# ai-forever/Kandinsky-2

Hardware: AMD Instinct MI355X
Metric: UNet denoise steps/sec @ 768x768 bs=1, 50 steps (higher is better)
Workload: dtype bf16; 1 GPU; Kandinsky-2.x text2img 768x768, decoder_steps=50, bs=1/GPU (CFG batch 2x4x96x96), 2.1-architecture UNet (1.23B) p_sampler step; parity pinned against the reference's modules; head=2.1, tile_configs_measured_in_this_process=0, images_per_gpu=1, parallelism=prompt-sharded x1, weights by one RCCL broadcast, world_size_observed=1, graph=True, chains=1, loop_graph=a 5-step loop replayed as ONE hipGraph (83 replay(s) = 415 timed steps)

## Files before the change

include/k22.h:

```cpp
#ifndef K22_H
#define K22_H
#include <stddef.h>
#include <stdint.h>
#ifdef __cplusplus
extern "C" {
#endif

#define K22_OK 0
#define K22_EINVAL (-1)
#define K22_EHIP (-2)
#define K22_ENOMEM (-3)

#define K22_BF16 0
#define K22_F32 1
#define K22_F16 2
#define K22_F16X3 3
#define K22_F16X2 4

int k22_version(void);
#define K22_BUILD_PACKED_FP32 1
#define K22_BUILD_DEBUG_VARIANTS 2
int k22_build_flags(void);
const char* k22_last_error(void);
int k22_set_option(const char* name, int value);
// ... 35 lines not shown
void k22_unet_destroy(K22UNet* u);


int k22_unet_plan(K22UNet* u, int B, int H, int W, size_t* workspace_bytes);
int k22_unet_bind(K22UNet* u, void* workspace, size_t workspace_bytes);

int k22_unet_set_condition(K22UNet* u, const float* full_emb, const float* pooled_emb, const float* image_emb,
                           void* stream);

int k22_unet_set_hint(K22UNet* u, const float* hint, void* stream);

int k22_unet_forward(K22UNet* u, const float* x, const float* timesteps, const float* inpaint_image,
                     const float* inpaint_mask, float* out, int use_graph, void* stream);

int k22_unet_sample_loop(K22UNet* u, float* x, float* x_tmp, const float* timesteps, const float* noise_seq, const float* init_img,
                         const float* mask, const float* inpaint_image, const float* inpaint_mask, const float* table,
                         const int* table_rows, int n_steps, float guidance, float clamp_lo, float clamp_hi, int pct_index,
                         double pct_gamma, void* scratch, int use_graph, void* stream);
enum { K22_LOOP_DDIM = 0, K22_LOOP_PLMS = 1 };
int k22_unet_ddim_loop(K22UNet* u, int kind, float* x, float* x_tmp, float* x0_out, const float* timesteps, const float* table,
                       const float* noise_seq, const float* inpaint_image, const float* inpaint_mask, float* eps_hist, int n_steps,
                       float guidance, int use_graph, void* stream);
int k22_unet_num_ops(const K22UNet* u);
int k22_unet_set_autotune(K22UNet* u, int on);
int k22_unet_tuning_report(const K22UNet* u, char* buf, size_t cap);

int k22_comm_broadcast_weights(void* arena, size_t bytes, int root, void* nccl_comm, void* stream);

int k22_tile_table_load(const char* path);
int k22_tile_table_save(const char* path);
int k22_tile_table_size(void);
int k22_tile_table_measured(void);
void k22_tile_table_clear(void);

int k22_unet_profile(K22UNet* u, int reps, double* ms, double* flops, double* bytes, int* launches, void* stream);

size_t k22_sampler_scratch_bytes(int N, int HW);
int k22_ddim_step(const float* x, const float* model_out, const float* noise, const float* table_row, float guidance, int use_cfg,
                  float* x_out, float* x0_out, int N, int HW, void* stream);
int k22_prepare_mask(const float* mask, float* out, int C, int H, int W, void* stream);
int k22_plms_step(const float* x, const float* model_out, const float* eps_hist1, const float* eps_hist2, const float* eps_hist3, int order,
                  const float* table_row, float guidance, int use_cfg, float* x_out, float* eps_out, float* x0_out, int N, int HW, void* stream);
int k22_sampler_step(const float* x, const float* model_out, const float* noise, const float* init_img,
                     const float* mask, const float* table, int step_index, float guidance, int use_cfg,
                     float clamp_lo, float clamp_hi, int pct_index, double pct_gamma, void* scratch,
                     float* x_out, float* x0_out, int N, int HW, void* stream);

int k22_gemm(const void* A0, const void* A1, const void* Wp, const float* bias, const void* residual, void* out,
             void* partial, int M, int N, int Npad, int K0, int K1, long lda0, long lda1, int ldo, int ldr,
             int out_f32, int act, int splitk, int bm, int bn, int dtype, void* stream);
int k22_x3_pack(const float* src, void* dst, long n, float scale, void* stream);
int k22_conv3x3(const void* x_padded, const void* Wp, const float* bias, const void* residual, void* out,
                void* partial, int B, int H, int W, int Cin, int Cout, int Npad, int out_mode, int act, int splitk,
                int bm, int bn, int dtype, void* stream);
int k22_conv3x3_skip(const void* x_padded, const void* Wp, const float* bias, const void* skip0, const void* skip1,
                     int SK0, int SK1, const void* Ws, const float* bias_s, void* out, void* partial, int B, int H, int W,
                     int Cin, int Cout, int Npad, int splitk, int bm, int dtype, void* stream);
int k22_conv3x3_gnstats(const void* x_padded, const void* Wp, const float* bias, const void* residual, void* out,
                        void* partial, int B, int H, int W, int Cin, int Cout, int Npad, int splitk, int bm, int bn,
                        float* stats, int stats_capacity_rows, int* rows_per_image, int dtype, void* stream);
int k22_gemm_gnstats(const void* A, const void* Wp, const float* bias, const void* residual, void* out, void* partial,
                     int B, int H, int W, int N, int Npad, int K, int splitk, int bm, float* stats,
                     int stats_capacity_rows, int* rows_per_image, int dtype, void* stream);
typedef struct K22IgemmProblem {
  int dtype, taps, M, N, Kc, K0, H, W;
  int out_mode, res_f32, act, a_raw, want_stats;
  int SK0, SK1;
  int att_T, att_S, att_Tkp;
  int ldo, ldr;
  int has_frag;
  int algo, bm, bn, splitk, stages;
} K22IgemmProblem;
typedef struct K22IgemmOperands {
  const void *A0, *A1, *Wp, *bias, *residual;
  void *out, *partial;
  const void *S0, *S1, *Ws, *bias2;
  void *kall, *vtall;
  const void *Wfrag, *Wsfrag;
  float* stats;
  int stats_capacity_rows;
} K22IgemmOperands;
int k22_igemm_cfg_accepted(const K22IgemmProblem* pr);
int k22_igemm_cfg(const K22IgemmProblem* pr, const K22IgemmOperands* ops, int* rows_per_image, void* stream);
int k22_debug_conv_trace(const void* x_padded, const void* Wp, const float* bias, void* out, int B, int H, int W, int Cin, int Cout,
                         int Npad, unsigned long long* trace, void* stream);
int k22_conv3x3_gn(const void* x0, const void* x1, int C0, int C1, const float* gamma, const float* beta, const float* film, long film_ld,
                   float eps, int act, void* scratch, const void* Wp, const float* bias, const void* residual, void* out, void* partial,
                   int B, int H, int W, int Cout, int Npad, int splitk, int bm, int algo, int dtype, void* stream);
int k22_groupnorm(const void* x0, const void* x1, int C0, int C1, int B, int H, int W, const float* gamma,
                  const float* beta, const float* film, long film_ld, float eps, int act, int mode, int pad,
                  void* scratch, void* out, int dtype, void* stream);
size_t k22_groupnorm_scratch_bytes(int B, int C);
int k22_attention(const void* qkv, const void* ctxkv, void* kall, void* vtall, void* out, int B, int H, int T, int S,
                  int dtype, void* stream);
int k22_qkv_project(const void* x, const void* Wp, const float* bias, void* q_out, void* kall, void* vtall,
                    int B, int H, int T, int S, int K, int bm, int bn, int dtype, void* stream);
int k22_qkv_project_stream(const void* x, const void* Wp, const float* bias, void* q_out, void* kall, void* vtall, void* partial,
                           int B, int H, int T, int S, int K, int bm, int splitk, int dtype, void* stream);
int k22_linear_smallm(const float* x, const void* W, const float* bias, const float* add, float* out, int M, int N,
                      int K, int act_in, int act_out, int wdtype, void* stream);
int k22_conv3x3_direct(const float* x, const float* w, const float* bias, float* y, int B, int Cin, int Cout, int Hin, int Win,
                       int stride, int act, void* stream);

size_t k22_afrag_bytes(int M, int K);
int k22_afrag_pack(const void* A, long lda, void* out, int M, int K, int dtype, void* stream);
int k22_skinny_gemm(const void* Afrag, const void* Wfrag, const float* bias, void* out, float* partial, int M, int N, int Npad, int K,
                    int splitk, int epi, int act, int ldo, int mt, int nb, int dtype, void* stream);
int k22_finish_ln(const float* partial, int splitk, const float* bias, float* x, long ldx, const float* gain, const float* beta, void* yfrag,
                  int M, int N, float eps, int dtype, void* stream);
int k22_small_attention(const void* qkv, const float* qkv_partial, int nsplit, const float* qkv_bias, void* out, int out_frag, int B, int H, int T,
                        int causal, const float* key_valid, int kv_n, int dtype, void* stream);

typedef struct K22PriorConfig {
  int dtype;
  int text_ctx;
  int xf_width;
  int xf_layers;
  int xf_heads;
  int xf_final_ln;
  int clip_dim;
  int clip_xf_width;
} K22PriorConfig;
typedef struct K22Prior K22Prior;
int k22_prior_create(const K22PriorConfig* cfg, const K22Weight* weights, int n_weights, K22Prior** out);
void k22_prior_destroy(K22Prior* m);
int k22_prior_plan(K22Prior* m, int B, size_t* workspace_bytes);
int k22_prior_bind(K22Prior* m, void* workspace, size_t workspace_bytes);
int k22_prior_tuning_report(const K22Prior* m, char* buf, size_t cap);
int k22_prior_forward(K22Prior* m, const float* x, const float* timesteps, const float* text_emb, const float* text_enc,
                      const float* key_valid, float* out, void* stream);
int k22_prior_sampler_step(const float* x, const float* model_out, const float* noise, const float* scales, const float* table_row,
                           float clamp, float* x_out, int bs, int D, void* stream);

typedef struct K22MoVQConfig {
  int dtype;
  int ch;
  int n_levels;
  int ch_mult[8];
  int num_res_blocks;
  int attn_levels;
  int z_channels;
  int out_ch;
} K22MoVQConfig;
typedef struct K22MoVQ K22MoVQ;
int k22_movq_create(const K22MoVQConfig* cfg, const K22Weight* weights, int n_weights, K22MoVQ** out);
void k22_movq_destroy(K22MoVQ* m);
int k22_movq_plan(K22MoVQ* m, int B, int h, int w, size_t* workspace_bytes);
int k22_movq_bind(K22MoVQ* m, void* workspace, size_t workspace_bytes);
int k22_movq_decode(K22MoVQ* m, const float* z, float* out, unsigned char* out_u8, void* stream);
int k22_movq_plan_encoder(K22MoVQ* m, int B, int H, int W, size_t* workspace_bytes);
int k22_movq_encode(K22MoVQ* m, const float* image, float* latent, void* stream);
int k22_movq_num_ops(const K22MoVQ* m);

enum { K22_ENC_CLIP_TEXT = 0, K22_ENC_CLIP_VISION = 1, K22_ENC_XLMR = 2 };
typedef struct K22EncoderConfig {
  int dtype;
  int kind;
  int width;
  int layers;
  int heads;
  int n_ctx;
  int vocab;
  int out_dim;
  int image_size;
  int patch;
  int max_pos;
// ... 47 lines not shown
```

kandinsky-2_amd/_lib.py:

```python
from __future__ import annotations

import ctypes as C
import os

_HERE = os.path.dirname(os.path.abspath(__file__))
LIB_PATH = os.environ.get("K22_LIB_PATH") or os.path.join(_HERE, "libk22hip.so")
TILE_TABLE_PATH = os.path.join(_HERE, "tiles_gfx950.txt")

K22_BF16, K22_F32, K22_F16, K22_F16X3, K22_F16X2 = 0, 1, 2, 3, 4
K22_LOOP_DDIM, K22_LOOP_PLMS = 0, 1
F16X3 = "f16x3"
F16X2 = "f16x2"
SPLIT_DTYPES = (F16X3, F16X2)
X3_WSCALE = 256.0


def dtype_code(backend_dtype) -> int:
    import torch
    try:
        return {torch.bfloat16: K22_BF16, torch.float32: K22_F32, torch.float16: K22_F16, F16X3: K22_F16X3, F16X2: K22_F16X2}[backend_dtype]
    except KeyError:
        raise ValueError('backend_dtype must be torch.bfloat16, torch.float16, torch.float32 "f16x3" or "f16x2"') from None
ACT_NONE, ACT_SILU, ACT_GELU = 0, 1, 2
OUT_ROWMAJOR, OUT_ROWMAJOR_F32, OUT_NCHW_F32, OUT_QKV = 0, 1, 2, 3
# ... 27 lines not shown


class K22PriorConfig(C.Structure):
    _fields_ = [("dtype", C.c_int), ("text_ctx", C.c_int), ("xf_width", C.c_int), ("xf_layers", C.c_int), ("xf_heads", C.c_int),
                ("xf_final_ln", C.c_int), ("clip_dim", C.c_int), ("clip_xf_width", C.c_int)]


class K22EncoderConfig(C.Structure):
    _fields_ = [("dtype", C.c_int), ("kind", C.c_int), ("width", C.c_int), ("layers", C.c_int), ("heads", C.c_int), ("n_ctx", C.c_int),
                ("vocab", C.c_int), ("out_dim", C.c_int), ("image_size", C.c_int), ("patch", C.c_int), ("max_pos", C.c_int),
                ("pad_id", C.c_int), ("ln_eps", C.c_float), ("mlp_dim", C.c_int), ("hidden_act", C.c_int)]


class K22Weight(C.Structure):
    _fields_ = [("name", C.c_char_p), ("ptr", C.c_void_p)]


_P, _I, _L, _F, _D, _Z = C.c_void_p, C.c_int, C.c_long, C.c_float, C.c_double, C.c_size_t

SIGNATURES = {
    "k22_version": (_I, []),
    "k22_build_flags": (_I, []),
    "k22_last_error": (C.c_char_p, []),
    "k22_set_option": (_I, [C.c_char_p, _I]),
    "k22_comm_broadcast_weights": (_I, [_P, _Z, _I, _P, _P]),
    "k22_tile_table_load": (_I, [C.c_char_p]),
    "k22_tile_table_save": (_I, [C.c_char_p]),
    "k22_tile_table_size": (_I, []),
    "k22_tile_table_measured": (_I, []),
    "k22_tile_table_clear": (None, []),
    "k22_unet_create": (_I, [C.POINTER(K22UNetConfig), C.POINTER(K22Weight), _I, C.POINTER(_P)]),
    "k22_unet_destroy": (None, [_P]),
    "k22_unet_plan": (_I, [_P, _I, _I, _I, C.POINTER(_Z)]),
    "k22_unet_bind": (_I, [_P, _P, _Z]),
    "k22_unet_set_condition": (_I, [_P, _P, _P, _P, _P]),
    "k22_unet_set_hint": (_I, [_P, _P, _P]),
    "k22_unet_forward": (_I, [_P, _P, _P, _P, _P, _P, _I, _P]),
    "k22_unet_sample_loop": (_I, [_P, _P, _P, _P, _P, _P, _P, _P, _P, _P, C.POINTER(_I), _I, _F, _F, _F, _I, _D, _P, _I, _P]),
    "k22_unet_ddim_loop": (_I, [_P, _I, _P, _P, _P, _P, _P, _P, _P, _P, _P, _I, _F, _I, _P]),
    "k22_unet_num_ops": (_I, [_P]),
    "k22_unet_set_autotune": (_I, [_P, _I]),
    "k22_unet_tuning_report": (_I, [_P, C.c_char_p, _Z]),
    "k22_unet_profile": (_I, [_P, _I, C.POINTER(_D), C.POINTER(_D), C.POINTER(_D), C.POINTER(_I), _P]),
    "k22_afrag_bytes": (_Z, [_I, _I]),
    "k22_afrag_pack": (_I, [_P, _L, _P, _I, _I, _I, _P]),
    "k22_skinny_gemm": (_I, [_P, _P, _P, _P, _P, _I, _I, _I, _I, _I, _I, _I, _I, _I, _I, _I, _P]),
    "k22_finish_ln": (_I, [_P, _I, _P, _P, _L, _P, _P, _P, _I, _I, _F, _I, _P]),
    "k22_small_attention": (_I, [_P, _P, _I, _P, _P, _I, _I, _I, _I, _I, _P, _I, _I, _P]),
    "k22_prior_create": (_I, [C.POINTER(K22PriorConfig), C.POINTER(K22Weight), _I, C.POINTER(_P)]),
    "k22_prior_destroy": (None, [_P]),
    "k22_prior_plan": (_I, [_P, _I, C.POINTER(_Z)]),
    "k22_prior_bind": (_I, [_P, _P, _Z]),
    "k22_prior_tuning_report": (_I, [_P, C.c_char_p, _Z]),
    "k22_prior_forward": (_I, [_P, _P, _P, _P, _P, _P, _P, _P]),
    "k22_prior_sampler_step": (_I, [_P, _P, _P, _P, _P, _F, _P, _I, _I, _P]),
    "k22_encoder_create": (_I, [C.POINTER(K22EncoderConfig), C.POINTER(K22Weight), _I, C.POINTER(_P)]),
    "k22_encoder_destroy": (None, [_P]),
    "k22_encoder_plan": (_I, [_P, _I, C.POINTER(_Z)]),
    "k22_encoder_bind": (_I, [_P, _P, _Z]),
    "k22_encoder_forward": (_I, [_P, _P, _P, _P, _P, _P, _P]),
    "k22_movq_create": (_I, [C.POINTER(K22MoVQConfig), C.POINTER(K22Weight), _I, C.POINTER(_P)]),
    "k22_movq_destroy": (None, [_P]),
    "k22_movq_plan": (_I, [_P, _I, _I, _I, C.POINTER(_Z)]),
    "k22_movq_bind": (_I, [_P, _P, _Z]),
    "k22_movq_decode": (_I, [_P, _P, _P, _P, _P]),
    "k22_movq_plan_encoder": (_I, [_P, _I, _I, _I, C.POINTER(_Z)]),
    "k22_movq_encode": (_I, [_P, _P, _P, _P]),
    "k22_movq_num_ops": (_I, [_P]),
    "k22_ddim_step": (_I, [_P, _P, _P, _P, _F, _I, _P, _P, _I, _I, _P]),
    "k22_blend_noised": (_I, [_P, _P, _P, _P, _F, _F, _P, _I, _I, _I, _I, _P]),
    "k22_prepare_mask": (_I, [_P, _P, _I, _I, _I, _P]),
    "k22_plms_step": (_I, [_P, _P, _P, _P, _P, _I, _P, _F, _I, _P, _P, _P, _I, _I, _P]),
    "k22_sampler_scratch_bytes": (_Z, [_I, _I]),
    "k22_sampler_step": (_I, [_P, _P, _P, _P, _P, _P, _I, _F, _I, _F, _F, _I, _D, _P, _P, _P, _I, _I, _P]),
    "k22_gemm": (_I, [_P, _P, _P, _P, _P, _P, _P, _I, _I, _I, _I, _I, _L, _L, _I, _I, _I, _I, _I, _I, _I, _I, _P]),
    "k22_x3_pack": (_I, [_P, _P, _L, _F, _P]),
    "k22_conv3x3": (_I, [_P, _P, _P, _P, _P, _P, _I, _I, _I, _I, _I, _I, _I, _I, _I, _I, _I, _I, _P]),
    "k22_conv3x3_skip": (_I, [_P, _P, _P, _P, _P, _I, _I, _P, _P, _P, _P, _I, _I, _I, _I, _I, _I, _I, _I, _I, _P]),
    "k22_gemm_gnstats": (_I, [_P, _P, _P, _P, _P, _P, _I, _I, _I, _I, _I, _I, _I, _I, _P, _I, C.POINTER(_I), _I, _P]),
    "k22_conv3x3_gnstats": (_I, [_P, _P, _P, _P, _P, _P, _I, _I, _I, _I, _I, _I, _I, _I, _I, _P, _I, C.POINTER(_I), _I, _P]),
    "k22_igemm_cfg_accepted": (_I, [C.POINTER(K22IgemmProblem)]),
    "k22_igemm_cfg": (_I, [C.POINTER(K22IgemmProblem), C.POINTER(K22IgemmOperands), C.POINTER(_I), _P]),
    "k22_conv3x3_gn": (_I, [_P, _P, _I, _I, _P, _P, _P, _L, _F, _I, _P, _P, _P, _P, _P, _P, _I, _I, _I, _I, _I, _I, _I, _I, _I, _P]),
    "k22_debug_conv_trace": (_I, [_P, _P, _P, _P, _I, _I, _I, _I, _I, _I, _P, _P]),
    "k22_groupnorm": (_I, [_P, _P, _I, _I, _I, _I, _I, _P, _P, _P, _L, _F, _I, _I, _I, _P, _P, _I, _P]),
    "k22_groupnorm_scratch_bytes": (_Z, [_I, _I]),
    "k22_attention": (_I, [_P, _P, _P, _P, _P, _I, _I, _I, _I, _I, _P]),
    "k22_qkv_project": (_I, [_P, _P, _P, _P, _P, _P, _I, _I, _I, _I, _I, _I, _I, _I, _P]),
    "k22_qkv_project_stream": (_I, [_P, _P, _P, _P, _P, _P, _P, _I, _I, _I, _I, _I, _I, _I, _I, _P]),
    "k22_linear_smallm": (_I, [_P, _P, _P, _P, _P, _I, _I, _I, _I, _I, _I, _P]),
    "k22_conv3x3_direct": (_I, [_P, _P, _P, _P, _I, _I, _I, _I, _I, _I, _I, _P]),
    "k22_debug_counter": (_L, [C.c_char_p]),
    "k22_stream_frag_bytes": (C.c_size_t, [_I, _I, _I, _I]),
    "k22_stream_repack": (_I, [_P, _P, _I, _I, _I, _I, _P]),
    "k22_debug_set_stream_frag": (_I, [_P, _P]),
    "k22_debug_set_stream_scratch": (_I, [_P, C.c_size_t]),
    "k22_spatialnorm_apply": (_I, [_P, _P, _P, _P, _P, _P, _P, _P, _I, _I, _I, _I, _I, _I, _I, _I, _I, _I, _P]),
    "k22_upsample2_pad": (_I, [_P, _P, _I, _I, _I, _I, _I, _P]),
    "k22_pad_copy": (_I, [_P, _P, _I, _I, _I, _I, _I, _P]),
    "k22_subsample_odd": (_I, [_P, _P, _I, _I, _I, _I, _I, _P]),
    "k22_softmax_rows": (_I, [_P, _L, _I, _F, _I, _P]),
    "k22_movq_prepare": (_I, [_P, _P, _P, _P, _P, _I, _I, _I, _I, _I, _P]),
    "k22_movq_enc_prepare": (_I, [_P, _P, _I, _I, _I, _I, _I, _P]),
    "k22_movq_quant_conv": (_I, [_P, _P, _P, _P, _I, _I, _P]),
    "k22_to_uint8_nhwc": (_I, [_P, _P, _I, _I, _I, _I, _P]),
    "k22_enc_layernorm": (_I, [_P, _L, _P, _P, _P, _L, _P, _I, _I, _F, _I, _P]),
    "k22_enc_embed": (_I, [_P, _P, _P, _P, _P, _I, _I, _I, _I, _I, _I, _I, _P]),
    "k22_enc_gather_eot": (_I, [_P, _P, _P, _I, _I, _I, _P]),
    "k22_enc_masked_mean": (_I, [_P, _P, _P, _I, _I, _I, _P]),
    "k22_enc_patchify": (_I, [_P, _P, _I, _I, _I, _I, _I, _P]),
    "k22_enc_vision_assemble": (_I, [_P, _P, _P, _P, _I, _I, _I, _P]),
    "k22_enc_mlp_act": (_I, [_P, _P, _L, _I, _I, _P]),
    "k22_enc_attention_generic": (_I, [_P, _P, _I, _I, _I, _I, _I, _P]),
    "k22_prior_layernorm": (_I, [_P, _L, _P, _P, _P, _I, _I, _I, _I, _P]),
    "k22_prior_finish_input": (_I, [_P, _P, _P, _I, _I, _I, _P]),
    "k22_attention_masked": (_I, [_P, _P, _P, _P, _P, _I, _I, _I, _I, _I, _P, _I, _I, _I, _P]),
}

_lib = None


def lib() -> C.CDLL:
    global _lib
    if _lib is None:
        if not os.path.exists(LIB_PATH):
            raise RuntimeError(
                f"{LIB_PATH} is missing: the HIP extension is the only compute path (no CPU fallback). "
                "Build it with `python -c 'import __graft_entry__ as g; g.build()'`.")
        l = C.CDLL(LIB_PATH)
        for name, (res, args) in SIGNATURES.items():
            fn = getattr(l, name)
            fn.restype = res
            fn.argtypes = args
        _lib = l
        tbl = os.environ.get("K22_TILE_TABLE", TILE_TABLE_PATH)
        if tbl != "0" and os.path.exists(tbl):
            if l.k22_tile_table_load(tbl.encode()) < 0:
                raise RuntimeError(f"k22: cannot read the tile table {tbl}")
    return _lib


def check(rc: int) -> None:
    if rc != 0:
        msg = lib().k22_last_error()
        raise RuntimeError(f"k22 error {rc}: {msg.decode() if msg else ''}")


def weight_array(arena, table):
    base = arena.data_ptr()
    arr = (K22Weight * len(table))()
    names = []
    for i, (name, (off, _n)) in enumerate(table.items()):
        nb = name.encode()
        names.append(nb)
        arr[i].name = nb
        arr[i].ptr = base + off
    return arr, names


def plan_and_bind(plan_fn, bind_fn, handle, device, *shape):
    import torch
    nbytes = C.c_size_t()
    check(plan_fn(handle, *shape, C.byref(nbytes)))
    ws = torch.empty(nbytes.value + 256, dtype=torch.uint8, device=device)
    check(bind_fn(handle, (ws.data_ptr() + 255) // 256 * 256, nbytes.value))
    return ws
# ... 13 lines not shown
```

kandinsky-2_amd/csrc/capi.hip:

```cpp
#include "kernels.h"
#include "elementwise.h"
#include "../../include/k22.h"
#include "tuning.h"
#include "skinny.h"
#include <dlfcn.h>
#include <stdio.h>
#include <string.h>

static thread_local char g_err[512] = "";

int k22_set_error(int code, const char* msg) {
  snprintf(g_err, sizeof(g_err), "%s", msg ? msg : "");
  return code;
}
int k22_set_error_hip(hipError_t e, const char* file, int line) {
  snprintf(g_err, sizeof(g_err), "HIP error %d (%s) at %s:%d", (int)e, hipGetErrorString(e), file, line);
  return K22_EHIP;
}

extern "C" {

int k22_version(void) { return 100; }
int k22_build_flags(void) {
  int f = 0;
#ifndef K22_NOPK
  f |= K22_BUILD_PACKED_FP32;
#endif
#if defined(K22_DEBUG_VARIANTS) || defined(K22_STREAM_DEBUG) || defined(K22_SKINNY_DEBUG)
  f |= K22_BUILD_DEBUG_VARIANTS;
#endif
  return f;
}

int k22_set_option(const char* name, int value) {
  if (name && !strcmp(name, "igemm_stages")) { igemm_set_default_stages(value); return K22_OK; }
  if (name && !strcmp(name, "igemm_xcd_remap")) { igemm_set_xcd_remap(value); return K22_OK; }
  if (name && !strcmp(name, "conv_algo")) { igemm_set_conv_algo(value); return K22_OK; }
  if (name && !strcmp(name, "gemm_algo")) { igemm_set_gemm_algo(value); return K22_OK; }
  if (name && !strcmp(name, "att_pipe")) { attention_set_pipe(value); return K22_OK; }
  return k22_set_error(K22_EINVAL, "k22_set_option: unknown option");
}
const char* k22_last_error(void) { return g_err; }

#ifdef K22_STREAM_DEBUG
static unsigned long long* g_dbg_trace = nullptr;
extern "C" int k22_debug_set_stream_trace(unsigned long long* t) { g_dbg_trace = t; return K22_OK; }
#define K22_DBG_TRACE(p) (p).st_trace = g_dbg_trace
#else
#define K22_DBG_TRACE(p) (void)0
#endif
static const void* g_dbg_wfrag = nullptr;
static const void* g_dbg_wsfrag = nullptr;
static void* g_dbg_scratch = nullptr;
static size_t g_dbg_scratch_bytes = 0;
static int dbg_frag(IgemmParams& p, int dtype, hipStream_t st) {
  K22_DBG_TRACE(p);
  p.Wfrag = g_dbg_wfrag; p.Wsfrag = g_dbg_wsfrag;
  if (g_dbg_wfrag || !g_dbg_scratch || dtype == K22_F32 || (p.taps != 1 && p.taps != 9) || p.Kc % 64 || p.Npad % 64) return K22_OK;
  const size_t n1 = stream_frag_bytes(p.Npad, p.taps, p.Kc, dtype);
  const bool skip = p.S0 != nullptr && p.Ws != nullptr && (p.SK0 + p.SK1) % 64 == 0;
  const size_t n2 = skip ? stream_frag_bytes(p.Npad, 1, p.SK0 + p.SK1, dtype) : 0;
  if (n1 + n2 > g_dbg_scratch_bytes) return k22_set_error(K22_ENOMEM, "debug stream scratch too small");
  if (int rc = launch_stream_repack(p.Wp, g_dbg_scratch, p.Npad, p.taps, p.Kc, dtype, st)) return rc;
  p.Wfrag = g_dbg_scratch;
  if (skip) {
    void* w2 = static_cast<char*>(g_dbg_scratch) + n1;
    if (int rc = launch_stream_repack(p.Ws, w2, p.Npad, 1, p.SK0 + p.SK1, dtype, st)) return rc;
    p.Wsfrag = w2;
  }
  return K22_OK;
}
#define K22_DBG_FRAG(p) do { if (int rc_ = dbg_frag((p), dtype, reinterpret_cast<hipStream_t>(stream))) return rc_; } while (0)
int k22_debug_set_stream_frag(const void* wfrag, const void* wsfrag) { g_dbg_wfrag = wfrag; g_dbg_wsfrag = wsfrag; return K22_OK; }
int k22_debug_set_stream_scratch(void* scratch, size_t bytes) { g_dbg_scratch = scratch; g_dbg_scratch_bytes = scratch ? bytes : 0; return K22_OK; }
size_t k22_stream_frag_bytes(int Npad, int taps, int Kc, int dtype) { return stream_frag_bytes(Npad, taps, Kc, dtype); }
int k22_stream_repack(const void* W, void* out, int Npad, int taps, int Kc, int dtype, void* stream) {
  return launch_stream_repack(W, out, Npad, taps, Kc, dtype, reinterpret_cast<hipStream_t>(stream));
}

long k22_debug_counter(const char* name) {
  if (name && !strcmp(name, "stream_launches")) return stream_launch_count();
  if (name && !strcmp(name, "loop_captures")) return loop_capture_count();
  if (name && !strcmp(name, "loop_launches")) return loop_launch_count();
  return -1;
}

int k22_comm_broadcast_weights(void* arena, size_t bytes, int root, void* nccl_comm, void* stream) {
  if (!arena || !nccl_comm) return k22_set_error(K22_EINVAL, "k22_comm_broadcast_weights: null arena / communicator");
  typedef int (*bcast_fn)(const void*, void*, size_t, int , int, void*, hipStream_t);
  static bcast_fn fn = nullptr;
  if (!fn) {
    void* sym = dlsym(RTLD_DEFAULT, "ncclBroadcast");
    if (!sym) {
      void* h = dlopen("librccl.so.1", RTLD_NOW | RTLD_GLOBAL);
      if (!h) h = dlopen("librccl.so", RTLD_NOW | RTLD_GLOBAL);
      if (h) sym = dlsym(h, "ncclBroadcast");
    }
    if (!sym) return k22_set_error(K22_EINVAL, "k22_comm_broadcast_weights: RCCL (ncclBroadcast) is not loadable in this process");
    fn = reinterpret_cast<bcast_fn>(sym);
  }
  const size_t piece = (size_t)1 << 30;
  char* base = reinterpret_cast<char*>(arena);
  for (size_t off = 0; off < bytes; off += piece) {
    const size_t n = bytes - off < piece ? bytes - off : piece;
    const int rc = fn(base + off, base + off, n,  1, root, nccl_comm, reinterpret_cast<hipStream_t>(stream));
    if (rc != 0) { char msg[96]; snprintf(msg, sizeof msg, "k22_comm_broadcast_weights: ncclBroadcast returned %d", rc); return k22_set_error(K22_EHIP, msg); }
  }
  return K22_OK;
}

int k22_tile_table_load(const char* path) {
  if (!path) return k22_set_error(K22_EINVAL, "k22_tile_table_load: null path");
  const int n = tile_table_load_file(path);
  if (n < 0) return k22_set_error(K22_EINVAL, "k22_tile_table_load: cannot read the file");
  return n;
}
int k22_tile_table_save(const char* path) {
  if (!path) return k22_set_error(K22_EINVAL, "k22_tile_table_save: null path");
  const int n = tile_table_save_file(path);
  if (n < 0) return k22_set_error(K22_EINVAL, "k22_tile_table_save: cannot write the file");
  return n;
}
int k22_tile_table_size(void) {
  TileTable& tt = tile_table();
  std::lock_guard<std::mutex> lk(tt.mu);
  return (int)tt.m.size();
}
int k22_tile_table_measured(void) {
  TileTable& tt = tile_table();
  std::lock_guard<std::mutex> lk(tt.mu);
  return (int)tt.measured;
}
void k22_tile_table_clear(void) {
  TileTable& tt = tile_table();
  std::lock_guard<std::mutex> lk(tt.mu);
  tt.m.clear();
  tt.measured = 0;
}

// ... 75 lines not shown
                     int Cin, int Cout, int Npad, int splitk, int bm, int dtype, void* stream) {
  IgemmParams p = {};
  p.stages = -1;
  p.A0 = x_padded; p.Wp = Wp; p.bias = bias; p.out = out; p.partial = reinterpret_cast<float*>(partial);
  p.M = B * H * W; p.N = Cout; p.Npad = Npad; p.Kc = Cin; p.K0 = Cin; p.taps = 9; p.H = H; p.W = W;
  p.ldo = Cout; p.ldr = Cout; p.out_mode = IG_OUT_ROWMAJOR; p.act = K22_ACT_NONE; p.splitk = splitk; p.force_bm = bm; p.force_bn = 0;
  p.S0 = skip0; p.S1 = skip1; p.SK0 = SK0; p.SK1 = SK1; p.Ws = Ws; p.bias2 = bias_s; p.algo = 0;
  if (p.splitk == 0) p.splitk = partial ? igemm_choose_splitk(p, dtype) : 1;
  K22_DBG_FRAG(p);
  return launch_igemm(p, dtype, reinterpret_cast<hipStream_t>(stream));
}

static int igemm_problem_tuned(const K22IgemmProblem& d, Tuned& t) {
  if (d.dtype < K22_BF16 || d.dtype > K22_F16X2) return k22_set_error(K22_EINVAL, "igemm_cfg: bad dtype");
  if ((d.taps != 1 && d.taps != 9) || d.M <= 0 || d.N <= 0 || d.Kc <= 0 || d.K0 <= 0 || d.K0 > d.Kc)
    return k22_set_error(K22_EINVAL, "igemm_cfg: bad problem (taps 1 / 9, M, N > 0, 0 < K0 <= Kc)");
  if (d.out_mode < IG_OUT_ROWMAJOR || d.out_mode > IG_OUT_QKV || d.SK0 < 0 || d.SK1 < 0 || (d.SK1 > 0 && d.SK0 == 0))
    return k22_set_error(K22_EINVAL, "igemm_cfg: bad output mode / skip widths");
  if (d.taps == 9 && (d.H <= 0 || d.W <= 0 || d.M % (d.H * d.W))) return k22_set_error(K22_EINVAL, "igemm_cfg: a convolution needs M = B * H * W");
  const void* mark = reinterpret_cast<const void*>(1);
  IgemmParams& p = t.p;
  p = IgemmParams{};
  p.stages = -1;
  p.M = d.M; p.N = d.N; p.Npad = (d.N + 63) / 64 * 64; p.Kc = d.Kc; p.K0 = d.K0; p.taps = d.taps; p.H = d.H; p.W = d.W;
  p.lda0 = d.K0; p.lda1 = d.Kc - d.K0;
  p.ldo = d.ldo > 0 ? d.ldo : (d.out_mode == IG_OUT_QKV ? d.N / 3 : d.N);
  p.ldr = d.ldr > 0 ? d.ldr : (d.res_f32 ? p.ldo : d.N);
  p.out_mode = d.out_mode; p.act = d.act; p.res_f32 = d.res_f32 ? 1 : 0; p.a_raw = d.a_raw ? 1 : 0;
  p.Wp = mark; p.bias = reinterpret_cast<const float*>(mark);
  if (d.SK0 > 0) { p.S0 = mark; p.S1 = d.SK1 > 0 ? mark : nullptr; p.SK0 = d.SK0; p.SK1 = d.SK1; p.Ws = mark; p.bias2 = reinterpret_cast<const float*>(mark); }
  if (d.out_mode == IG_OUT_QKV) { p.att_T = d.att_T; p.att_S = d.att_S; p.att_Tkp = d.att_Tkp; }
  if (d.has_frag) { p.Wfrag = mark; if (d.SK0 > 0) p.Wsfrag = mark; }
  t.want_stats = d.want_stats != 0;
  t.dt = d.dtype;
  tuned_make_candidates(t, d.dtype);
  return K22_OK;
}
static Cfg igemm_problem_cfg(const K22IgemmProblem& d) {
  Cfg c; c.algo = d.algo; c.bm = d.bm; c.bn = d.bn; c.splitk = d.splitk; c.stages = d.stages;
  return c;
}

int k22_igemm_cfg_accepted(const K22IgemmProblem* pr) {
  if (!pr) return k22_set_error(K22_EINVAL, "igemm_cfg_accepted: null problem");
  Tuned t;
  if (int rc = igemm_problem_tuned(*pr, t)) return rc;
  return tuned_is_candidate(t, igemm_problem_cfg(*pr)) ? 1 : 0;
}

int k22_igemm_cfg(const K22IgemmProblem* pr, const K22IgemmOperands* ops, int* rows_per_image, void* stream) {
  if (rows_per_image) *rows_per_image = 0;
  if (!pr || !ops) return k22_set_error(K22_EINVAL, "igemm_cfg: null problem / operands");
  const K22IgemmProblem& d = *pr;
  const K22IgemmOperands& o = *ops;
  Tuned t;
  if (int rc = igemm_problem_tuned(d, t)) return rc;
  const Cfg c = igemm_problem_cfg(d);
  if (!tuned_is_candidate(t, c)) return k22_set_error(K22_EINVAL, "igemm_cfg: this build does not generate the configuration for the problem");
  if (!o.A0 || !o.Wp || !o.out) return k22_set_error(K22_EINVAL, "igemm_cfg: A0, Wp and out are required");
  if (d.K0 < d.Kc && !o.A1) return k22_set_error(K22_EINVAL, "igemm_cfg: A1 missing for the concat operand");
  if (d.SK0 > 0 && (!o.S0 || !o.Ws || (d.SK1 > 0 && !o.S1))) return k22_set_error(K22_EINVAL, "igemm_cfg: fused-skip operands missing");
  if (d.out_mode == IG_OUT_QKV && (!o.kall || !o.vtall)) return k22_set_error(K22_EINVAL, "igemm_cfg: kall / vtall missing");
  if ((c.splitk > 1 || c.algo == 20) && !o.partial) return k22_set_error(K22_EINVAL, "igemm_cfg: the configuration needs the fp32 partial buffer");
  if (c.algo == 20 && (!o.Wfrag || (d.SK0 > 0 && !o.Wsfrag))) return k22_set_error(K22_EINVAL, "igemm_cfg: algo 20 needs the fragment-major weights");
  IgemmParams q = t.p;
  tuned_apply_cfg(q, c);
  q.A0 = o.A0; q.A1 = o.A1; q.Wp = o.Wp; q.bias = reinterpret_cast<const float*>(o.bias); q.residual = o.residual; q.out = o.out;
  q.partial = reinterpret_cast<float*>(o.partial);
  q.S0 = d.SK0 > 0 ? o.S0 : nullptr; q.S1 = d.SK1 > 0 ? o.S1 : nullptr; q.Ws = d.SK0 > 0 ? o.Ws : nullptr;
  q.bias2 = d.SK0 > 0 ? reinterpret_cast<const float*>(o.bias2) : nullptr;
  q.kall = o.kall; q.vtall = o.vtall;
  q.Wfrag = c.algo == 20 ? o.Wfrag : nullptr; q.Wsfrag = (c.algo == 20 && d.SK0 > 0) ? o.Wsfrag : nullptr;
  if (t.want_stats) {
    const int rpi = igemm_stats_rows_per_image(q, d.dtype);
    const int B = d.H > 0 ? d.M / (d.H * d.W) : 1;
    if (rpi <= 0) return k22_set_error(K22_EINVAL, "igemm_cfg: this configuration cannot produce GroupNorm partial sums");
    if (!o.stats || (long)rpi * B > o.stats_capacity_rows) return k22_set_error(K22_ENOMEM, "igemm_cfg: stats buffer missing / too small");
    if (rows_per_image) *rows_per_image = rpi;
    q.stats = o.stats;
  }
  return launch_igemm(q, d.dtype, reinterpret_cast<hipStream_t>(stream));
}

int k22_debug_conv_trace(const void* x_padded, const void* Wp, const float* bias, void* out, int B, int H, int W, int Cin, int Cout,
                         int Npad, unsigned long long* trace, void* stream) {
  IgemmParams p = {};
  p.stages = -1;
  p.A0 = x_padded; p.Wp = Wp; p.bias = bias; p.out = out;
  p.M = B * H * W; p.N = Cout; p.Npad = Npad; p.Kc = Cin; p.K0 = Cin; p.taps = 9; p.H = H; p.W = W;
  p.ldo = Cout; p.ldr = Cout; p.out_mode = IG_OUT_ROWMAJOR; p.act = K22_ACT_NONE; p.splitk = 1; p.trace = trace;
  return launch_conv3_halo_trace(p, K22_BF16, reinterpret_cast<hipStream_t>(stream));
}

size_t k22_groupnorm_scratch_bytes(int B, int C) {
  return (size_t)B * 128 * C * 2 * sizeof(float) + (size_t)B * C * 2 * sizeof(float) + 512;
}

int k22_groupnorm(const void* x0, const void* x1, int C0, int C1, int B, int H, int W, const float* gamma,
                  const float* beta, const float* film, long film_ld, float eps, int act, int mode, int pad,
                  void* scratch, void* out, int dtype, void* stream) {
  hipStream_t st = reinterpret_cast<hipStream_t>(stream);
  const int C = C0 + C1, HW = H * W;
  const int out_x3 = k22_is_split(dtype) ? 1 : 0;
  dtype = k22_storage_dtype(dtype);
  float* partial = reinterpret_cast<float*>(scratch);
  float* coeff = partial + (size_t)B * 128 * C * 2;
  const int rc = launch_gn_stats_coeff(x0, x1, C0, C1, B, HW, eps, gamma, beta, film, film_ld, partial, coeff, dtype, st);
  if (rc) return rc;
  GnApplyParams ap = {};
  ap.x0 = x0; ap.x1 = x1; ap.C0 = C0; ap.C1 = C1; ap.B = B; ap.H = H; ap.W = W; ap.mode = mode; ap.pad = pad; ap.act = act;
  ap.coeff = coeff; ap.out = out; ap.out_x3 = out_x3;
  return launch_gn_apply(ap, dtype, st);
}

int k22_conv3x3_gn(const void* x0, const void* x1, int C0, int C1, const float* gamma, const float* beta, const float* film, long film_ld,
                   float eps, int act, void* scratch, const void* Wp, const float* bias, const void* residual, void* out, void* partial,
                   int B, int H, int W, int Cout, int Npad, int splitk, int bm, int algo, int dtype, void* stream) {
  hipStream_t st = reinterpret_cast<hipStream_t>(stream);
  const int C = C0 + C1, HW = H * W;
  const int sdt = k22_storage_dtype(dtype);
  float* part = reinterpret_cast<float*>(scratch);
  float* coeff = part + (size_t)B * 128 * C * 2;
  const int rc = launch_gn_stats_coeff(x0, x1, C0, C1, B, HW, eps, gamma, beta, film, film_ld, part, coeff, sdt, st);
  if (rc) return rc;
  IgemmParams p = {};
  p.stages = -1;
  p.Wp = Wp; p.bias = bias; p.residual = residual; p.out = out; p.partial = reinterpret_cast<float*>(partial);
  p.M = B * H * W; p.N = Cout; p.Npad = Npad; p.Kc = C; p.K0 = C; p.taps = 9; p.H = H; p.W = W;
  p.ldo = Cout; p.ldr = Cout; p.out_mode = IG_OUT_ROWMAJOR; p.act = K22_ACT_NONE; p.splitk = splitk > 0 ? splitk : 1; p.force_bm = bm; p.algo = algo;
  p.gn_coeff = coeff; p.gn_x0 = x0; p.gn_x1 = x1; p.gn_C0 = C0; p.gn_act = act;
  return launch_igemm(p, dtype, st);
}


int k22_attention(const void* qkv, const void* ctxkv, void* kall, void* vtall, void* out, int B, int H, int T, int S,
                  int dtype, void* stream) {
  hipStream_t st = reinterpret_cast<hipStream_t>(stream);
  const int C = H * 64, Tk = S + T, Tkp = (Tk + 63) / 64 * 64;
  KvPackParams kp;
  kp.qkv = qkv; kp.ctxkv = ctxkv; kp.kall = kall; kp.vtall = vtall; kp.B = B; kp.H = H; kp.T = T; kp.S = S; kp.Tkp = Tkp;
  int rc = launch_kv_pack(kp, k22_storage_dtype(dtype), st);
  if (rc) return rc;
  AttentionParams ap = {};
  ap.q = qkv; ap.ldq = 3 * C; ap.kall = kall; ap.vtall = vtall; ap.out = out; ap.ldo = C;
  ap.B = B; ap.H = H; ap.T = T; ap.Tk = Tk; ap.Tkp = Tkp; ap.scale = 0.125f;
  return launch_attention(ap, dtype, st);
}

int k22_qkv_project(const void* x, const void* Wp, const float* bias, void* q_out, void* kall, void* vtall,
                    int B, int H, int T, int S, int K, int bm, int bn, int dtype, void* stream) {
  const int C = H * 64, Tkp = (S + T + 63) / 64 * 64;
  IgemmParams p = {};
  p.stages = -1;
  p.A0 = x; p.Wp = Wp; p.bias = bias; p.out = q_out; p.kall = kall; p.vtall = vtall;
  p.M = B * T; p.N = 3 * C; p.Npad = 3 * C; p.Kc = K; p.K0 = K; p.taps = 1; p.lda0 = K; p.lda1 = 0;
  p.ldo = C; p.ldr = 3 * C; p.out_mode = IG_OUT_QKV; p.act = K22_ACT_NONE; p.splitk = 1; p.force_bm = bm; p.force_bn = bn;
  p.att_T = T; p.att_S = S; p.att_Tkp = Tkp; p.H = 1; p.W = T;
  p.a_raw = k22_is_split(dtype) ? 1 : 0;
  K22_DBG_FRAG(p);
  return launch_igemm(p, dtype, reinterpret_cast<hipStream_t>(stream));
}

int k22_qkv_project_stream(const void* x, const void* Wp, const float* bias, void* q_out, void* kall, void* vtall, void* partial,
                           int B, int H, int T, int S, int K, int bm, int splitk, int dtype, void* stream) {
  const int C = H * 64, Tkp = (S + T + 63) / 64 * 64;
  IgemmParams p = {};
// ... 177 lines not shown
```

kandinsky-2_amd/csrc/common.h:

```cpp
#pragma once
#include <hip/hip_runtime.h>
#include <stdint.h>

typedef unsigned short bf16_t;
typedef _Float16 f16_t;
typedef __attribute__((ext_vector_type(8))) __bf16 bf16x8_t;
typedef __attribute__((ext_vector_type(8))) _Float16 f16x8_t;
typedef __attribute__((ext_vector_type(2))) _Float16 f16x2_t;
typedef __attribute__((ext_vector_type(16))) float f32x16_t;
typedef __attribute__((ext_vector_type(4))) float f32x4_t;
typedef __attribute__((ext_vector_type(4))) unsigned int u32x4_t;

enum K22DType { K22_BF16 = 0, K22_F32 = 1, K22_F16 = 2, K22_F16X3 = 3, K22_F16X2 = 4 };
inline bool k22_is_split(int dtype) { return dtype == K22_F16X3 || dtype == K22_F16X2; }
inline int k22_esz(int dtype) { return (dtype == K22_F32 || k22_is_split(dtype)) ? 4 : 2; }
inline int k22_bk(int dtype) { return (dtype == K22_F32 || k22_is_split(dtype)) ? 32 : 64; }
inline bool k22_dtype_ok(int dtype) { return dtype == K22_BF16 || dtype == K22_F32 || dtype == K22_F16; }
inline int k22_storage_dtype(int dtype) { return k22_is_split(dtype) ? (int)K22_F32 : dtype; }
enum K22Act { K22_ACT_NONE = 0, K22_ACT_SILU = 1, K22_ACT_GELU = 2 };

__device__ __forceinline__ float bf16_to_f32(bf16_t v) { return __uint_as_float(((uint32_t)v) << 16); }
typedef __attribute__((ext_vector_type(2))) float f32x2_t;
typedef __attribute__((ext_vector_type(2))) __bf16 bf16x2_t;
__device__ __forceinline__ uint32_t pack2_bf16(float lo, float hi) {
// ... 111 lines not shown
  f.hi = c0;
  f.lo = c1;
}
__device__ __forceinline__ void x3_frag_from_f32(Frag<x3_t>& f, const float4 a, const float4 b) {
  const u32x4_t s0 = x3_split4(a), s1 = x3_split4(b);
  f.hi = u32x4_t{s0.x, s0.y, s1.x, s1.y};
  f.lo = u32x4_t{s0.z, s0.w, s1.z, s1.w};
}
__device__ __forceinline__ void x3_frag_from_chunks(Frag<x2_t>& f, const u32x4_t c0, const u32x4_t c1) {
  f.hi = c0;
  f.lo = c1;
}
__device__ __forceinline__ void x3_frag_from_f32(FragHi& f, const float4 a, const float4 b) {
  f.hi = u32x4_t{pack2_f16(a.x, a.y), pack2_f16(a.z, a.w), pack2_f16(b.x, b.y), pack2_f16(b.z, b.w)};
}

__device__ __forceinline__ int lds_chunk_off(int r, int c) { return r * 128 + ((c ^ ((r >> 1) & 7)) << 4); }

__device__ __forceinline__ void ld_frag(Frag<bf16_t>& f, const char* tile, int r, int ks, int h) {
  f.v = *reinterpret_cast<const u32x4_t*>(tile + lds_chunk_off(r, 2 * ks + h));
}
__device__ __forceinline__ void ld_frag(Frag<f16_t>& f, const char* tile, int r, int ks, int h) {
  f.v = *reinterpret_cast<const u32x4_t*>(tile + lds_chunk_off(r, 2 * ks + h));
}
__device__ __forceinline__ void ld_frag(Frag<float>& f, const char* tile, int r, int ks, int h) {
  const float4 a = *reinterpret_cast<const float4*>(tile + lds_chunk_off(r, 4 * ks + 2 * h));
  const float4 b = *reinterpret_cast<const float4*>(tile + lds_chunk_off(r, 4 * ks + 2 * h + 1));
  f.v[0] = a.x; f.v[1] = a.y; f.v[2] = a.z; f.v[3] = a.w;
  f.v[4] = b.x; f.v[5] = b.y; f.v[6] = b.z; f.v[7] = b.w;
}
__device__ __forceinline__ void ld_frag(Frag<x3_t>& f, const char* tile, int r, int ks, int h) {
  x3_frag_from_chunks(f, *reinterpret_cast<const u32x4_t*>(tile + lds_chunk_off(r, 4 * ks + 2 * h)),
                      *reinterpret_cast<const u32x4_t*>(tile + lds_chunk_off(r, 4 * ks + 2 * h + 1)));
}
__device__ __forceinline__ void ld_frag(Frag<x2_t>& f, const char* tile, int r, int ks, int h) {
  x3_frag_from_chunks(f, *reinterpret_cast<const u32x4_t*>(tile + lds_chunk_off(r, 4 * ks + 2 * h)),
                      *reinterpret_cast<const u32x4_t*>(tile + lds_chunk_off(r, 4 * ks + 2 * h + 1)));
}
__device__ __forceinline__ void ld_frag(FragHi& f, const char* tile, int r, int ks, int h) {
  f.hi = *reinterpret_cast<const u32x4_t*>(tile + lds_chunk_off(r, 4 * ks + 2 * h));
}
template <bool RAW, typename T, typename F> __device__ __forceinline__ void ld_frag_a(F& f, const char* tile, int r, int ks, int h) {
  if constexpr (RAW && is_x3<T>::value) {
    x3_frag_from_f32(f, *reinterpret_cast<const float4*>(tile + lds_chunk_off(r, 4 * ks + 2 * h)),
                     *reinterpret_cast<const float4*>(tile + lds_chunk_off(r, 4 * ks + 2 * h + 1)));
  } else {
    ld_frag(f, tile, r, ks, h);
  }
}

__device__ __forceinline__ void mma_atom(f32x16_t& acc, const Frag<bf16_t>& a, const Frag<bf16_t>& b) {
  acc = __builtin_amdgcn_mfma_f32_32x32x16_bf16(__builtin_bit_cast(bf16x8_t, a.v), __builtin_bit_cast(bf16x8_t, b.v),
                                                acc, 0, 0, 0);
}
__device__ __forceinline__ void mma_atom(f32x16_t& acc, const Frag<f16_t>& a, const Frag<f16_t>& b) {
  acc = __builtin_amdgcn_mfma_f32_32x32x16_f16(__builtin_bit_cast(f16x8_t, a.v), __builtin_bit_cast(f16x8_t, b.v), acc, 0, 0, 0);
}
__device__ __forceinline__ void mma_atom(f32x16_t& acc, const Frag<float>& a, const Frag<float>& b) {
#pragma unroll
  for (int j = 0; j < 8; ++j) acc = __builtin_amdgcn_mfma_f32_32x32x2f32(a.v[j], b.v[j], acc, 0, 0, 0);
}

__device__ __forceinline__ void mma_atom(f32x16_t& acc, const Frag<x3_t>& a, const Frag<x3_t>& b) {
  acc = __builtin_amdgcn_mfma_f32_32x32x16_f16(__builtin_bit_cast(f16x8_t, a.hi), __builtin_bit_cast(f16x8_t, b.hi), acc, 0, 0, 0);
  acc = __builtin_amdgcn_mfma_f32_32x32x16_f16(__builtin_bit_cast(f16x8_t, a.hi), __builtin_bit_cast(f16x8_t, b.lo), acc, 0, 0, 0);
  acc = __builtin_amdgcn_mfma_f32_32x32x16_f16(__builtin_bit_cast(f16x8_t, a.lo), __builtin_bit_cast(f16x8_t, b.hi), acc, 0, 0, 0);
}
__device__ __forceinline__ void mma_atom(f32x16_t& acc, const Frag<x2_t>& w, const FragHi& a) {
  acc = __builtin_amdgcn_mfma_f32_32x32x16_f16(__builtin_bit_cast(f16x8_t, w.hi), __builtin_bit_cast(f16x8_t, a.hi), acc, 0, 0, 0);
  acc = __builtin_amdgcn_mfma_f32_32x32x16_f16(__builtin_bit_cast(f16x8_t, w.lo), __builtin_bit_cast(f16x8_t, a.hi), acc, 0, 0, 0);
}
template <typename T> __device__ __forceinline__ float acc_unscale(float v) {
  if constexpr (is_x3<T>::value) return v * K22_X3_WSCALE_INV; else return v;
}

__device__ __forceinline__ int c_row(int reg, int lane) { return (reg & 3) + 8 * (reg >> 2) + 4 * (lane >> 5); }

__device__ __forceinline__ void raw_barrier() {
  asm volatile("" ::: "memory");
  __builtin_amdgcn_s_barrier();
  asm volatile("" ::: "memory");
}

__device__ __forceinline__ float wave_sum(float v) {
#pragma unroll
  for (int o = 32; o > 0; o >>= 1) v += __shfl_xor(v, o, 64);
  return v;
}
__device__ __forceinline__ float wave_max(float v) {
#pragma unroll
  for (int o = 32; o > 0; o >>= 1) v = fmaxf(v, __shfl_xor(v, o, 64));
  return v;
}

template <typename T> struct Vec16;
template <> struct Vec16<bf16_t> {
  static constexpr int N = 8;
  uint4 raw;
  __device__ __forceinline__ float get(int i) const {
    const uint32_t w = (&raw.x)[i >> 1];
    return __uint_as_float((i & 1) ? (w & 0xffff0000u) : (w << 16));
  }
  __device__ __forceinline__ void set2(int pair, float lo, float hi) {
    (&raw.x)[pair] = pack2_bf16(lo, hi);
  }
};
template <> struct Vec16<f16_t> {
  static constexpr int N = 8;
  uint4 raw;
  __device__ __forceinline__ float get(int i) const {
    const f16x2_t v = __builtin_bit_cast(f16x2_t, (&raw.x)[i >> 1]);
    return (float)v[i & 1];
  }
  __device__ __forceinline__ void set2(int pair, float lo, float hi) { (&raw.x)[pair] = pack2_f16(lo, hi); }
};
template <> struct Vec16<float> {
  static constexpr int N = 4;
  float4 raw;
  __device__ __forceinline__ float get(int i) const { return (&raw.x)[i]; }
  __device__ __forceinline__ void set2(int pair, float lo, float hi) {
    (&raw.x)[2 * pair] = lo;
    (&raw.x)[2 * pair + 1] = hi;
  }
};
template <> struct Vec16<x3_t> : Vec16<float> {};
template <> struct Vec16<x2_t> : Vec16<float> {};

#define K22_CHECK_LAUNCH()                                   \
  do {                                                       \
    hipError_t e__ = hipGetLastError();                      \
    if (e__ != hipSuccess) return k22_set_error_hip(e__, __FILE__, __LINE__); \
  } while (0)

int k22_set_error(int code, const char* msg);
int k22_set_error_hip(hipError_t e, const char* file, int line);
```

kandinsky-2_amd/csrc/conv3_common.h:

```cpp
#pragma once
#include "kernels.h"
#include <stdlib.h>

namespace {

template <int N> __device__ __forceinline__ void wait_vmcnt() { asm volatile("s_waitcnt vmcnt(%0)" ::"n"(N) : "memory"); }

__device__ __forceinline__ void ld_frag_at(Frag<bf16_t>& f, const char* rowp, int sw, int ks, int h) {
  f.v = *reinterpret_cast<const u32x4_t*>(rowp + (((2 * ks + h) ^ sw) << 4));
}
__device__ __forceinline__ void ld_frag_at(Frag<f16_t>& f, const char* rowp, int sw, int ks, int h) {
  f.v = *reinterpret_cast<const u32x4_t*>(rowp + (((2 * ks + h) ^ sw) << 4));
}
__device__ __forceinline__ void ld_frag_at(Frag<float>& f, const char* rowp, int sw, int ks, int h) {
  const float4 a = *reinterpret_cast<const float4*>(rowp + (((4 * ks + 2 * h) ^ sw) << 4));
  const float4 b = *reinterpret_cast<const float4*>(rowp + (((4 * ks + 2 * h + 1) ^ sw) << 4));
  f.v[0] = a.x; f.v[1] = a.y; f.v[2] = a.z; f.v[3] = a.w;
  f.v[4] = b.x; f.v[5] = b.y; f.v[6] = b.z; f.v[7] = b.w;
}

__device__ __forceinline__ void ld_frag_at(Frag<x3_t>& f, const char* rowp, int sw, int ks, int h) {
  x3_frag_from_chunks(f, *reinterpret_cast<const u32x4_t*>(rowp + (((4 * ks + 2 * h) ^ sw) << 4)),
                      *reinterpret_cast<const u32x4_t*>(rowp + (((4 * ks + 2 * h + 1) ^ sw) << 4)));
}
__device__ __forceinline__ void ld_frag_at(Frag<x2_t>& f, const char* rowp, int sw, int ks, int h) {
  x3_frag_from_chunks(f, *reinterpret_cast<const u32x4_t*>(rowp + (((4 * ks + 2 * h) ^ sw) << 4)),
                      *reinterpret_cast<const u32x4_t*>(rowp + (((4 * ks + 2 * h + 1) ^ sw) << 4)));
}
__device__ __forceinline__ void ld_frag_at(FragHi& f, const char* rowp, int sw, int ks, int h) {
  f.hi = *reinterpret_cast<const u32x4_t*>(rowp + (((4 * ks + 2 * h) ^ sw) << 4));
}
template <bool RAW, typename T, typename F> __device__ __forceinline__ void ld_frag_at_a(F& f, const char* rowp, int sw, int ks, int h) {
  if constexpr (RAW && is_x3<T>::value) {
    x3_frag_from_f32(f, *reinterpret_cast<const float4*>(rowp + (((4 * ks + 2 * h) ^ sw) << 4)),
                     *reinterpret_cast<const float4*>(rowp + (((4 * ks + 2 * h + 1) ^ sw) << 4)));
  } else {
    ld_frag_at(f, rowp, sw, ks, h);
  }
}

template <typename T> __device__ __forceinline__ void store8(T* dst, const float* v);
template <> __device__ __forceinline__ void store8<bf16_t>(bf16_t* dst, const float* v) {
  uint4 w;
  w.x = pack2_bf16(v[0], v[1]);
  w.y = pack2_bf16(v[2], v[3]);
  w.z = pack2_bf16(v[4], v[5]);
  w.w = pack2_bf16(v[6], v[7]);
  *reinterpret_cast<uint4*>(dst) = w;
}
template <> __device__ __forceinline__ void store8<f16_t>(f16_t* dst, const float* v) {
  uint4 w;
  w.x = pack2_f16(v[0], v[1]);
  w.y = pack2_f16(v[2], v[3]);
  w.z = pack2_f16(v[4], v[5]);
  w.w = pack2_f16(v[6], v[7]);
  *reinterpret_cast<uint4*>(dst) = w;
}
template <> __device__ __forceinline__ void store8<float>(float* dst, const float* v) {
  *reinterpret_cast<float4*>(dst) = make_float4(v[0], v[1], v[2], v[3]);
  *reinterpret_cast<float4*>(dst + 4) = make_float4(v[4], v[5], v[6], v[7]);
}
template <> __device__ __forceinline__ void store8<x3_t>(x3_t* dst, const float* v) { store8<float>(reinterpret_cast<float*>(dst), v); }
template <> __device__ __forceinline__ void store8<x2_t>(x2_t* dst, const float* v) { store8<float>(reinterpret_cast<float*>(dst), v); }
template <typename T> __device__ __forceinline__ void load8f(const T* src, float* v);
template <> __device__ __forceinline__ void load8f<bf16_t>(const bf16_t* src, float* v) {
  const uint4 r = *reinterpret_cast<const uint4*>(src);
  v[0] = __uint_as_float(r.x << 16); v[1] = __uint_as_float(r.x & 0xffff0000u);
  v[2] = __uint_as_float(r.y << 16); v[3] = __uint_as_float(r.y & 0xffff0000u);
  v[4] = __uint_as_float(r.z << 16); v[5] = __uint_as_float(r.z & 0xffff0000u);
  v[6] = __uint_as_float(r.w << 16); v[7] = __uint_as_float(r.w & 0xffff0000u);
}
template <> __device__ __forceinline__ void load8f<f16_t>(const f16_t* src, float* v) {
  const uint4 r = *reinterpret_cast<const uint4*>(src);
  unpack2_f16(r.x, v[0], v[1]); unpack2_f16(r.y, v[2], v[3]); unpack2_f16(r.z, v[4], v[5]); unpack2_f16(r.w, v[6], v[7]);
}
template <> __device__ __forceinline__ void load8f<float>(const float* src, float* v) {
  const float4 a = *reinterpret_cast<const float4*>(src), b = *reinterpret_cast<const float4*>(src + 4);
  v[0] = a.x; v[1] = a.y; v[2] = a.z; v[3] = a.w; v[4] = b.x; v[5] = b.y; v[6] = b.z; v[7] = b.w;
}
template <> __device__ __forceinline__ void load8f<x3_t>(const x3_t* src, float* v) { load8f<float>(reinterpret_cast<const float*>(src), v); }
template <> __device__ __forceinline__ void load8f<x2_t>(const x2_t* src, float* v) { load8f<float>(reinterpret_cast<const float*>(src), v); }
template <typename T> __device__ __forceinline__ float stored(float v);
template <> __device__ __forceinline__ float stored<bf16_t>(float v) { return bf16_to_f32(f32_to_bf16(v)); }
template <> __device__ __forceinline__ float stored<f16_t>(float v) { return (float)(f16_t)v; }
template <> __device__ __forceinline__ float stored<float>(float v) { return v; }
template <> __device__ __forceinline__ float stored<x3_t>(float v) { return v; }
template <> __device__ __forceinline__ float stored<x2_t>(float v) { return v; }

__device__ __forceinline__ int xcd_remap_h(int bid, int nblocks) {
  const int q = nblocks >> 3, r = nblocks & 7, x = bid & 7;
  return (x < r ? x * (q + 1) : r * (q + 1) + (x - r) * q) + (bid >> 3);
}

__device__ __forceinline__ void glds16_asm(const void* g, unsigned lds_dst) {
  unsigned keep;
  asm volatile("s_mov_b32 %0, m0\n\ts_mov_b32 m0, %2\n\ts_nop 0\n\tglobal_load_lds_dwordx4 %1, off\n\ts_mov_b32 m0, %0"
               : "=&s"(keep) : "v"(g), "s"(lds_dst) : "memory");
}


__device__ __forceinline__ u32x4_t gn_rewrite16(bf16_t, u32x4_t raw, const float* cf, int act, bool border) {
  float v[8];
  unpack2_bf16(raw.x, v[0], v[1]); unpack2_bf16(raw.y, v[2], v[3]); unpack2_bf16(raw.z, v[4], v[5]); unpack2_bf16(raw.w, v[6], v[7]);
#pragma unroll
  for (int k = 0; k < 8; ++k) v[k] = apply_act(v[k] * cf[2 * k] + cf[2 * k + 1], act);
  const u32x4_t o = {pack2_bf16(v[0], v[1]), pack2_bf16(v[2], v[3]), pack2_bf16(v[4], v[5]), pack2_bf16(v[6], v[7])};
  return border ? u32x4_t{0u, 0u, 0u, 0u} : o;
}
__device__ __forceinline__ u32x4_t gn_rewrite16(f16_t, u32x4_t raw, const float* cf, int act, bool border) {
  float v[8];
  unpack2_f16(raw.x, v[0], v[1]); unpack2_f16(raw.y, v[2], v[3]); unpack2_f16(raw.z, v[4], v[5]); unpack2_f16(raw.w, v[6], v[7]);
#pragma unroll
  for (int k = 0; k < 8; ++k) v[k] = apply_act(v[k] * cf[2 * k] + cf[2 * k + 1], act);
  const u32x4_t o = {pack2_f16(v[0], v[1]), pack2_f16(v[2], v[3]), pack2_f16(v[4], v[5]), pack2_f16(v[6], v[7])};
  return border ? u32x4_t{0u, 0u, 0u, 0u} : o;
}
__device__ __forceinline__ u32x4_t gn_rewrite16(float, u32x4_t raw, const float* cf, int act, bool border) {
  float v[4] = {__uint_as_float(raw.x), __uint_as_float(raw.y), __uint_as_float(raw.z), __uint_as_float(raw.w)};
#pragma unroll
  for (int k = 0; k < 4; ++k) v[k] = apply_act_sel<false>(v[k] * cf[2 * k] + cf[2 * k + 1], act);
  const u32x4_t o = {__float_as_uint(v[0]), __float_as_uint(v[1]), __float_as_uint(v[2]), __float_as_uint(v[3])};
  return border ? u32x4_t{0u, 0u, 0u, 0u} : o;
}
__device__ __forceinline__ u32x4_t gn_rewrite16(x3_t, u32x4_t raw, const float* cf, int act, bool border) {
  float v[4] = {__uint_as_float(raw.x), __uint_as_float(raw.y), __uint_as_float(raw.z), __uint_as_float(raw.w)};
#pragma unroll
  for (int k = 0; k < 4; ++k) v[k] = apply_act_sel<true>(v[k] * cf[2 * k] + cf[2 * k + 1], act);
  const u32x4_t o = x3_split4(v[0], v[1], v[2], v[3]);
  return border ? u32x4_t{0u, 0u, 0u, 0u} : o;
}
__device__ __forceinline__ u32x4_t gn_rewrite16(x2_t, u32x4_t raw, const float* cf, int act, bool border) { return gn_rewrite16(x3_t{}, raw, cf, act, border); }
__device__ __forceinline__ void gload16_asm(u32x4_t& dst, const void* g) {
  asm volatile("global_load_dwordx4 %0, %1, off" : "=v"(dst) : "v"(g) : "memory");
}
template <int N> __device__ __forceinline__ void gn_wait(u32x4_t (&c)[4]) {
  asm volatile("s_waitcnt vmcnt(%4)" : "+v"(c[0]), "+v"(c[1]), "+v"(c[2]), "+v"(c[3]) : "n"(N) : "memory");
}
template <int N> __device__ __forceinline__ void gn_wait(u32x4_t (&c)[2]) {
  asm volatile("s_waitcnt vmcnt(%2)" : "+v"(c[0]), "+v"(c[1]) : "n"(N) : "memory");
}

__device__ __forceinline__ void glds16w_asm(const void* g, unsigned lds_dst) {
#ifdef K22_W_NT
  unsigned keep;
  asm volatile("s_mov_b32 %0, m0\n\ts_mov_b32 m0, %2\n\ts_nop 0\n\tglobal_load_lds_dwordx4 %1, off nt\n\ts_mov_b32 m0, %0"
               : "=&s"(keep) : "v"(g), "s"(lds_dst) : "memory");
#else
  glds16_asm(g, lds_dst);
#endif
}

constexpr int HALO_BN = 128;
constexpr int HALO_NW = 8;
constexpr int HALO_MAXA = 8;

template <int NBST> constexpr int halo_count_a(int t) {
  int c = 0;
  for (int k = 1; k <= NBST - 1; ++k) {
    const int u = t - k;
    if (u >= 0 && u <= 9 - NBST) ++c;
  }
  return c;
}

}

template <typename T, int BM, bool PLAIN = false, bool SPEC = false>
__device__ __forceinline__ void halo_tail(const IgemmParams& p, f32x16_t (&acc)[SPEC ? BM / 64 : BM / 128][2], char* smem, int bx, int bz, int img, int v0, int n0) {
  using TR = TT<T>;
  constexpr int BK = TR::BK, EPC = TR::EPC, KSTEPS = TR::KSTEPS;
  constexpr int BN = HALO_BN, NW = HALO_NW, WM = SPEC ? 2 : 4, WN = 2;
  constexpr int MI = BM / (WM * 32), NI = BN / (WN * 32);
  constexpr int B_SLOTS = BN / 8 / NW;
  constexpr int B_BYTES = BN * 128;
  constexpr int TS = BN * 4 + 16;
  const int tid = threadIdx.x, lane = tid & 63;
  const int wave = __builtin_amdgcn_readfirstlane(tid >> 6);
  const int wm = wave >> 1, wn = wave & 1;
  const bool cw = !SPEC || wave < 4;
  const int h = lane >> 5, l31 = lane & 31;
  const int W2 = PLAIN ? 1 : p.W + 2;
  const int VR = PLAIN ? (p.H > 0 ? p.H * p.W : p.M) : p.H * W2;
  const int abase = wm * (BM / WM) + l31;
  int brow[NI];
#pragma unroll
  for (int ni = 0; ni < NI; ++ni) brow[ni] = (wn * (BN / WN) + ni * 32 + l31) * 128;
  const int bsw = (l31 >> 1) & 7;

  if (p.S0 != nullptr) {
    const int SK = p.SK0 + p.SK1;
    const int nss = SK / BK;
    const int sp = p.splitk > 1 ? p.splitk : 1;
    const int q0 = nss * bz / sp, q1 = nss * (bz + 1) / sp;
    if (q0 < q1) {
      constexpr int SA_SLOTS = BM / 8 / NW;
      constexpr int SBUF = BM * 128 + B_BYTES;
      wait_vmcnt<0>();
      __syncthreads();
      int spix[SA_SLOTS], schunk[SA_SLOTS];
#pragma unroll
      for (int i = 0; i < SA_SLOTS; ++i) {
        const int row = 8 * (wave + NW * i) + (lane >> 3);
        int v = v0 + row;
        if (v > VR - 1) v = VR - 1;
        const int y = v / W2;
        int x = v - y * W2;
        if (x > p.W - 1) x = p.W - 1;
        spix[i] = (img * p.H + y) * p.W + x;
        schunk[i] = ((lane & 7) ^ ((row >> 1) & 7)) * EPC;
      }
      int wsoff[B_SLOTS];
#pragma unroll
      for (int i = 0; i < B_SLOTS; ++i) {
        const int row = 8 * (wave + NW * i) + (lane >> 3);
        int n = n0 + row;
        if (n > p.Npad - 1) n = p.Npad - 1;
        wsoff[i] = n * SK + ((lane & 7) ^ ((row >> 1) & 7)) * EPC;
      }
      const T* __restrict__ X0 = reinterpret_cast<const T*>(p.S0);
      const T* __restrict__ X1 = reinterpret_cast<const T*>(p.S1);
      const T* __restrict__ Ws = reinterpret_cast<const T*>(p.Ws);
      constexpr int NSK = BM == 256 ? 3 : 4;
      constexpr int SCH = SA_SLOTS + B_SLOTS;
      const unsigned lds0 = __builtin_amdgcn_readfirstlane((unsigned)(size_t)(__attribute__((address_space(3))) char*)smem);
#define K22_ISSUE_SKIP(Q, BUFI)                                                                            \
      {                                                                                                    \
        int q_ = (Q);                                                                                      \
        if (q_ > q1 - 1) q_ = q1 - 1;                                                                      \
        const int k0_ = q_ * BK;                                                                           \
        const bool second_ = k0_ >= p.SK0;                                                                 \
        const T* xs_ = second_ ? X1 : X0;                                                                  \
        const int ldx_ = second_ ? p.SK1 : p.SK0;                                                          \
        const int kk_ = second_ ? k0_ - p.SK0 : k0_;                                                       \
        const unsigned dA_ = lds0 + (BUFI) * SBUF + wave * 1024;                                           \
        _Pragma("unroll") for (int i = 0; i < SA_SLOTS; ++i)                                               \
            glds16_asm(xs_ + (int64_t)spix[i] * ldx_ + kk_ + schunk[i], __builtin_amdgcn_readfirstlane(dA_ + i * NW * 1024)); \
        _Pragma("unroll") for (int i = 0; i < B_SLOTS; ++i)                                                \
            glds16w_asm(Ws + wsoff[i] + k0_, __builtin_amdgcn_readfirstlane(dA_ + BM * 128 + i * NW * 1024)); \
      }
#pragma unroll
      for (int t = 0; t < NSK - 1; ++t) K22_ISSUE_SKIP(q0 + t, t);
      int buf = 0, fill = NSK - 1;
      for (int q = q0; q < q1; ++q) {
        wait_vmcnt<(NSK - 2) * SCH>();
        raw_barrier();
        K22_ISSUE_SKIP(q + NSK - 1, fill);
        const char* sA = smem + buf * SBUF;
        const char* sB = sA + BM * 128;
        if (cw) {
        using TSK = typename SkipT<T>::type;
#pragma unroll
        for (int ks = 0; ks < KSTEPS; ++ks) {
          Frag<TSK> a[MI], b[NI];
#pragma unroll
          for (int mi = 0; mi < MI; ++mi) ld_frag_at_a<true, TSK>(a[mi], sA + (abase + mi * 32) * 128, bsw, ks, h);
#pragma unroll
          for (int ni = 0; ni < NI; ++ni) ld_frag_at(b[ni], sB + brow[ni], bsw, ks, h);
#pragma unroll
          for (int mi = 0; mi < MI; ++mi)
#pragma unroll
            for (int ni = 0; ni < NI; ++ni) mma_atom(acc[mi][ni], b[ni], a[mi]);
        }
        }
        asm volatile("s_waitcnt lgkmcnt(0)" ::: "memory");
        buf = (buf + 1 == NSK) ? 0 : buf + 1;
        fill = (fill + 1 == NSK) ? 0 : fill + 1;
      }
#undef K22_ISSUE_SKIP
    }
  }
  wait_vmcnt<0>();
  __syncthreads();

  if (cw)
#pragma unroll
  for (int mi = 0; mi < MI; ++mi) {
    const int row = wm * (BM / WM) + mi * 32 + l31;
#pragma unroll
    for (int ni = 0; ni < NI; ++ni)
#pragma unroll
      for (int j = 0; j < 4; ++j) {
        const int col = wn * (BN / WN) + ni * 32 + 8 * j + 4 * h;
        *reinterpret_cast<float4*>(smem + row * TS + col * 4) =
            make_float4(acc_unscale<T>(acc[mi][ni][4 * j]), acc_unscale<T>(acc[mi][ni][4 * j + 1]), acc_unscale<T>(acc[mi][ni][4 * j + 2]),
                        acc_unscale<T>(acc[mi][ni][4 * j + 3]));
      }
  }
  __syncthreads();

  if constexpr (PLAIN) {
    if (p.out_mode == IG_OUT_QKV && n0 >= 2 * (p.N / 3)) {
      const int C = p.N / 3, heads = C >> 6;
      constexpr int CPG = BN / (512 / BM);
      const int r = tid % BM, cg = tid / BM;
      const int v = v0 + r;
      if (v < VR) {
#pragma unroll 4
        for (int c4 = 0; c4 < CPG; c4 += 4) {
          const int col = cg * CPG + c4, n = n0 + col;
          if (n >= p.N) break;
          const float4 t = *reinterpret_cast<const float4*>(smem + r * TS + col * 4);
          float4 b = make_float4(0.f, 0.f, 0.f, 0.f);
          if (p.bias != nullptr) b = *reinterpret_cast<const float4*>(p.bias + n);
          const int c = n - 2 * C, head = c >> 6, d = c & 63;
          T* vt = reinterpret_cast<T*>(p.vtall) + ((int64_t)(img * heads + head) * 64 + d) * p.att_Tkp + p.att_S + v;
          vt[0] = from_f32<T>(t.x + b.x);
          vt[(int64_t)p.att_Tkp] = from_f32<T>(t.y + b.y);
          vt[(int64_t)2 * p.att_Tkp] = from_f32<T>(t.z + b.z);
          vt[(int64_t)3 * p.att_Tkp] = from_f32<T>(t.w + b.w);
        }
      }
      return;
    }
  }

  constexpr int SEGS = BN / 8;
  constexpr int RGS = 512 / SEGS;
  constexpr int RPT = BM / RGS;
  const int cs = tid % SEGS, rg = tid / SEGS;
  const int n = n0 + cs * 8;
  const bool n_ok = n < p.N;
  float bias8[8];
#pragma unroll
  for (int e = 0; e < 8; ++e) bias8[e] = 0.f;
  const bool finish = (p.splitk <= 1);
  if (finish && n_ok && p.bias != nullptr) {
    const float4 b0 = *reinterpret_cast<const float4*>(p.bias + n), b1 = *reinterpret_cast<const float4*>(p.bias + n + 4);
    bias8[0] = b0.x; bias8[1] = b0.y; bias8[2] = b0.z; bias8[3] = b0.w;
    bias8[4] = b1.x; bias8[5] = b1.y; bias8[6] = b1.z; bias8[7] = b1.w;
  }
  if (finish && n_ok && p.bias2 != nullptr) {
    const float4 b0 = *reinterpret_cast<const float4*>(p.bias2 + n), b1 = *reinterpret_cast<const float4*>(p.bias2 + n + 4);
    bias8[0] += b0.x; bias8[1] += b0.y; bias8[2] += b0.z; bias8[3] += b0.w;
    bias8[4] += b1.x; bias8[5] += b1.y; bias8[6] += b1.z; bias8[7] += b1.w;
  }
  const T* __restrict__ res = reinterpret_cast<const T*>(p.residual);
  float* part = finish ? nullptr : p.partial + (int64_t)bz * p.M * p.N;
  float ssum[8], ssq[8];
#pragma unroll
  for (int e = 0; e < 8; ++e) { ssum[e] = 0.f; ssq[e] = 0.f; }
#pragma unroll
  for (int k = 0; k < RPT; ++k) {
    const int row = rg * RPT + k;
    const int v = v0 + row;
    int64_t m;
    if constexpr (PLAIN) {
      if (!n_ok || v >= VR) continue;
      m = (int64_t)img * VR + v;
    } else {
      const int y = v / W2, x = v - y * W2;
      if (!n_ok || v >= VR || x >= p.W) continue;
      m = ((int64_t)img * p.H + y) * p.W + x;
    }
    const float4 t0 = *reinterpret_cast<const float4*>(smem + row * TS + cs * 32);
    const float4 t1 = *reinterpret_cast<const float4*>(smem + row * TS + cs * 32 + 16);
    float val[8] = {t0.x, t0.y, t0.z, t0.w, t1.x, t1.y, t1.z, t1.w};
    if (!finish) {
      *reinterpret_cast<float4*>(part + m * p.N + n) = t0;
      *reinterpret_cast<float4*>(part + m * p.N + n + 4) = t1;
      continue;
    }
#pragma unroll
    for (int e = 0; e < 8; ++e) val[e] += bias8[e];
    if (res != nullptr) {
      float rv[8];
      load8f<T>(res + m * p.ldr + n, rv);
#pragma unroll
      for (int e = 0; e < 8; ++e) val[e] += rv[e];
    }
#pragma unroll
    for (int e = 0; e < 8; ++e) val[e] = apply_act(val[e], p.act);
    if (PLAIN && p.out_mode == IG_OUT_QKV) {
      const int C = p.N / 3, heads = C >> 6;
      const int which = n / C, c = n - which * C;
      const int head = c >> 6, d = c & 63;
      if (which == 0) {
        store8<T>(reinterpret_cast<T*>(p.out) + m * p.ldo + c, val);
      } else if (which == 1) {
        store8<T>(reinterpret_cast<T*>(p.kall) + ((int64_t)(img * heads + head) * p.att_Tkp + p.att_S + v) * 64 + d, val);
      } else {
        T* vt = reinterpret_cast<T*>(p.vtall) + ((int64_t)(img * heads + head) * 64 + d) * p.att_Tkp + p.att_S + v;
#pragma unroll
        for (int e = 0; e < 8; ++e) vt[(int64_t)e * p.att_Tkp] = from_f32<T>(val[e]);
      }
      continue;
    }
    if (p.out_mode == IG_OUT_ROWMAJOR) store8<T>(reinterpret_cast<T*>(p.out) + m * p.ldo + n, val);
    else store8<float>(reinterpret_cast<float*>(p.out) + m * p.ldo + n, val);
    if (p.stats != nullptr) {
#pragma unroll
      for (int e = 0; e < 8; ++e) {
        const float sv = (p.out_mode == IG_OUT_ROWMAJOR) ? stored<T>(val[e]) : val[e];
        ssum[e] += sv;
        ssq[e] += sv * sv;
      }
    }
  }
  if (!finish || p.stats == nullptr) return;

  __syncthreads();
  float* red = reinterpret_cast<float*>(smem);
#pragma unroll
  for (int e = 0; e < 8; ++e) {
    *reinterpret_cast<float2*>(red + ((rg * BN) + cs * 8 + e) * 2) = make_float2(ssum[e], ssq[e]);
  }
  __syncthreads();
  if (tid < BN * 2) {
    const int ch = tid >> 1, which = tid & 1;
    float a = 0.f;
#pragma unroll 8
    for (int r = 0; r < RGS; ++r) a += red[((r * BN) + ch) * 2 + which];
    if (n0 + ch < p.N) p.stats[((int64_t)bx * p.N + n0 + ch) * 2 + which] = a;
  }
}

inline int halo_rows(const IgemmParams& p, int bm) { return (bm + 2 * (p.W + 2) + 2 + 7) & ~7; }

inline size_t halo_smem_bytes(const IgemmParams& p, int bm, int nbst) {
  const size_t main_loop = (size_t)2 * halo_rows(p, bm) * 128 + (size_t)nbst * HALO_BN * 128 + (p.gn_coeff ? 1024 : 0);
  const size_t epi = (size_t)bm * (HALO_BN * 4 + 16);
  const size_t red = (size_t)32 * HALO_BN * 2 * 4;
  const size_t skip = p.S0 ? (size_t)(bm == 256 ? 3 : 4) * (bm * 128 + HALO_BN * 128) : 0;
  size_t m = main_loop > epi ? main_loop : epi;
  m = m > skip ? m : skip;
  return m > red ? m : red;
}

inline int halo_pick_nbst(const IgemmParams& p, int bm) {
  const int np = halo_rows(p, bm) / 8;
  for (int nbst : {6, 4, 3, 2}) {
    if (np > (10 - nbst) * HALO_NW) continue;
    if (halo_smem_bytes(p, bm, nbst) > 160 * 1024) continue;
    return nbst;
  }
  return 0;
}
```

kandinsky-2_amd/csrc/conv3_halo.hip:

```cpp
#include "conv3_common.h"

int launch_conv3_halo_spec(const IgemmParams& p, int dtype, int bm, int nbst, int splitk, hipStream_t stream);
#ifdef K22_DEBUG_VARIANTS
int launch_conv3_halo_spec_debug(const IgemmParams& p, int nbst, int splitk, hipStream_t stream);
#endif

template <typename T, int BM, int NBST, bool TRACE = false, int LW = 8, int MODE = 0>
__global__ __launch_bounds__(512) void conv3_halo_kernel(const IgemmParams p) {
  constexpr bool PIPE = MODE == 1;
  constexpr bool GASM = MODE == 1 || MODE == 2;
  constexpr bool DBG_NOLOAD = MODE == 3;
  constexpr bool DBG_NOMMA = MODE == 4;
  using TR = TT<T>;
  constexpr int BK = TR::BK, EPC = TR::EPC, KSTEPS = TR::KSTEPS;
  constexpr int BN = HALO_BN, NW = LW, WM = 4, WN = 2;
  constexpr int MI = BM / (WM * 32), NI = BN / (WN * 32);
  constexpr int B_SLOTS = BN / 8 / NW;
  constexpr int B_BYTES = BN * 128;
  constexpr int APT = HALO_NW / LW;
  constexpr int A_SLOTS = (10 - NBST) * APT;
  constexpr int GM = 8;
  extern __shared__ __attribute__((aligned(16))) char smem[];

  const int tid = threadIdx.x, lane = tid & 63;
  const int wave = __builtin_amdgcn_readfirstlane(tid >> 6);
  const int wm = wave >> 1, wn = wave & 1;
  const int h = lane >> 5, l31 = lane & 31;
  const bool loader = LW == HALO_NW || wave < LW;

  const int W2 = p.W + 2;
  const int VR = p.H * W2;
  const int TPI = (VR + BM - 1) / BM;
  const int HRp = (BM + 2 * W2 + 2 + 7) & ~7;
  const int NP = HRp >> 3;
  const int A_BYTES = HRp * 128;
  const int PR_MAX = (p.H + 2) * W2 - 1;
  const int B = p.M / (p.H * p.W);

  const int gx = B * TPI, gy = (p.N + BN - 1) / BN;
  int L = p.xcd_remap ? xcd_remap_h(blockIdx.x, gridDim.x) : (int)blockIdx.x;
  const int per_z = gx * gy;
  const int bz = L / per_z;
  L -= bz * per_z;
  const int grp = L / (GM * gy);
  const int first_m = grp * GM;
  const int gsz = gx - first_m < GM ? gx - first_m : GM;
  const int lin = L - grp * GM * gy;
  const int bx = first_m + lin % gsz, by = lin / gsz;
  const int img = bx / TPI, v0 = (bx - img * TPI) * BM;
  const int n0 = by * BN;

  const T* __restrict__ Aimg = reinterpret_cast<const T*>(p.A0) + (int64_t)img * (p.H + 2) * W2 * p.Kc;
  const T* __restrict__ Wp = reinterpret_cast<const T*>(p.Wp);

  int aoff[A_SLOTS];
#pragma unroll
  for (int q = 0; q < A_SLOTS; ++q) {
    int j = q * NW + wave;
    if (j > NP - 1) j = NP - 1;
    const int hr = 8 * j + (lane >> 3);
    int pr = v0 + hr;
    if (pr > PR_MAX) pr = PR_MAX;
    const int chunk = (lane & 7) ^ ((hr >> 1) & 7);
    aoff[q] = pr * p.Kc + chunk * EPC;
  }
  int boff[B_SLOTS];
#pragma unroll
  for (int i = 0; i < B_SLOTS; ++i) {
    const int row = 8 * (wave + NW * i) + (lane >> 3);
    int n = n0 + row;
    if (n > p.Npad - 1) n = p.Npad - 1;
    const int chunk = (lane & 7) ^ ((row >> 1) & 7);
    boff[i] = n * 9 * p.Kc + chunk * EPC;
  }
  const int nslab = p.Kc / BK;
  int s0 = 0, s1 = nslab;
  if (p.splitk > 1) {
    const int per = (nslab + p.splitk - 1) / p.splitk;
    s0 = bz * per;
    s1 = s0 + per < nslab ? s0 + per : nslab;
  }

  f32x16_t acc[MI][NI];
#pragma unroll
  for (int mi = 0; mi < MI; ++mi)
#pragma unroll
    for (int ni = 0; ni < NI; ++ni)
#pragma unroll
      for (int r = 0; r < 16; ++r) acc[mi][ni][r] = 0.f;

  FragA<T> pa[MI];
  Frag<T> pb[NI];
  if constexpr (PIPE) {
#pragma unroll
    for (int mi = 0; mi < MI; ++mi) pa[mi] = FragA<T>{};
#pragma unroll
    for (int ni = 0; ni < NI; ++ni) pb[ni] = Frag<T>{};
  }
  char* const Bst = smem + 2 * A_BYTES;
  const int abase = wm * (BM / WM) + l31;
  int brow[NI];
#pragma unroll
  for (int ni = 0; ni < NI; ++ni) brow[ni] = (wn * (BN / WN) + ni * 32 + l31) * 128;
  const int bsw = (l31 >> 1) & 7;

  const unsigned lds0 = __builtin_amdgcn_readfirstlane((unsigned)(size_t)(__attribute__((address_space(3))) char*)smem);
#define K22_ISSUE_A(Q, SLAB, DST)                                                                          \
  {                                                                                                        \
    int j_ = (Q) * NW + wave;                                                                              \
    if (j_ > NP - 1) j_ = NP - 1;                                                                          \
    if constexpr (GASM)                                                                                    \
      glds16_asm(Aimg + aoff[Q] + (SLAB) * BK, __builtin_amdgcn_readfirstlane(lds0 + (unsigned)((DST) - smem) + j_ * 1024)); \
    else                                                                                                   \
    __builtin_amdgcn_global_load_lds((const __attribute__((address_space(1))) void*)(Aimg + aoff[Q] + (SLAB) * BK), \
                                     (__attribute__((address_space(3))) void*)((DST) + j_ * 1024), 16, 0, 0); \
  }
#define K22_ISSUE_B(SLAB, TAP, STAGE)                                                                      \
  {                                                                                                        \
    const int kofs_ = (TAP) * p.Kc + (SLAB) * BK;                                                          \
    char* dst_ = Bst + (STAGE) * B_BYTES + wave * 1024;                                                    \
    _Pragma("unroll") for (int i = 0; i < B_SLOTS; ++i) {                                                  \
      if constexpr (GASM)                                                                                  \
        glds16w_asm(Wp + boff[i] + kofs_, __builtin_amdgcn_readfirstlane(lds0 + (unsigned)(dst_ - smem) + i * NW * 1024)); \
      else                                                                                                 \
        __builtin_amdgcn_global_load_lds((const __attribute__((address_space(1))) void*)(Wp + boff[i] + kofs_), \
                                         (__attribute__((address_space(3))) void*)(dst_ + i * NW * 1024), 16, 0, 0); \
    }                                                                                                      \
  }

  if (s0 < s1) {
    if (loader) {
#pragma unroll
      for (int q = 0; q < A_SLOTS; ++q) K22_ISSUE_A(q, s0, smem);
#pragma unroll
      for (int t = 0; t < NBST - 1; ++t) K22_ISSUE_B(s0, t, t);
    }
    int trace_it = 0;
    (void)trace_it;
    int cur = 0;
    int fill = NBST - 1;
    for (int s = s0; s < s1; ++s) {
      char* const Acur = smem + ((s - s0) & 1) * A_BYTES;
      char* const Anext = smem + (((s - s0) & 1) ^ 1) * A_BYTES;
      const int sn = s + 1 < s1 ? s + 1 : s1 - 1;
#define K22_TAP(TAP)                                                                                       \
      {                                                                                                    \
        unsigned long long tr0_ = 0, tr1_ = 0, tr2_ = 0;                                                   \
        if constexpr (TRACE) tr0_ = __builtin_amdgcn_s_memtime();                                          \
        if (loader && !DBG_NOLOAD) wait_vmcnt<B_SLOTS * (NBST - 2) + APT * halo_count_a<NBST>(TAP)>();     \
        if constexpr (TRACE) tr1_ = __builtin_amdgcn_s_memtime();                                          \
        raw_barrier();                                                                      \
        if constexpr (TRACE) tr2_ = __builtin_amdgcn_s_memtime();                                          \
                    \
        if (loader && !DBG_NOLOAD) {                                                                       \
          constexpr int ta_ = ((TAP) + NBST - 1) % 9;                                                      \
          const int sa_ = ((TAP) + NBST - 1 >= 9) ? sn : s;                                                \
          K22_ISSUE_B(sa_, ta_, fill);                                                                     \
          if constexpr ((TAP) <= 9 - NBST) {                                                               \
            _Pragma("unroll") for (int a_ = 0; a_ < APT; ++a_) {                                           \
              constexpr int qb_ = ((TAP) <= 9 - NBST ? (TAP) : 0) * APT;                                   \
              K22_ISSUE_A(qb_ + a_, sn, Anext);                                                            \
            }                                                                                              \
          }                                                                                                \
        }                                                                                                  \
        const char* Bcur = Bst + cur * B_BYTES;                                                            \
        const int shift = ((TAP) / 3) * W2 + ((TAP) % 3);                                                  \
        const char* arow[MI];                                                                              \
        int asw[MI];                                                                                       \
        _Pragma("unroll") for (int mi = 0; mi < MI; ++mi) {                                                \
          const int ar = abase + mi * 32 + shift;                                                          \
          arow[mi] = Acur + ar * 128;                                                                      \
          asw[mi] = (ar >> 1) & 7;                                                                         \
        }                                                                                                  \
        if constexpr (PIPE) {                                                                              \
          FragA<T> ca[MI];                                                                                 \
          Frag<T> cb[NI];                                                                                  \
          _Pragma("unroll") for (int ks = 0; ks < KSTEPS; ks += 2) {                                       \
            _Pragma("unroll") for (int mi = 0; mi < MI; ++mi) ld_frag_at(ca[mi], arow[mi], asw[mi], ks, h); \
            _Pragma("unroll") for (int ni = 0; ni < NI; ++ni) ld_frag_at(cb[ni], Bcur + brow[ni], bsw, ks, h); \
            __builtin_amdgcn_sched_barrier(0);                                                             \
            _Pragma("unroll") for (int mi = 0; mi < MI; ++mi)                                              \
              _Pragma("unroll") for (int ni = 0; ni < NI; ++ni) mma_atom(acc[mi][ni], pb[ni], pa[mi]);     \
            __builtin_amdgcn_sched_barrier(0);                                                             \
            _Pragma("unroll") for (int mi = 0; mi < MI; ++mi) ld_frag_at(pa[mi], arow[mi], asw[mi], ks + 1, h); \
            _Pragma("unroll") for (int ni = 0; ni < NI; ++ni) ld_frag_at(pb[ni], Bcur + brow[ni], bsw, ks + 1, h); \
            __builtin_amdgcn_sched_barrier(0);                                                             \
            _Pragma("unroll") for (int mi = 0; mi < MI; ++mi)                                              \
              _Pragma("unroll") for (int ni = 0; ni < NI; ++ni) mma_atom(acc[mi][ni], cb[ni], ca[mi]);     \
            __builtin_amdgcn_sched_barrier(0);                                                             \
          }                                                                                                \
           \
          asm volatile("s_waitcnt lgkmcnt(0)" ::: "memory");                                               \
        } else {                                                                                           \
        _Pragma("unroll") for (int ks = 0; ks < KSTEPS; ++ks) {                                            \
          FragA<T> a[MI];                                                                                  \
          Frag<T> b[NI];                                                                                   \
          _Pragma("unroll") for (int mi = 0; mi < MI; ++mi) ld_frag_at(a[mi], arow[mi], asw[mi], ks, h);   \
          _Pragma("unroll") for (int ni = 0; ni < NI; ++ni) ld_frag_at(b[ni], Bcur + brow[ni], bsw, ks, h); \
          if constexpr (DBG_NOMMA) {                                                                       \
            _Pragma("unroll") for (int mi = 0; mi < MI; ++mi) asm volatile("" ::"v"(a[mi].v));             \
            _Pragma("unroll") for (int ni = 0; ni < NI; ++ni) asm volatile("" ::"v"(b[ni].v));             \
          } else {                                                                                         \
          _Pragma("unroll") for (int mi = 0; mi < MI; ++mi)                                                \
            _Pragma("unroll") for (int ni = 0; ni < NI; ++ni) mma_atom(acc[mi][ni], b[ni], a[mi]);         \
          }                                                                                                \
        }                                                                                                  \
         \
        asm volatile("s_waitcnt lgkmcnt(0)" ::: "memory");                                                 \
        }                                                                                                  \
        if constexpr (TRACE) {                                                                             \
                      \
          asm volatile("" ::"v"(acc[0][0][0]), "v"(acc[MI - 1][NI - 1][15]));                             \
          const unsigned long long tr3_ = __builtin_amdgcn_s_memtime();                                    \
          if (blockIdx.x == 0 && (wave == 0 || wave == 5) && lane == 0 && p.trace != nullptr) {            \
            unsigned long long* o_ = p.trace + ((size_t)(wave ? 1 : 0) * 4096 + (size_t)trace_it * 4);     \
            if (trace_it < 1024) { o_[0] = tr0_; o_[1] = tr1_; o_[2] = tr2_; o_[3] = tr3_; }                \
          }                                                                                                \
          ++trace_it;                                                                                      \
        }                                                                                                  \
        cur = (cur + 1 == NBST) ? 0 : cur + 1;                                                             \
        fill = (fill + 1 == NBST) ? 0 : fill + 1;                                                          \
      }
      K22_TAP(0) K22_TAP(1) K22_TAP(2) K22_TAP(3) K22_TAP(4) K22_TAP(5) K22_TAP(6) K22_TAP(7) K22_TAP(8)
#undef K22_TAP
    }
  }
#undef K22_ISSUE_A
#undef K22_ISSUE_B
  if constexpr (PIPE) {
#pragma unroll
    for (int mi = 0; mi < MI; ++mi)
#pragma unroll
      for (int ni = 0; ni < NI; ++ni) mma_atom(acc[mi][ni], pb[ni], pa[mi]);
  }
  halo_tail<T, BM>(p, acc, smem, bx, bz, img, v0, n0);
}

template <typename T, int BM, int NST, bool ARAW = false>
__global__ __launch_bounds__(512) void gemm8_kernel(const IgemmParams p) {
  using TR = TT<T>;
  constexpr int BK = TR::BK, EPC = TR::EPC, KSTEPS = TR::KSTEPS;
  constexpr int BN = HALO_BN, NW = HALO_NW, WM = 4, WN = 2;
  constexpr int MI = BM / (WM * 32), NI = BN / (WN * 32);
  constexpr int A_SLOTS = BM / 8 / NW, B_SLOTS = BN / 8 / NW, CH = A_SLOTS + B_SLOTS;
  constexpr int A_BYTES = BM * 128, B_BYTES = BN * 128, BUF = A_BYTES + B_BYTES;
  constexpr int GM = 8;
  extern __shared__ __attribute__((aligned(16))) char smem[];

  const int tid = threadIdx.x, lane = tid & 63;
  const int wave = __builtin_amdgcn_readfirstlane(tid >> 6);
  const int wm = wave >> 1, wn = wave & 1;
  const int h = lane >> 5, l31 = lane & 31;

  const int HW = p.H > 0 ? p.H * p.W : p.M;
  const int TPI = (HW + BM - 1) / BM;
  const int B = p.M / HW;
  const int gx = B * TPI, gy = (p.N + BN - 1) / BN;
  int L = p.xcd_remap ? xcd_remap_h(blockIdx.x, gridDim.x) : (int)blockIdx.x;
  const int per_z = gx * gy;
  const int bz = L / per_z;
  L -= bz * per_z;
  const int grp = L / (GM * gy);
  const int first_m = grp * GM;
  const int gsz = gx - first_m < GM ? gx - first_m : GM;
  const int lin = L - grp * GM * gy;
  const int bx = first_m + lin % gsz, by = lin / gsz;
  const int img = bx / TPI, v0 = (bx - img * TPI) * BM;
  const int n0 = by * BN;

  const T* __restrict__ A = reinterpret_cast<const T*>(p.A0) + (int64_t)img * HW * p.lda0;
  const T* __restrict__ Wp = reinterpret_cast<const T*>(p.Wp);
  int aoff[A_SLOTS], boff[B_SLOTS];
#pragma unroll
  for (int i = 0; i < A_SLOTS; ++i) {
    const int row = 8 * (wave + NW * i) + (lane >> 3);
    int v = v0 + row;
    if (v > HW - 1) v = HW - 1;
    aoff[i] = v * (int)p.lda0 + ((lane & 7) ^ ((row >> 1) & 7)) * EPC;
  }
#pragma unroll
  for (int i = 0; i < B_SLOTS; ++i) {
    const int row = 8 * (wave + NW * i) + (lane >> 3);
    int n = n0 + row;
    if (n > p.Npad - 1) n = p.Npad - 1;
    boff[i] = n * p.Kc + ((lane & 7) ^ ((row >> 1) & 7)) * EPC;
  }
  const int nslab = p.Kc / BK;
  int s0 = 0, s1 = nslab;
  if (p.splitk > 1) {
    const int per = (nslab + p.splitk - 1) / p.splitk;
    s0 = bz * per;
    s1 = s0 + per < nslab ? s0 + per : nslab;
  }

  f32x16_t acc[MI][NI];
#pragma unroll
  for (int mi = 0; mi < MI; ++mi)
#pragma unroll
    for (int ni = 0; ni < NI; ++ni)
#pragma unroll
      for (int r = 0; r < 16; ++r) acc[mi][ni][r] = 0.f;

  const unsigned lds0 = __builtin_amdgcn_readfirstlane((unsigned)(size_t)(__attribute__((address_space(3))) char*)smem);
#define K22_ISSUE_G(SLAB, STAGE)                                                                           \
  {                                                                                                        \
    int sl_ = (SLAB);                                                                                      \
    if (sl_ > s1 - 1) sl_ = s1 - 1;       \
    const unsigned d_ = lds0 + (STAGE) * BUF + wave * 1024;                                                \
    _Pragma("unroll") for (int i = 0; i < A_SLOTS; ++i)                                                    \
        glds16_asm(A + aoff[i] + sl_ * BK, __builtin_amdgcn_readfirstlane(d_ + i * NW * 1024));            \
    _Pragma("unroll") for (int i = 0; i < B_SLOTS; ++i)                                                    \
        glds16w_asm(Wp + boff[i] + sl_ * BK, __builtin_amdgcn_readfirstlane(d_ + A_BYTES + i * NW * 1024)); \
  }
  int arow[MI], brow[NI];
#pragma unroll
  for (int mi = 0; mi < MI; ++mi) arow[mi] = (wm * (BM / WM) + mi * 32 + l31) * 128;
#pragma unroll
  for (int ni = 0; ni < NI; ++ni) brow[ni] = A_BYTES + (wn * (BN / WN) + ni * 32 + l31) * 128;
  const int sw = (l31 >> 1) & 7;

  if (s0 < s1) {
#pragma unroll
    for (int t = 0; t < NST - 1; ++t) K22_ISSUE_G(s0 + t, t);
    int cur = 0, fill = NST - 1;
    for (int s = s0; s < s1; ++s) {
      wait_vmcnt<(NST - 2) * CH>();
      raw_barrier();
      K22_ISSUE_G(s + NST - 1, fill);
      const char* St = smem + cur * BUF;
#pragma unroll
      for (int ks = 0; ks < KSTEPS; ++ks) {
        FragA<T> a[MI];
        Frag<T> b[NI];
#pragma unroll
        for (int mi = 0; mi < MI; ++mi) ld_frag_at_a<ARAW, T>(a[mi], St + arow[mi], sw, ks, h);
#pragma unroll
        for (int ni = 0; ni < NI; ++ni) ld_frag_at(b[ni], St + brow[ni], sw, ks, h);
#pragma unroll
        for (int mi = 0; mi < MI; ++mi)
#pragma unroll
          for (int ni = 0; ni < NI; ++ni) mma_atom(acc[mi][ni], b[ni], a[mi]);
      }
      cur = (cur + 1 == NST) ? 0 : cur + 1;
      fill = (fill + 1 == NST) ? 0 : fill + 1;
    }
  }
#undef K22_ISSUE_G
  halo_tail<T, BM, true>(p, acc, smem, bx, bz, img, v0, n0);
}

template <typename T, int BM, int NST>
__global__ __launch_bounds__(512) void gemm8_spec_kernel(const IgemmParams p) {
  using TR = TT<T>;
  static_assert(sizeof(T) == 2, "gemm8_spec_kernel: 16-bit operands");
  constexpr int BK = TR::BK, EPC = TR::EPC, KSTEPS = TR::KSTEPS;
  static_assert(KSTEPS % 2 == 0, "two-set fragment pipeline");
  constexpr int BN = HALO_BN, NWL = 4, WM = 2, WN = 2;
  constexpr int MI = BM / (WM * 32), NI = BN / (WN * 32);
  constexpr int A_SLOTS = BM / 8 / NWL, B_SLOTS = BN / 8 / NWL, CH = A_SLOTS + B_SLOTS;
  constexpr int A_BYTES = BM * 128, B_BYTES = BN * 128, BUF = A_BYTES + B_BYTES;
  constexpr int GM = 8;
  extern __shared__ __attribute__((aligned(16))) char smem[];

  const int tid = threadIdx.x, lane = tid & 63;
  const int wave = __builtin_amdgcn_readfirstlane(tid >> 6);
  const bool producer = wave >= 4;
  const int h = lane >> 5, l31 = lane & 31;

  const int HW = p.H > 0 ? p.H * p.W : p.M;
  const int TPI = (HW + BM - 1) / BM;
  const int B = p.M / HW;
  const int gx = B * TPI, gy = (p.N + BN - 1) / BN;
  int L = p.xcd_remap ? xcd_remap_h(blockIdx.x, gridDim.x) : (int)blockIdx.x;
  const int per_z = gx * gy;
  const int bz = L / per_z;
  L -= bz * per_z;
  const int grp = L / (GM * gy);
  const int first_m = grp * GM;
  const int gsz = gx - first_m < GM ? gx - first_m : GM;
  const int lin = L - grp * GM * gy;
  const int bx = first_m + lin % gsz, by = lin / gsz;
  const int img = bx / TPI, v0 = (bx - img * TPI) * BM;
  const int n0 = by * BN;

  const int nslab = p.Kc / BK;
  int s0 = 0, s1 = nslab;
  if (p.splitk > 1) {
    const int per = (nslab + p.splitk - 1) / p.splitk;
    s0 = bz * per;
    s1 = s0 + per < nslab ? s0 + per : nslab;
  }

  f32x16_t acc[MI][NI];
#pragma unroll
  for (int mi = 0; mi < MI; ++mi)
#pragma unroll
    for (int ni = 0; ni < NI; ++ni)
#pragma unroll
      for (int r = 0; r < 16; ++r) acc[mi][ni][r] = 0.f;

  if (s0 < s1) {
    if (producer) {
      const int lw = wave - 4;
      const T* __restrict__ A = reinterpret_cast<const T*>(p.A0) + (int64_t)img * HW * p.lda0;
      const T* __restrict__ Wp = reinterpret_cast<const T*>(p.Wp);
      int aoff[A_SLOTS], boff[B_SLOTS];
#pragma unroll
      for (int i = 0; i < A_SLOTS; ++i) {
        const int row = 8 * (lw + NWL * i) + (lane >> 3);
        int v = v0 + row;
        if (v > HW - 1) v = HW - 1;
        aoff[i] = v * (int)p.lda0 + ((lane & 7) ^ ((row >> 1) & 7)) * EPC;
      }
#pragma unroll
      for (int i = 0; i < B_SLOTS; ++i) {
        const int row = 8 * (lw + NWL * i) + (lane >> 3);
        int n = n0 + row;
        if (n > p.Npad - 1) n = p.Npad - 1;
        boff[i] = n * p.Kc + ((lane & 7) ^ ((row >> 1) & 7)) * EPC;
      }
      const unsigned lds0 = __builtin_amdgcn_readfirstlane((unsigned)(size_t)(__attribute__((address_space(3))) char*)smem);
#define K22_ISSUE_GS(SLAB, STAGE)                                                                          \
      {                                                                                                    \
        int sl_ = (SLAB);                                                                                  \
        if (sl_ > s1 - 1) sl_ = s1 - 1;    \
        const unsigned d_ = lds0 + (STAGE) * BUF + lw * 1024;                                              \
        _Pragma("unroll") for (int i = 0; i < A_SLOTS; ++i)                                                \
            glds16_asm(A + aoff[i] + sl_ * BK, __builtin_amdgcn_readfirstlane(d_ + i * NWL * 1024));       \
        _Pragma("unroll") for (int i = 0; i < B_SLOTS; ++i)                                                \
            glds16w_asm(Wp + boff[i] + sl_ * BK, __builtin_amdgcn_readfirstlane(d_ + A_BYTES + i * NWL * 1024)); \
      }
#pragma unroll
      for (int t = 0; t < NST - 1; ++t) K22_ISSUE_GS(s0 + t, t);
      int fill = NST - 1;
      for (int s = s0; s < s1; ++s) {
        wait_vmcnt<(NST - 2) * CH>();
        raw_barrier();
        K22_ISSUE_GS(s + NST - 1, fill);
        fill = (fill + 1 == NST) ? 0 : fill + 1;
      }
#undef K22_ISSUE_GS
    } else {
      const int wm = wave >> 1, wn = wave & 1;
      int arow[MI], brow[NI];
#pragma unroll
      for (int mi = 0; mi < MI; ++mi) arow[mi] = (wm * (BM / WM) + mi * 32 + l31) * 128;
#pragma unroll
      for (int ni = 0; ni < NI; ++ni) brow[ni] = A_BYTES + (wn * (BN / WN) + ni * 32 + l31) * 128;
      const int sw = (l31 >> 1) & 7;
      Frag<T> pa[MI], pb[NI];
#pragma unroll
      for (int mi = 0; mi < MI; ++mi) pa[mi] = Frag<T>{};
#pragma unroll
      for (int ni = 0; ni < NI; ++ni) pb[ni] = Frag<T>{};
      constexpr int NRD = MI + NI, NMF = MI * NI, MPR = NMF / NRD;
#define K22_GS_INTERLEAVE()                                                                                \
      {                                                                                                    \
        _Pragma("unroll") for (int i_ = 0; i_ < NRD; ++i_) {                                               \
          __builtin_amdgcn_sched_group_barrier(0x008, MPR, 0);                                             \
          __builtin_amdgcn_sched_group_barrier(0x100, 1, 0);                                               \
        }                                                                                                  \
        if constexpr (NMF - MPR * NRD > 0) __builtin_amdgcn_sched_group_barrier(0x008, NMF - MPR * NRD, 0); \
        __builtin_amdgcn_sched_barrier(0);                                                                 \
      }
      int cur = 0;
      for (int s = s0; s < s1; ++s) {
        raw_barrier();
        const char* St = smem + cur * BUF;
        Frag<T> ca[MI], cb[NI];
#pragma unroll
        for (int ks = 0; ks < KSTEPS; ks += 2) {
#pragma unroll
          for (int mi = 0; mi < MI; ++mi) ld_frag_at(ca[mi], St + arow[mi], sw, ks, h);
#pragma unroll
          for (int ni = 0; ni < NI; ++ni) ld_frag_at(cb[ni], St + brow[ni], sw, ks, h);
#pragma unroll
          for (int mi = 0; mi < MI; ++mi)
#pragma unroll
            for (int ni = 0; ni < NI; ++ni) mma_atom(acc[mi][ni], pb[ni], pa[mi]);
          K22_GS_INTERLEAVE();
#pragma unroll
          for (int mi = 0; mi < MI; ++mi) ld_frag_at(pa[mi], St + arow[mi], sw, ks + 1, h);
#pragma unroll
          for (int ni = 0; ni < NI; ++ni) ld_frag_at(pb[ni], St + brow[ni], sw, ks + 1, h);
#pragma unroll
          for (int mi = 0; mi < MI; ++mi)
#pragma unroll
            for (int ni = 0; ni < NI; ++ni) mma_atom(acc[mi][ni], cb[ni], ca[mi]);
          K22_GS_INTERLEAVE();
        }
        asm volatile("s_waitcnt lgkmcnt(0)" ::: "memory");
        cur = (cur + 1 == NST) ? 0 : cur + 1;
      }
#undef K22_GS_INTERLEAVE
#pragma unroll
      for (int mi = 0; mi < MI; ++mi)
#pragma unroll
        for (int ni = 0; ni < NI; ++ni) mma_atom(acc[mi][ni], pb[ni], pa[mi]);
    }
  }
  halo_tail<T, BM, true, true>(p, acc, smem, bx, bz, img, v0, n0);
}

namespace {
__device__ __forceinline__ void ld_frag64(Frag<bf16_t>& f, const char* rowp, int sw, int ks, int h) {
  f.v = *reinterpret_cast<const u32x4_t*>(rowp + (((2 * ks + h) ^ sw) << 4));
}
__device__ __forceinline__ void ld_frag64(Frag<f16_t>& f, const char* rowp, int sw, int ks, int h) {
  f.v = *reinterpret_cast<const u32x4_t*>(rowp + (((2 * ks + h) ^ sw) << 4));
}
__device__ __forceinline__ void ld_frag64(Frag<float>& f, const char* rowp, int sw, int , int h) {
  const float4 a = *reinterpret_cast<const float4*>(rowp + (((2 * h) ^ sw) << 4));
  const float4 b = *reinterpret_cast<const float4*>(rowp + (((2 * h + 1) ^ sw) << 4));
  f.v[0] = a.x; f.v[1] = a.y; f.v[2] = a.z; f.v[3] = a.w;
  f.v[4] = b.x; f.v[5] = b.y; f.v[6] = b.z; f.v[7] = b.w;
}
template <int RB> constexpr int halo3_wait(int ky) { return RB == 2 ? 0 : (RB == 3 ? (ky == 0 ? 3 : 6) : (ky == 0 ? 6 : (ky == 1 ? 9 : 12))); }
constexpr int HALO3_ASLOTS = 6;
}

template <typename T, int BM, int RB>
__global__ __launch_bounds__(512) void conv3_halo3_kernel(const IgemmParams p) {
  constexpr int EPH = 64 / (int)sizeof(T);
  constexpr int EPC = TT<T>::EPC;
  constexpr int KS_U = EPH / 16;
  constexpr int BN = HALO_BN, NW = HALO_NW, WM = 4, WN = 2;
  constexpr int MI = BM / (WM * 32), NI = BN / (WN * 32);
  constexpr int BT_BYTES = 3 * BN * 64;
  constexpr int GM = 8;
  extern __shared__ __attribute__((aligned(16))) char smem[];

  const int tid = threadIdx.x, lane = tid & 63;
  const int wave = __builtin_amdgcn_readfirstlane(tid >> 6);
  const int wm = wave >> 1, wn = wave & 1;
  const int h = lane >> 5, l31 = lane & 31;

  const int W2 = p.W + 2;
  const int VR = p.H * W2;
  const int TPI = (VR + BM - 1) / BM;
  const int HR16 = (BM + 2 * W2 + 2 + 15) & ~15;
  const int NPA = HR16 >> 4;
  const int A_BYTES = HR16 * 64;
  const int PR_MAX = (p.H + 2) * W2 - 1;
  const int B = p.M / (p.H * p.W);

  const int gx = B * TPI, gy = (p.N + BN - 1) / BN;
  int L = p.xcd_remap ? xcd_remap_h(blockIdx.x, gridDim.x) : (int)blockIdx.x;
  const int per_z = gx * gy;
  const int bz = L / per_z;
  L -= bz * per_z;
  const int grp = L / (GM * gy);
  const int first_m = grp * GM;
  const int gsz = gx - first_m < GM ? gx - first_m : GM;
  const int lin = L - grp * GM * gy;
  const int bx = first_m + lin % gsz, by = lin / gsz;
  const int img = bx / TPI, v0 = (bx - img * TPI) * BM;
  const int n0 = by * BN;

  const T* __restrict__ Aimg = reinterpret_cast<const T*>(p.A0) + (int64_t)img * (p.H + 2) * W2 * p.Kc;
  const T* __restrict__ Wp = reinterpret_cast<const T*>(p.Wp);

  int aoff[HALO3_ASLOTS];
#pragma unroll
  for (int q = 0; q < HALO3_ASLOTS; ++q) {
    int j = q * NW + wave;
    if (j > NPA - 1) j = NPA - 1;
    const int hr = 16 * j + (lane >> 2);
    int pr = v0 + hr;
    if (pr > PR_MAX) pr = PR_MAX;
    aoff[q] = pr * p.Kc + ((lane & 3) ^ ((hr >> 2) & 3)) * EPC;
  }
  int boff;
  {
    const int row = 16 * wave + (lane >> 2);
    int n = n0 + row;
    if (n > p.Npad - 1) n = p.Npad - 1;
    boff = n * 9 * p.Kc + ((lane & 3) ^ ((row >> 2) & 3)) * EPC;
  }
  const int nhs = p.Kc / EPH;
  int h0 = 0, h1 = nhs;
  if (p.splitk > 1) {
    const int per = (nhs + p.splitk - 1) / p.splitk;
    h0 = bz * per;
    h1 = h0 + per < nhs ? h0 + per : nhs;
// ... 5 lines not shown
#pragma unroll
    for (int ni = 0; ni < NI; ++ni)
#pragma unroll
      for (int r = 0; r < 16; ++r) acc[mi][ni][r] = 0.f;

  char* const Bring = smem + 2 * A_BYTES;
  const int abase = wm * (BM / WM) + l31;
  int brow[NI];
#pragma unroll
  for (int ni = 0; ni < NI; ++ni) brow[ni] = (wn * (BN / WN) + ni * 32 + l31) * 64;
  const int bsw = (l31 >> 2) & 3;

#define K22_ISSUE_A3(Q, HS, DST)                                                                           \
  {                                                                                                        \
    int j_ = (Q) * NW + wave;                                                                              \
    if (j_ > NPA - 1) j_ = NPA - 1;                                                                        \
    __builtin_amdgcn_global_load_lds((const __attribute__((address_space(1))) void*)(Aimg + aoff[Q] + (HS) * EPH), \
                                     (__attribute__((address_space(3))) void*)((DST) + j_ * 1024), 16, 0, 0); \
  }
#define K22_ISSUE_B3(HS, KY, SLOT)                                                                         \
  {                                                                                                        \
    const int kofs_ = (KY) * 3 * p.Kc + (HS) * EPH;                                                        \
    char* dst_ = Bring + (SLOT) * BT_BYTES + wave * 1024;                                                  \
    _Pragma("unroll") for (int kx = 0; kx < 3; ++kx)                                                       \
        __builtin_amdgcn_global_load_lds((const __attribute__((address_space(1))) void*)(Wp + boff + kofs_ + kx * p.Kc), \
                                         (__attribute__((address_space(3))) void*)(dst_ + kx * BN * 64), 16, 0, 0); \
  }

  if (h0 < h1) {
#pragma unroll
    for (int q = 0; q < HALO3_ASLOTS; ++q) K22_ISSUE_A3(q, h0, smem);
#pragma unroll
    for (int j = 0; j < RB - 1; ++j) {
      const int hs_ = h0 + j / 3 < h1 ? h0 + j / 3 : h1 - 1;
      K22_ISSUE_B3(hs_, j % 3, j);
    }
    int cur = 0, fill = RB - 1;
    for (int hs = h0; hs < h1; ++hs) {
      char* const Acur = smem + ((hs - h0) & 1) * A_BYTES;
      char* const Anext = smem + (((hs - h0) & 1) ^ 1) * A_BYTES;
      const int hn = hs + 1 < h1 ? hs + 1 : h1 - 1;
#define K22_IT3(KY)                                                                                        \
      {                                                                                                    \
        wait_vmcnt<halo3_wait<RB>(KY)>();                                                                  \
        raw_barrier();                                                                      \
        if constexpr ((KY) < 2) {                                                                          \
          K22_ISSUE_A3(3 * ((KY) < 2 ? (KY) : 0) + 0, hn, Anext);                                          \
          K22_ISSUE_A3(3 * ((KY) < 2 ? (KY) : 0) + 1, hn, Anext);                                          \
          K22_ISSUE_A3(3 * ((KY) < 2 ? (KY) : 0) + 2, hn, Anext);                                          \
        }                                                                                                  \
        {                                                                                                  \
          constexpr int kya_ = ((KY) + RB - 1) % 3;                                                        \
          int hsa_ = hs + ((KY) + RB - 1) / 3;                                                             \
          if (hsa_ > h1 - 1) hsa_ = h1 - 1;                                                                \
          K22_ISSUE_B3(hsa_, kya_, fill);                                                                  \
        }                                                                                                  \
        const char* Bcur = Bring + cur * BT_BYTES;                                                         \
        _Pragma("unroll") for (int kx = 0; kx < 3; ++kx) {                                                 \
          const int shift = (KY) * W2 + kx;                                                                \
          const char* arow[MI];                                                                            \
          int asw[MI];                                                                                     \
          _Pragma("unroll") for (int mi = 0; mi < MI; ++mi) {                                              \
            const int ar = abase + mi * 32 + shift;                                                        \
            arow[mi] = Acur + ar * 64;                                                                     \
            asw[mi] = (ar >> 2) & 3;                                                                       \
          }                                                                                                \
          _Pragma("unroll") for (int ks = 0; ks < KS_U; ++ks) {                                            \
            Frag<T> a[MI], b[NI];                                                                          \
            _Pragma("unroll") for (int mi = 0; mi < MI; ++mi) ld_frag64(a[mi], arow[mi], asw[mi], ks, h);  \
            _Pragma("unroll") for (int ni = 0; ni < NI; ++ni) ld_frag64(b[ni], Bcur + kx * BN * 64 + brow[ni], bsw, ks, h); \
            _Pragma("unroll") for (int mi = 0; mi < MI; ++mi)                                              \
              _Pragma("unroll") for (int ni = 0; ni < NI; ++ni) mma_atom(acc[mi][ni], b[ni], a[mi]);       \
          }                                                                                                \
        }                                                                                                  \
        cur = (cur + 1 == RB) ? 0 : cur + 1;                                                               \
        fill = (fill + 1 == RB) ? 0 : fill + 1;                                                            \
      }
      K22_IT3(0) K22_IT3(1) K22_IT3(2)
#undef K22_IT3
    }
  }
#undef K22_ISSUE_A3
#undef K22_ISSUE_B3
  halo_tail<T, BM>(p, acc, smem, bx, bz, img, v0, n0);
}

static int halo3_rows(const IgemmParams& p, int bm) { return (bm + 2 * (p.W + 2) + 2 + 15) & ~15; }
static size_t halo3_smem_bytes(const IgemmParams& p, int bm, int rb) {
  const size_t main_loop = (size_t)2 * halo3_rows(p, bm) * 64 + (size_t)rb * 3 * HALO_BN * 64;
  const size_t epi = (size_t)bm * (HALO_BN * 4 + 16);
  const size_t skip = p.S0 ? (size_t)(bm == 256 ? 3 : 4) * (bm * 128 + HALO_BN * 128) : 0;
  size_t m = main_loop > epi ? main_loop : epi;
  return m > skip ? m : skip;
}
static int halo3_pick_rb(const IgemmParams& p, int bm) {
  if (halo3_rows(p, bm) / 16 > HALO3_ASLOTS * HALO_NW) return 0;
  for (int rb : {4, 3, 2})
    if (halo3_smem_bytes(p, bm, rb) <= 160 * 1024) return rb;
  return 0;
}

static int gemm8_nst(int bm, int stages) { return bm == 256 ? 3 : (stages == 2 ? 2 : 4); }
static size_t gemm8_smem_bytes(int bm, int nst) {
  const size_t main_loop = (size_t)nst * (bm + HALO_BN) * 128;
  const size_t epi = (size_t)bm * (HALO_BN * 4 + 16);
  return main_loop > epi ? main_loop : epi;
}
int gemm8_tiles_per_image(const IgemmParams& p, int bm) { return ((p.H > 0 ? p.H * p.W : p.M) + bm - 1) / bm; }

bool gemm8_supported(const IgemmParams& p, int dtype, int bm) {
  const int BK = k22_bk(dtype);
  if (p.taps != 1 || (bm != 256 && bm != 128) || p.N < 128) return false;
  if (p.K0 != p.Kc || p.S0 != nullptr || p.res_f32) return false;
  if (p.out_mode != IG_OUT_ROWMAJOR && p.out_mode != IG_OUT_ROWMAJOR_F32 && p.out_mode != IG_OUT_QKV) return false;
  if (p.N % 8 || p.ldo % 8 || (p.residual && p.ldr % 8) || p.Kc % BK || p.lda0 % 8) return false;
  const int hw = p.H > 0 ? p.H * p.W : p.M;
  if (hw <= 0 || p.M % hw) return false;
  if (p.out_mode == IG_OUT_QKV && (p.att_T != hw || p.N % 384)) return false;
  if ((int64_t)p.M * p.lda0 >= (1ll << 31) || (int64_t)p.Npad * p.Kc >= (1ll << 31)) return false;
  return true;
}

template <typename T, int BM, int NST, bool ARAW = false>
static int launch_gemm8_cfg(const IgemmParams& p, int splitk, hipStream_t stream) {
  if constexpr (is_x3<T>::value && !ARAW) { if (p.a_raw) return launch_gemm8_cfg<T, BM, NST, true>(p, splitk, stream); }
  const size_t smem = gemm8_smem_bytes(BM, NST);
  static LdsAttrGuard attr_guard;
  if (int rc_ = k22_ensure_lds_attr(attr_guard, reinterpret_cast<const void*>(&gemm8_kernel<T, BM, NST, ARAW>), 160 * 1024, __FILE__, __LINE__)) return rc_;
  IgemmParams q = p;
  q.splitk = splitk;
  const int hw = p.H > 0 ? p.H * p.W : p.M;
  const int nblocks = (p.M / hw) * gemm8_tiles_per_image(p, BM) * ((p.N + HALO_BN - 1) / HALO_BN) * splitk;
  hipLaunchKernelGGL((gemm8_kernel<T, BM, NST, ARAW>), dim3(nblocks), dim3(512), smem, stream, q);
  K22_CHECK_LAUNCH();
  return K22_OK;
}

template <typename T, int BM, int NST>
static int launch_gemm8_spec_cfg(const IgemmParams& p, int splitk, hipStream_t stream) {
  const size_t smem = gemm8_smem_bytes(BM, NST);
  static LdsAttrGuard attr_guard;
  if (int rc_ = k22_ensure_lds_attr(attr_guard, reinterpret_cast<const void*>(&gemm8_spec_kernel<T, BM, NST>), 160 * 1024, __FILE__, __LINE__)) return rc_;
  IgemmParams q = p;
  q.splitk = splitk;
  const int hw = p.H > 0 ? p.H * p.W : p.M;
  const int nblocks = (p.M / hw) * gemm8_tiles_per_image(p, BM) * ((p.N + HALO_BN - 1) / HALO_BN) * splitk;
  hipLaunchKernelGGL((gemm8_spec_kernel<T, BM, NST>), dim3(nblocks), dim3(512), smem, stream, q);
  K22_CHECK_LAUNCH();
  return K22_OK;
}

bool gemm8_spec_supported(int dtype) { return dtype == K22_BF16 || dtype == K22_F16; }

int launch_gemm8(const IgemmParams& p, int dtype, int bm, int splitk, hipStream_t stream) {
  if (!gemm8_supported(p, dtype, bm)) return k22_set_error(K22_EINVAL, "gemm8: unsupported problem");
  if ((p.stages == 3 || p.stages == 4) && gemm8_spec_supported(dtype)) {
    if (p.stages == 4 && bm == 128) return dtype == K22_BF16 ? launch_gemm8_spec_cfg<bf16_t, 128, 2>(p, splitk, stream) : launch_gemm8_spec_cfg<f16_t, 128, 2>(p, splitk, stream);
    if (dtype == K22_BF16) return bm == 256 ? launch_gemm8_spec_cfg<bf16_t, 256, 3>(p, splitk, stream) : launch_gemm8_spec_cfg<bf16_t, 128, 4>(p, splitk, stream);
    return bm == 256 ? launch_gemm8_spec_cfg<f16_t, 256, 3>(p, splitk, stream) : launch_gemm8_spec_cfg<f16_t, 128, 4>(p, splitk, stream);
  }
  const int nst = gemm8_nst(bm, p.stages);
  if (dtype == K22_BF16) {
    if (bm == 256) return launch_gemm8_cfg<bf16_t, 256, 3>(p, splitk, stream);
    return nst == 2 ? launch_gemm8_cfg<bf16_t, 128, 2>(p, splitk, stream) : launch_gemm8_cfg<bf16_t, 128, 4>(p, splitk, stream);
  }
  if (dtype == K22_F16) {
    if (bm == 256) return launch_gemm8_cfg<f16_t, 256, 3>(p, splitk, stream);
    return nst == 2 ? launch_gemm8_cfg<f16_t, 128, 2>(p, splitk, stream) : launch_gemm8_cfg<f16_t, 128, 4>(p, splitk, stream);
  }
  if (dtype == K22_F16X3) {
    if (bm == 256) return launch_gemm8_cfg<x3_t, 256, 3>(p, splitk, stream);
    return nst == 2 ? launch_gemm8_cfg<x3_t, 128, 2>(p, splitk, stream) : launch_gemm8_cfg<x3_t, 128, 4>(p, splitk, stream);
  }
  if (dtype == K22_F16X2) {
    if (bm == 256) return launch_gemm8_cfg<x2_t, 256, 3>(p, splitk, stream);
    return nst == 2 ? launch_gemm8_cfg<x2_t, 128, 2>(p, splitk, stream) : launch_gemm8_cfg<x2_t, 128, 4>(p, splitk, stream);
  }
  if (bm == 256) return launch_gemm8_cfg<float, 256, 3>(p, splitk, stream);
  return nst == 2 ? launch_gemm8_cfg<float, 128, 2>(p, splitk, stream) : launch_gemm8_cfg<float, 128, 4>(p, splitk, stream);
}

bool conv3_halo_supported(const IgemmParams& p, int dtype, int bm) {
  const int BK = k22_bk(dtype);
  if (p.taps != 9 || (bm != 256 && bm != 128)) return false;
  if (k22_is_split(dtype) && (p.a_raw || p.algo == 3)) return false;
  if (p.gn_coeff != nullptr) {
    if (!conv3_algo_fuses_gn(p.algo) || !p.gn_x0 || p.gn_C0 <= 0 || p.gn_C0 > p.Kc || p.gn_C0 % BK || (p.gn_C0 < p.Kc && !p.gn_x1)) return false;
    if ((int64_t)p.H * p.W * p.Kc >= (1ll << 31)) return false;
  }
  if (p.out_mode != IG_OUT_ROWMAJOR && p.out_mode != IG_OUT_ROWMAJOR_F32) return false;
  if (p.N % 8 || p.ldo % 8 || (p.residual && p.ldr % 8) || p.Kc % BK) return false;
  if (p.H <= 0 || p.W <= 0 || p.M % (p.H * p.W)) return false;
  if (p.S0 != nullptr) {
    if (!p.Ws || p.SK0 % BK || p.SK1 % BK || (p.SK1 > 0 && !p.S1) || p.SK0 <= 0) return false;
    if ((int64_t)p.M * (p.SK0 > p.SK1 ? p.SK0 : p.SK1) >= (1ll << 31) || (int64_t)p.Npad * (p.SK0 + p.SK1) >= (1ll << 31)) return false;
  }
  if ((p.algo == 3 ? halo3_pick_rb(p, bm) : halo_pick_nbst(p, bm)) == 0) return false;
  if ((int64_t)(p.H + 2) * (p.W + 2) * p.Kc >= (1ll << 31) || (int64_t)p.Npad * 9 * p.Kc >= (1ll << 31)) return false;
  return true;
}

int conv3_halo_tiles_per_image(const IgemmParams& p, int bm) { return (p.H * (p.W + 2) + bm - 1) / bm; }

template <typename T, int BM, int NBST, int LW, int MODE>
static int launch_halo_cfg(const IgemmParams& p, int splitk, hipStream_t stream) {
  const size_t smem = halo_smem_bytes(p, BM, NBST);
  static LdsAttrGuard attr_guard;
  if (int rc_ = k22_ensure_lds_attr(attr_guard, reinterpret_cast<const void*>(&conv3_halo_kernel<T, BM, NBST, false, LW, MODE>), 160 * 1024, __FILE__, __LINE__)) return rc_;
  IgemmParams q = p;
  q.splitk = splitk;
  const int B = p.M / (p.H * p.W);
  const int nblocks = B * conv3_halo_tiles_per_image(p, BM) * ((p.N + HALO_BN - 1) / HALO_BN) * splitk;
  hipLaunchKernelGGL((conv3_halo_kernel<T, BM, NBST, false, LW, MODE>), dim3(nblocks), dim3(512), smem, stream, q);
  K22_CHECK_LAUNCH();
  return K22_OK;
}

template <typename T, int BM, int LW, int MODE>
static int launch_halo_nbst(const IgemmParams& p, int nbst, int splitk, hipStream_t stream) {
  if (nbst == 2) return launch_halo_cfg<T, BM, 2, LW, MODE>(p, splitk, stream);
  if (nbst == 3) return launch_halo_cfg<T, BM, 3, LW, MODE>(p, splitk, stream);
  if (nbst <= 5) return launch_halo_cfg<T, BM, 4, LW, MODE>(p, splitk, stream);
  return launch_halo_cfg<T, BM, 6, LW, MODE>(p, splitk, stream);
}

template <typename T, int BM, int RB>
static int launch_halo3_cfg(const IgemmParams& p, int splitk, hipStream_t stream) {
  const size_t smem = halo3_smem_bytes(p, BM, RB);
  static LdsAttrGuard attr_guard;
  if (int rc_ = k22_ensure_lds_attr(attr_guard, reinterpret_cast<const void*>(&conv3_halo3_kernel<T, BM, RB>), 160 * 1024, __FILE__, __LINE__)) return rc_;
  IgemmParams q = p;
  q.splitk = splitk;
  const int B = p.M / (p.H * p.W);
  const int nblocks = B * conv3_halo_tiles_per_image(p, BM) * ((p.N + HALO_BN - 1) / HALO_BN) * splitk;
  hipLaunchKernelGGL((conv3_halo3_kernel<T, BM, RB>), dim3(nblocks), dim3(512), smem, stream, q);
  K22_CHECK_LAUNCH();
  return K22_OK;
}
template <typename T, int BM>
static int launch_halo3_rb(const IgemmParams& p, int rb, int splitk, hipStream_t stream) {
  if (rb == 2) return launch_halo3_cfg<T, BM, 2>(p, splitk, stream);
  if (rb == 3) return launch_halo3_cfg<T, BM, 3>(p, splitk, stream);
  return launch_halo3_cfg<T, BM, 4>(p, splitk, stream);
}

int launch_conv3_halo_trace(const IgemmParams& p, int dtype, hipStream_t stream) {
  if (dtype != K22_BF16 || !conv3_halo_supported(p, dtype, 256) || p.trace == nullptr) return k22_set_error(K22_EINVAL, "conv3_halo_trace: bf16, BM = 256 only");
  const int nbst = halo_pick_nbst(p, 256) >= 4 ? 4 : 2;
  const size_t smem = halo_smem_bytes(p, 256, nbst);
  IgemmParams q = p;
  q.splitk = 1; q.xcd_remap = 1;
  const int B = p.M / (p.H * p.W);
  const int nblocks = B * conv3_halo_tiles_per_image(p, 256) * ((p.N + HALO_BN - 1) / HALO_BN);
  if (nbst == 4) {
    (void)hipFuncSetAttribute(reinterpret_cast<const void*>(&conv3_halo_kernel<bf16_t, 256, 4, true>), hipFuncAttributeMaxDynamicSharedMemorySize, 160 * 1024);
    hipLaunchKernelGGL((conv3_halo_kernel<bf16_t, 256, 4, true>), dim3(nblocks), dim3(512), smem, stream, q);
  } else {
    (void)hipFuncSetAttribute(reinterpret_cast<const void*>(&conv3_halo_kernel<bf16_t, 256, 2, true>), hipFuncAttributeMaxDynamicSharedMemorySize, 160 * 1024);
    hipLaunchKernelGGL((conv3_halo_kernel<bf16_t, 256, 2, true>), dim3(nblocks), dim3(512), smem, stream, q);
  }
  K22_CHECK_LAUNCH();
  return K22_OK;
}
// ... 50 lines not shown
```

kandinsky-2_amd/csrc/conv3_spec.hip:

```cpp
#include "conv3_common.h"

template <typename T, int BM, int NBST, bool PIPE = false, int DBG = 0>
__global__ __launch_bounds__(512) void conv3_halo_spec_kernel(const IgemmParams p) {
  using TR = TT<T>;
  constexpr int BK = TR::BK, EPC = TR::EPC, KSTEPS = TR::KSTEPS;
  constexpr int BN = HALO_BN, NWL = 4, WM = 2, WN = 2;
  constexpr int MI = BM / (WM * 32), NI = BN / (WN * 32);
  constexpr int B_SLOTS = BN / 8 / NWL;
  constexpr int B_BYTES = BN * 128;
  constexpr int APT = 2;
  constexpr int A_SLOTS = (10 - NBST) * APT;
  constexpr int GM = 8;
  extern __shared__ __attribute__((aligned(16))) char smem[];

  const int tid = threadIdx.x, lane = tid & 63;
  const int wave = __builtin_amdgcn_readfirstlane(tid >> 6);
  const bool producer = wave >= 4;
  const int h = lane >> 5, l31 = lane & 31;

  const int W2 = p.W + 2;
  const int VR = p.H * W2;
  const int TPI = (VR + BM - 1) / BM;
  const int HRp = (BM + 2 * W2 + 2 + 7) & ~7;
  const int NP = HRp >> 3;
  const int A_BYTES = HRp * 128;
  const int PR_MAX = (p.H + 2) * W2 - 1;
  const int B = p.M / (p.H * p.W);

  const int gx = B * TPI, gy = (p.N + BN - 1) / BN;
  int L = p.xcd_remap ? xcd_remap_h(blockIdx.x, gridDim.x) : (int)blockIdx.x;
  const int per_z = gx * gy;
  const int bz = L / per_z;
  L -= bz * per_z;
  const int grp = L / (GM * gy);
  const int first_m = grp * GM;
  const int gsz = gx - first_m < GM ? gx - first_m : GM;
  const int lin = L - grp * GM * gy;
  const int bx = first_m + lin % gsz, by = lin / gsz;
  const int img = bx / TPI, v0 = (bx - img * TPI) * BM;
  const int n0 = by * BN;

  const int nslab = p.Kc / BK;
  int s0 = 0, s1 = nslab;
  if (p.splitk > 1) {
    const int per = (nslab + p.splitk - 1) / p.splitk;
    s0 = bz * per;
    s1 = s0 + per < nslab ? s0 + per : nslab;
  }

  f32x16_t acc[MI][NI];
#pragma unroll
  for (int mi = 0; mi < MI; ++mi)
#pragma unroll
    for (int ni = 0; ni < NI; ++ni)
#pragma unroll
      for (int r = 0; r < 16; ++r) acc[mi][ni][r] = 0.f;

  char* const Bst = smem + 2 * A_BYTES;
  if (s0 < s1) {
    if (producer && p.gn_coeff != nullptr) {
      const int lw = wave - 4;
      constexpr int NCF = EPC / 2;
      const T* __restrict__ X0 = reinterpret_cast<const T*>(p.gn_x0) + (int64_t)img * p.H * p.W * p.gn_C0;
      const int C1 = p.Kc - p.gn_C0;
      const T* __restrict__ X1 = p.gn_x1 ? reinterpret_cast<const T*>(p.gn_x1) + (int64_t)img * p.H * p.W * C1 : nullptr;
      const T* __restrict__ Wp = reinterpret_cast<const T*>(p.Wp);
      const int gchunk = (lane & 7) ^ ((4 * (lw & 1) + (lane >> 4)) & 7);
      const float* __restrict__ cfbase = p.gn_coeff + ((int64_t)img * p.Kc + gchunk * EPC) * 2;
      int pix[A_SLOTS];
      unsigned bmask = 0;
#pragma unroll
      for (int q = 0; q < A_SLOTS; ++q) {
        int j = q * NWL + lw;
        if (j > NP - 1) j = NP - 1;
        const int hr = 8 * j + (lane >> 3);
        int pr = v0 + hr;
        if (pr > PR_MAX) pr = PR_MAX;
        const int y = pr / W2, x = pr - y * W2;
        const bool border = y < 1 || y > p.H || x < 1 || x > p.W;
        const int yy = y < 1 ? 0 : (y > p.H ? p.H - 1 : y - 1), xx = x < 1 ? 0 : (x > p.W ? p.W - 1 : x - 1);
        pix[q] = yy * p.W + xx;
        bmask |= (border ? 1u : 0u) << q;
      }
      int boff[B_SLOTS];
#pragma unroll
      for (int i = 0; i < B_SLOTS; ++i) {
        const int row = 8 * (lw + NWL * i) + (lane >> 3);
        int n = n0 + row;
        if (n > p.Npad - 1) n = p.Npad - 1;
        boff[i] = n * 9 * p.Kc + ((lane & 7) ^ ((row >> 1) & 7)) * EPC;
      }
      const unsigned lds0 = __builtin_amdgcn_readfirstlane((unsigned)(size_t)(__attribute__((address_space(3))) char*)smem);
      const unsigned lds_scratch = lds0 + 2 * A_BYTES + NBST * B_BYTES;
      u32x4_t cfr[NCF];
#pragma unroll
      for (int k = 0; k < NCF; ++k) cfr[k] = u32x4_t{0u, 0u, 0u, 0u};
#define K22_GN_A(Q, SLAB, DSTOFF)                                                                          \
// ... 47 lines not shown
#pragma unroll
      for (int q = 0; q < A_SLOTS; ++q) K22_GN_REWRITE(q, 0);
      asm volatile("s_waitcnt lgkmcnt(0)" ::: "memory");
      int fill = NBST - 1;
      for (int s = s0; s < s1; ++s) {
        const int anext_off = (((s - s0) & 1) ^ 1) * A_BYTES;
        const int sn = s + 1 < s1 ? s + 1 : s1 - 1;
        const bool more = s + 1 < s1;
#define K22_GN_PTAP(TAP)                                                                                   \
        {                                                                                                  \
          wait_vmcnt<B_SLOTS * (NBST - 2) + APT * halo_count_a<NBST>(TAP)>();                              \
          raw_barrier();                                                                                   \
          if constexpr ((TAP) == 0) { if (more) K22_GN_COEF(sn); }                                         \
          constexpr int ta_ = ((TAP) + NBST - 1) % 9;                                                      \
          const int sa_ = ((TAP) + NBST - 1 >= 9) ? sn : s;                                                \
          K22_GN_B(sa_, ta_, fill);                                                                        \
          if constexpr ((TAP) <= 9 - NBST) {                                                               \
            _Pragma("unroll") for (int a_i = 0; a_i < APT; ++a_i) {                                        \
              constexpr int qb_ = ((TAP) <= 9 - NBST ? (TAP) : 0) * APT;                                   \
              K22_GN_A(qb_ + a_i, sn, anext_off);                                                          \
            }                                                                                              \
          }                                                                                                \
                                  \
          if constexpr ((TAP) >= 1 && (TAP) - 1 <= 9 - NBST) {                                             \
            if (more) {                                                                                    \
              gn_wait<B_SLOTS + ((TAP) <= 9 - NBST ? APT : 0)>(cfr);                                       \
              _Pragma("unroll") for (int a_i = 0; a_i < APT; ++a_i) {                                      \
                constexpr int qr_ = ((TAP) >= 1 ? (TAP) - 1 : 0) * APT;                                    \
                K22_GN_REWRITE(qr_ + a_i, anext_off);                                                      \
              }                                                                                            \
              asm volatile("s_waitcnt lgkmcnt(0)" ::: "memory");                                           \
            }                                                                                              \
          }                                                                                                \
          fill = (fill + 1 == NBST) ? 0 : fill + 1;                                                        \
        }
        K22_GN_PTAP(0) K22_GN_PTAP(1) K22_GN_PTAP(2) K22_GN_PTAP(3) K22_GN_PTAP(4) K22_GN_PTAP(5) K22_GN_PTAP(6) K22_GN_PTAP(7) K22_GN_PTAP(8)
#undef K22_GN_PTAP
      }
#undef K22_GN_A
#undef K22_GN_B
#undef K22_GN_COEF
#undef K22_GN_REWRITE
    } else if (producer) {
      const int lw = wave - 4;
      const T* __restrict__ Aimg = reinterpret_cast<const T*>(p.A0) + (int64_t)img * (p.H + 2) * W2 * p.Kc;
      const T* __restrict__ Wp = reinterpret_cast<const T*>(p.Wp);
      int aoff[A_SLOTS];
#pragma unroll
      for (int q = 0; q < A_SLOTS; ++q) {
        int j = q * NWL + lw;
        if (j > NP - 1) j = NP - 1;
        const int hr = 8 * j + (lane >> 3);
        int pr = v0 + hr;
        if (pr > PR_MAX) pr = PR_MAX;
        aoff[q] = pr * p.Kc + ((lane & 7) ^ ((hr >> 1) & 7)) * EPC;
      }
      int boff[B_SLOTS];
#pragma unroll
      for (int i = 0; i < B_SLOTS; ++i) {
        const int row = 8 * (lw + NWL * i) + (lane >> 3);
        int n = n0 + row;
        if (n > p.Npad - 1) n = p.Npad - 1;
        boff[i] = n * 9 * p.Kc + ((lane & 7) ^ ((row >> 1) & 7)) * EPC;
      }
      const unsigned lds0 = __builtin_amdgcn_readfirstlane((unsigned)(size_t)(__attribute__((address_space(3))) char*)smem);
#define K22_SP_A(Q, SLAB, DSTOFF)                                                                          \
      {                                                                                                    \
        int j_ = (Q) * NWL + lw;                                                                           \
        if (j_ > NP - 1) j_ = NP - 1;                                                                      \
        glds16_asm(Aimg + aoff[Q] + (SLAB) * BK, __builtin_amdgcn_readfirstlane(lds0 + (unsigned)(DSTOFF) + j_ * 1024)); \
      }
#define K22_SP_B(SLAB, TAP, STAGE)                                                                         \
      {                                                                                                    \
        const int kofs_ = (TAP) * p.Kc + (SLAB) * BK;                                                      \
        const unsigned d_ = lds0 + 2 * A_BYTES + (STAGE) * B_BYTES + lw * 1024;                            \
        _Pragma("unroll") for (int i = 0; i < B_SLOTS; ++i)                                                \
            glds16w_asm(Wp + boff[i] + kofs_, __builtin_amdgcn_readfirstlane(d_ + i * NWL * 1024));         \
      }
#pragma unroll
      for (int q = 0; q < A_SLOTS; ++q) K22_SP_A(q, s0, 0);
#pragma unroll
      for (int t = 0; t < NBST - 1; ++t) K22_SP_B(s0, t, t);
      int fill = NBST - 1;
      for (int s = s0; s < s1; ++s) {
        const int anext_off = (((s - s0) & 1) ^ 1) * A_BYTES;
        const int sn = s + 1 < s1 ? s + 1 : s1 - 1;
#define K22_SP_PTAP(TAP)                                                                                   \
        {                                                                                                  \
          if constexpr (DBG == 0) wait_vmcnt<B_SLOTS * (NBST - 2) + APT * halo_count_a<NBST>(TAP)>();      \
          raw_barrier();                                                                                   \
          constexpr int ta_ = ((TAP) + NBST - 1) % 9;                                                      \
          const int sa_ = ((TAP) + NBST - 1 >= 9) ? sn : s;                                                \
          if constexpr (DBG != 1) K22_SP_B(sa_, ta_, fill);                                                \
          if constexpr ((TAP) <= 9 - NBST && DBG != 1) {                                                   \
            _Pragma("unroll") for (int a_ = 0; a_ < APT; ++a_) {                                           \
              constexpr int qb_ = ((TAP) <= 9 - NBST ? (TAP) : 0) * APT;                                   \
              K22_SP_A(qb_ + a_, sn, anext_off);                                                           \
            }                                                                                              \
          }                                                                                                \
          fill = (fill + 1 == NBST) ? 0 : fill + 1;                                                        \
        }
        K22_SP_PTAP(0) K22_SP_PTAP(1) K22_SP_PTAP(2) K22_SP_PTAP(3) K22_SP_PTAP(4) K22_SP_PTAP(5) K22_SP_PTAP(6) K22_SP_PTAP(7) K22_SP_PTAP(8)
#undef K22_SP_PTAP
      }
#undef K22_SP_A
#undef K22_SP_B
    } else {
      const int wm = wave >> 1, wn = wave & 1;
      const int abase = wm * (BM / WM) + l31;
      int brow[NI];
#pragma unroll
      for (int ni = 0; ni < NI; ++ni) brow[ni] = (wn * (BN / WN) + ni * 32 + l31) * 128;
      const int bsw = (l31 >> 1) & 7;
      int cur = 0;
      FragA<T> pa[MI];
      Frag<T> pb[NI];
      if constexpr (PIPE) {
#pragma unroll
        for (int mi = 0; mi < MI; ++mi) pa[mi] = FragA<T>{};
#pragma unroll
        for (int ni = 0; ni < NI; ++ni) pb[ni] = Frag<T>{};
      }
      constexpr int NRD = is_x2<T>::value ? MI + 2 * NI : (MI + NI) * FragCost<T>::READS;
      constexpr int NMF = MI * NI * FragCost<T>::MFMAS;
      constexpr int MPR = NMF / NRD;
#define K22_SP_INTERLEAVE()                                                                                \
      {                                                                                                    \
        _Pragma("unroll") for (int i_ = 0; i_ < NRD; ++i_) {                                               \
          __builtin_amdgcn_sched_group_barrier(0x008, MPR, 0);                                             \
          __builtin_amdgcn_sched_group_barrier(0x100, 1, 0);                                               \
        }                                                                                                  \
        if constexpr (NMF - MPR * NRD > 0) __builtin_amdgcn_sched_group_barrier(0x008, NMF - MPR * NRD, 0); \
        __builtin_amdgcn_sched_barrier(0);                                                                 \
      }
      for (int s = s0; s < s1; ++s) {
        const char* const Acur = smem + ((s - s0) & 1) * A_BYTES;
#define K22_SP_CTAP(TAP)                                                                                   \
        {                                                                                                  \
          raw_barrier();                                                                                   \
          const char* Bcur = Bst + cur * B_BYTES;                                                          \
          const int shift = ((TAP) / 3) * W2 + ((TAP) % 3);                                                \
          const char* arow[MI];                                                                            \
          int asw[MI];                                                                                     \
          _Pragma("unroll") for (int mi = 0; mi < MI; ++mi) {                                              \
            const int ar = abase + mi * 32 + shift;                                                        \
            arow[mi] = Acur + ar * 128;                                                                    \
            asw[mi] = (ar >> 1) & 7;                                                                       \
          }                                                                                                \
          if constexpr (PIPE) {                                                                            \
            FragA<T> ca[MI];                                                                               \
            Frag<T> cb[NI];                                                                                \
            _Pragma("unroll") for (int ks = 0; ks < KSTEPS; ks += 2) {                                     \
              _Pragma("unroll") for (int mi = 0; mi < MI; ++mi) ld_frag_at(ca[mi], arow[mi], asw[mi], ks, h); \
              _Pragma("unroll") for (int ni = 0; ni < NI; ++ni) ld_frag_at(cb[ni], Bcur + brow[ni], bsw, ks, h); \
              _Pragma("unroll") for (int mi = 0; mi < MI; ++mi)                                            \
                _Pragma("unroll") for (int ni = 0; ni < NI; ++ni) mma_atom(acc[mi][ni], pb[ni], pa[mi]);   \
              K22_SP_INTERLEAVE();                                                                         \
              _Pragma("unroll") for (int mi = 0; mi < MI; ++mi) ld_frag_at(pa[mi], arow[mi], asw[mi], ks + 1, h); \
              _Pragma("unroll") for (int ni = 0; ni < NI; ++ni) ld_frag_at(pb[ni], Bcur + brow[ni], bsw, ks + 1, h); \
              _Pragma("unroll") for (int mi = 0; mi < MI; ++mi)                                            \
                _Pragma("unroll") for (int ni = 0; ni < NI; ++ni) mma_atom(acc[mi][ni], cb[ni], ca[mi]);   \
              K22_SP_INTERLEAVE();                                                                         \
            }                                                                                              \
          } else {                                                                                         \
          _Pragma("unroll") for (int ks = 0; ks < KSTEPS; ++ks) {                                          \
            FragA<T> a[MI];                                                                                \
            Frag<T> b[NI];                                                                                 \
            _Pragma("unroll") for (int mi = 0; mi < MI; ++mi) ld_frag_at(a[mi], arow[mi], asw[mi], ks, h); \
            _Pragma("unroll") for (int ni = 0; ni < NI; ++ni) ld_frag_at(b[ni], Bcur + brow[ni], bsw, ks, h); \
            _Pragma("unroll") for (int mi = 0; mi < MI; ++mi)                                              \
              _Pragma("unroll") for (int ni = 0; ni < NI; ++ni) mma_atom(acc[mi][ni], b[ni], a[mi]);       \
          }                                                                                                \
          }                                                                                                \
            \
          asm volatile("s_waitcnt lgkmcnt(0)" ::: "memory");                                               \
          cur = (cur + 1 == NBST) ? 0 : cur + 1;                                                           \
        }
        K22_SP_CTAP(0) K22_SP_CTAP(1) K22_SP_CTAP(2) K22_SP_CTAP(3) K22_SP_CTAP(4) K22_SP_CTAP(5) K22_SP_CTAP(6) K22_SP_CTAP(7) K22_SP_CTAP(8)
#undef K22_SP_CTAP
      }
#undef K22_SP_INTERLEAVE
      if constexpr (PIPE) {
#pragma unroll
        for (int mi = 0; mi < MI; ++mi)
#pragma unroll
          for (int ni = 0; ni < NI; ++ni) mma_atom(acc[mi][ni], pb[ni], pa[mi]);
      }
    }
  }
  halo_tail<T, BM, false, true>(p, acc, smem, bx, bz, img, v0, n0);
}


template <typename T, int BM, int NBST, bool PIPE, int DBG = 0>
static int launch_halo_spec_cfg(const IgemmParams& p, int splitk, hipStream_t stream) {
  const size_t smem = halo_smem_bytes(p, BM, NBST);
  static LdsAttrGuard attr_guard;
  if (int rc_ = k22_ensure_lds_attr(attr_guard, reinterpret_cast<const void*>(&conv3_halo_spec_kernel<T, BM, NBST, PIPE, DBG>), 160 * 1024, __FILE__, __LINE__)) return rc_;
  IgemmParams q = p;
  q.splitk = splitk;
  const int B = p.M / (p.H * p.W);
  const int nblocks = B * conv3_halo_tiles_per_image(p, BM) * ((p.N + HALO_BN - 1) / HALO_BN) * splitk;
  hipLaunchKernelGGL((conv3_halo_spec_kernel<T, BM, NBST, PIPE, DBG>), dim3(nblocks), dim3(512), smem, stream, q);
  K22_CHECK_LAUNCH();
  return K22_OK;
}
template <typename T, int BM, bool PIPE>
static int launch_halo_spec_nbst(const IgemmParams& p, int nbst, int splitk, hipStream_t stream) {
  if (nbst == 2) return launch_halo_spec_cfg<T, BM, 2, PIPE>(p, splitk, stream);
  if (nbst == 3) return launch_halo_spec_cfg<T, BM, 3, PIPE>(p, splitk, stream);
  if (nbst <= 5) return launch_halo_spec_cfg<T, BM, 4, PIPE>(p, splitk, stream);
  return launch_halo_spec_cfg<T, BM, 6, PIPE>(p, splitk, stream);
}

int launch_conv3_halo_spec(const IgemmParams& p, int dtype, int bm, int nbst, int splitk, hipStream_t stream) {
  const bool pipe = p.algo == 12;
  if (dtype == K22_F16X2) {
    if (!pipe) return bm == 256 ? launch_halo_spec_nbst<x2_t, 256, false>(p, nbst, splitk, stream) : launch_halo_spec_nbst<x2_t, 128, false>(p, nbst, splitk, stream);
    return bm == 256 ? launch_halo_spec_nbst<x2_t, 256, true>(p, nbst, splitk, stream) : launch_halo_spec_nbst<x2_t, 128, true>(p, nbst, splitk, stream);
  }
  if (dtype == K22_F16X3) {
    if (!pipe) return bm == 256 ? launch_halo_spec_nbst<x3_t, 256, false>(p, nbst, splitk, stream) : launch_halo_spec_nbst<x3_t, 128, false>(p, nbst, splitk, stream);
    return bm == 256 ? launch_halo_spec_nbst<x3_t, 256, false>(p, nbst, splitk, stream) : launch_halo_spec_nbst<x3_t, 128, true>(p, nbst, splitk, stream);
  }
  if (!pipe) {
    if (dtype == K22_BF16) return bm == 256 ? launch_halo_spec_nbst<bf16_t, 256, false>(p, nbst, splitk, stream) : launch_halo_spec_nbst<bf16_t, 128, false>(p, nbst, splitk, stream);
    else if (dtype == K22_F16) return bm == 256 ? launch_halo_spec_nbst<f16_t, 256, false>(p, nbst, splitk, stream) : launch_halo_spec_nbst<f16_t, 128, false>(p, nbst, splitk, stream);
    return bm == 256 ? launch_halo_spec_nbst<float, 256, false>(p, nbst, splitk, stream) : launch_halo_spec_nbst<float, 128, false>(p, nbst, splitk, stream);
  }
  if (dtype == K22_BF16) return bm == 256 ? launch_halo_spec_nbst<bf16_t, 256, true>(p, nbst, splitk, stream) : launch_halo_spec_nbst<bf16_t, 128, true>(p, nbst, splitk, stream);
  else if (dtype == K22_F16) return bm == 256 ? launch_halo_spec_nbst<f16_t, 256, true>(p, nbst, splitk, stream) : launch_halo_spec_nbst<f16_t, 128, true>(p, nbst, splitk, stream);
  return bm == 256 ? launch_halo_spec_nbst<float, 256, false>(p, nbst, splitk, stream) : launch_halo_spec_nbst<float, 128, true>(p, nbst, splitk, stream);
}
#ifdef K22_DEBUG_VARIANTS
int launch_conv3_halo_spec_debug(const IgemmParams& p, int nbst, int splitk, hipStream_t stream) {
  if (p.algo == 13) return nbst == 2 ? launch_halo_spec_cfg<bf16_t, 256, 2, true, 1>(p, splitk, stream) : launch_halo_spec_cfg<bf16_t, 256, 4, true, 1>(p, splitk, stream);
  return nbst == 2 ? launch_halo_spec_cfg<bf16_t, 256, 2, true, 2>(p, splitk, stream) : launch_halo_spec_cfg<bf16_t, 256, 4, true, 2>(p, splitk, stream);
}
#endif
```

kandinsky-2_amd/csrc/igemm.hip:

```cpp
#include "kernels.h"
#include <stdlib.h>

template <int N> __device__ __forceinline__ void wait_vmcnt() { asm volatile("s_waitcnt vmcnt(%0)" ::"n"(N) : "memory"); }

template <typename T> __device__ __forceinline__ void store4(T* dst, const float* v);
template <> __device__ __forceinline__ void store4<bf16_t>(bf16_t* dst, const float* v) {
  uint2 w;
  w.x = pack2_bf16(v[0], v[1]);
  w.y = pack2_bf16(v[2], v[3]);
  *reinterpret_cast<uint2*>(dst) = w;
}
template <> __device__ __forceinline__ void store4<f16_t>(f16_t* dst, const float* v) {
  uint2 w;
  w.x = pack2_f16(v[0], v[1]);
  w.y = pack2_f16(v[2], v[3]);
  *reinterpret_cast<uint2*>(dst) = w;
}
template <> __device__ __forceinline__ void store4<float>(float* dst, const float* v) {
  *reinterpret_cast<float4*>(dst) = make_float4(v[0], v[1], v[2], v[3]);
}
template <> __device__ __forceinline__ void store4<x3_t>(x3_t* dst, const float* v) { store4<float>(reinterpret_cast<float*>(dst), v); }
template <> __device__ __forceinline__ void store4<x2_t>(x2_t* dst, const float* v) { store4<float>(reinterpret_cast<float*>(dst), v); }
template <typename T> __device__ __forceinline__ void load4f(const T* src, float* v);
template <> __device__ __forceinline__ void load4f<bf16_t>(const bf16_t* src, float* v) {
  const uint2 r = *reinterpret_cast<const uint2*>(src);
  v[0] = __uint_as_float(r.x << 16); v[1] = __uint_as_float(r.x & 0xffff0000u);
  v[2] = __uint_as_float(r.y << 16); v[3] = __uint_as_float(r.y & 0xffff0000u);
}
template <> __device__ __forceinline__ void load4f<f16_t>(const f16_t* src, float* v) {
  const uint2 r = *reinterpret_cast<const uint2*>(src);
  unpack2_f16(r.x, v[0], v[1]); unpack2_f16(r.y, v[2], v[3]);
}
template <> __device__ __forceinline__ void load4f<float>(const float* src, float* v) {
  const float4 r = *reinterpret_cast<const float4*>(src);
  v[0] = r.x; v[1] = r.y; v[2] = r.z; v[3] = r.w;
}

template <> __device__ __forceinline__ void load4f<x3_t>(const x3_t* src, float* v) { load4f<float>(reinterpret_cast<const float*>(src), v); }
template <> __device__ __forceinline__ void load4f<x2_t>(const x2_t* src, float* v) { load4f<float>(reinterpret_cast<const float*>(src), v); }

__device__ __forceinline__ int xcd_remap(int bid, int nblocks) {
  const int q = nblocks >> 3, r = nblocks & 7, x = bid & 7;
  return (x < r ? x * (q + 1) : r * (q + 1) + (x - r) * q) + (bid >> 3);
}

template <typename T, int BM, int BN, int STAGES, bool ARAW = false>
__global__ __launch_bounds__(256) void igemm_kernel(const IgemmParams p) {
  using TR = TT<T>;
  constexpr int BK = TR::BK, EPC = TR::EPC, KSTEPS = TR::KSTEPS;
  constexpr int MI = BM / 64, NI = BN / 64;
  constexpr int A_CH = BM / 32, B_CH = BN / 32, CH = A_CH + B_CH;
  constexpr int A_BYTES = BM * 128, B_BYTES = BN * 128, BUF = A_BYTES + B_BYTES;
  constexpr int GM = 8;
  extern __shared__ __attribute__((aligned(16))) char smem[];

  const int tid = threadIdx.x, lane = tid & 63;
  const int wave = __builtin_amdgcn_readfirstlane(tid >> 6);
  const int wm = wave >> 1, wn = wave & 1;

  const int gx = (p.M + BM - 1) / BM, gy = (p.N + BN - 1) / BN;
  int L = p.xcd_remap ? xcd_remap(blockIdx.x, gridDim.x) : (int)blockIdx.x;
  const int per_z = gx * gy;
  const int bz = L / per_z;
  L -= bz * per_z;
  const int grp = L / (GM * gy);
  const int first_m = grp * GM;
  const int gsz = gx - first_m < GM ? gx - first_m : GM;
  const int lin = L - grp * GM * gy;
  const int bx = first_m + lin % gsz, by = lin / gsz;
  const int m0 = bx * BM, n0 = by * BN;

  const bool conv = (p.taps == 9);
  const T* __restrict__ A0 = reinterpret_cast<const T*>(p.A0);
  const T* __restrict__ A1 = reinterpret_cast<const T*>(p.A1);
  const T* __restrict__ Wp = reinterpret_cast<const T*>(p.Wp);

  const int lrow = tid >> 3, lpos = tid & 7;
  const int lchunk = lpos ^ ((lrow >> 1) & 7);
  int64_t aoff0[A_CH], aoff1[A_CH], boff[B_CH];
  const int ldb = p.taps * p.Kc;
#pragma unroll
  for (int i = 0; i < A_CH; ++i) {
    int m = m0 + lrow + 32 * i;
    if (m > p.M - 1) m = p.M - 1;
    if (conv) {
      const int hw = p.H * p.W;
      const int b = m / hw, rem = m - b * hw;
      const int y = rem / p.W, x = rem - y * p.W;
      aoff0[i] = ((int64_t)(b * (p.H + 2) + y) * (p.W + 2) + x) * p.Kc;
      aoff1[i] = 0;
    } else {
      aoff0[i] = (int64_t)m * p.lda0;
      aoff1[i] = (int64_t)m * p.lda1;
    }
  }
#pragma unroll
  for (int i = 0; i < B_CH; ++i) {
    int n = n0 + lrow + 32 * i;
    if (n > p.Npad - 1) n = p.Npad - 1;
    boff[i] = (int64_t)n * ldb;
  }
  const int kt_per_tap = p.Kc / BK;
  const int nkt = p.taps * kt_per_tap;
  int kt0 = 0, kt1 = nkt;
  if (p.splitk > 1) {
    const int per = (nkt + p.splitk - 1) / p.splitk;
    kt0 = bz * per;
    kt1 = kt0 + per < nkt ? kt0 + per : nkt;
  }

  f32x16_t acc[MI][NI];
#pragma unroll
  for (int mi = 0; mi < MI; ++mi)
#pragma unroll
    for (int ni = 0; ni < NI; ++ni)
#pragma unroll
      for (int r = 0; r < 16; ++r) acc[mi][ni][r] = 0.f;
  const int h = lane >> 5, l31 = lane & 31;
  const int64_t lck = lchunk * EPC;
  const int wave_row0 = wave * 8;

#define K22_ISSUE(KT, BUFI)                                                                              \
  {                                                                                                      \
    int kt_ = (KT);                                                                                      \
    if (kt_ > kt1 - 1) kt_ = kt1 - 1;  \
    const int tap_ = kt_ / kt_per_tap;                                                                   \
    const int k0_ = (kt_ - tap_ * kt_per_tap) * BK;                                                      \
    const bool second_ = (!conv) && (k0_ >= p.K0);                                                       \
    const T* src_ = second_ ? A1 : A0;                                                                   \
    const int ty_ = tap_ / 3, tx_ = tap_ - ty_ * 3;                                                      \
    const int64_t add_ = (conv ? (int64_t)(ty_ * (p.W + 2) + tx_) * p.Kc + k0_ : (int64_t)(second_ ? k0_ - p.K0 : k0_)) + lck; \
    char* As_ = smem + (BUFI) * BUF + wave_row0 * 128;                                                   \
    _Pragma("unroll") for (int i = 0; i < A_CH; ++i)                                                     \
        __builtin_amdgcn_global_load_lds((const __attribute__((address_space(1))) void*)(src_ + (second_ ? aoff1[i] : aoff0[i]) + add_), \
                                         (__attribute__((address_space(3))) void*)(As_ + i * 4096), 16, 0, 0); \
    const int64_t badd_ = (int64_t)tap_ * p.Kc + k0_ + lck;                                              \
    char* Bs_ = As_ + A_BYTES;                                                                           \
    _Pragma("unroll") for (int i = 0; i < B_CH; ++i)                                                     \
        __builtin_amdgcn_global_load_lds((const __attribute__((address_space(1))) void*)(Wp + boff[i] + badd_), \
                                         (__attribute__((address_space(3))) void*)(Bs_ + i * 4096), 16, 0, 0); \
  }

  if (kt0 < kt1) {
#pragma unroll
    for (int s_ = 0; s_ < STAGES - 1; ++s_) K22_ISSUE(kt0 + s_, s_);
    int cur = 0, fill = STAGES - 1;
    for (int kt = kt0; kt < kt1; ++kt) {
      wait_vmcnt<(STAGES - 2) * CH>();
      raw_barrier();
      K22_ISSUE(kt + STAGES - 1, fill);
      {
        const char* As = smem + cur * BUF;
        const char* Bs = As + A_BYTES;
#pragma unroll
        for (int ks = 0; ks < KSTEPS; ++ks) {
          FragA<T> a[MI];
          Frag<T> b[NI];
#pragma unroll
          for (int mi = 0; mi < MI; ++mi) ld_frag_a<ARAW, T>(a[mi], As, wm * (BM / 2) + mi * 32 + l31, ks, h);
#pragma unroll
          for (int ni = 0; ni < NI; ++ni) ld_frag(b[ni], Bs, wn * (BN / 2) + ni * 32 + l31, ks, h);
#pragma unroll
          for (int mi = 0; mi < MI; ++mi)
#pragma unroll
            for (int ni = 0; ni < NI; ++ni) mma_atom(acc[mi][ni], b[ni], a[mi]);
        }
      }
      cur = (cur + 1 == STAGES) ? 0 : cur + 1;
      fill = (fill + 1 == STAGES) ? 0 : fill + 1;
    }
    wait_vmcnt<0>();
  }
#undef K22_ISSUE

  const int mbase = m0 + wm * (BM / 2), nbase = n0 + wn * (BN / 2);
  const bool vec_ok = ((p.N & 3) == 0) && ((p.ldo & 3) == 0) && ((p.ldr & 3) == 0);
  const T* __restrict__ res = reinterpret_cast<const T*>(p.residual);
  float* part = p.splitk > 1 ? p.partial + (int64_t)bz * p.M * p.N : nullptr;
#pragma unroll
  for (int mi = 0; mi < MI; ++mi) {
    const int m = mbase + mi * 32 + l31;
    if (m >= p.M) continue;
    int64_t nchw_base = 0;
    if (p.out_mode == IG_OUT_NCHW_F32) {
      const int hw = p.H * p.W;
      const int b = m / hw, rem = m - b * hw;
      nchw_base = (int64_t)b * p.N * hw + rem;
    }
#pragma unroll
    for (int ni = 0; ni < NI; ++ni)
#pragma unroll
      for (int j = 0; j < 4; ++j) {
        const int n = nbase + ni * 32 + 8 * j + 4 * h;
        if (n >= p.N) continue;
        float v[4];
#pragma unroll
        for (int e = 0; e < 4; ++e) v[e] = acc_unscale<T>(acc[mi][ni][4 * j + e]);
        if (part != nullptr) {
          if (vec_ok) {
            *reinterpret_cast<float4*>(part + (int64_t)m * p.N + n) = make_float4(v[0], v[1], v[2], v[3]);
          } else {
#pragma unroll
            for (int e = 0; e < 4; ++e)
              if (n + e < p.N) part[(int64_t)m * p.N + n + e] = v[e];
          }
          continue;
        }
        if (vec_ok) {
          if (p.bias != nullptr) {
            const float4 bv = *reinterpret_cast<const float4*>(p.bias + n);
            v[0] += bv.x; v[1] += bv.y; v[2] += bv.z; v[3] += bv.w;
          }
          if (res != nullptr) {
            float rv[4];
            if (p.res_f32) load4f<float>(reinterpret_cast<const float*>(p.residual) + (int64_t)m * p.ldr + n, rv);
            else load4f<T>(res + (int64_t)m * p.ldr + n, rv);
#pragma unroll
            for (int e = 0; e < 4; ++e) v[e] += rv[e];
          }
#pragma unroll
          for (int e = 0; e < 4; ++e) v[e] = apply_act(v[e], p.act);
          if (p.out_mode == IG_OUT_ROWMAJOR) {
            store4<T>(reinterpret_cast<T*>(p.out) + (int64_t)m * p.ldo + n, v);
          } else if (p.out_mode == IG_OUT_ROWMAJOR_F32) {
            store4<float>(reinterpret_cast<float*>(p.out) + (int64_t)m * p.ldo + n, v);
          } else if (p.out_mode == IG_OUT_QKV) {
            const int C = p.N / 3, heads = C >> 6;
            const int which = n / C, c = n - which * C;
            const int head = c >> 6, d = c & 63;
            const int b = m / p.att_T, t = m - b * p.att_T;
            if (which == 0) {
              store4<T>(reinterpret_cast<T*>(p.out) + (int64_t)m * p.ldo + c, v);
            } else if (which == 1) {
              store4<T>(reinterpret_cast<T*>(p.kall) + ((int64_t)(b * heads + head) * p.att_Tkp + p.att_S + t) * 64 + d, v);
            } else {
              T* vt = reinterpret_cast<T*>(p.vtall) + ((int64_t)(b * heads + head) * 64 + d) * p.att_Tkp + p.att_S + t;
#pragma unroll
              for (int e = 0; e < 4; ++e) vt[(int64_t)e * p.att_Tkp] = from_f32<T>(v[e]);
            }
          } else {
            const int64_t hw = (int64_t)p.H * p.W;
#pragma unroll
            for (int e = 0; e < 4; ++e) reinterpret_cast<float*>(p.out)[nchw_base + (int64_t)(n + e) * hw] = v[e];
          }
        } else {
#pragma unroll
          for (int e = 0; e < 4; ++e) {
            if (n + e >= p.N) continue;
            float u = v[e];
            if (p.bias != nullptr) u += p.bias[n + e];
            if (res != nullptr) u += p.res_f32 ? reinterpret_cast<const float*>(p.residual)[(int64_t)m * p.ldr + n + e] : to_f32(res[(int64_t)m * p.ldr + n + e]);
            u = apply_act(u, p.act);
            if (p.out_mode == IG_OUT_ROWMAJOR) {
              reinterpret_cast<T*>(p.out)[(int64_t)m * p.ldo + n + e] = from_f32<T>(u);
// ... 425 lines not shown
```

kandinsky-2_amd/csrc/kernels.h:

```cpp
#pragma once
#include "common.h"

#include <atomic>

#define K22_OK 0
#define K22_EINVAL (-1)
#define K22_EHIP (-2)
#define K22_ENOMEM (-3)

struct LdsAttrGuard { std::atomic<unsigned long long> done{0}; };
inline int k22_ensure_lds_attr(LdsAttrGuard& g, const void* fn, int bytes, const char* file, int line) {
  int dev = 0;
  (void)hipGetDevice(&dev);
  const unsigned long long bit = 1ull << (dev & 63);
  if (g.done.load(std::memory_order_acquire) & bit) return K22_OK;
  const hipError_t e = hipFuncSetAttribute(fn, hipFuncAttributeMaxDynamicSharedMemorySize, bytes);
  if (e != hipSuccess) return k22_set_error_hip(e, file, line);
  g.done.fetch_or(bit, std::memory_order_release);
  return K22_OK;
}

enum IgemmOut { IG_OUT_ROWMAJOR = 0,
                IG_OUT_ROWMAJOR_F32 = 1,
                IG_OUT_NCHW_F32 = 2,
                IG_OUT_QKV = 3 };

struct IgemmParams {
  const void* A0;
  const void* A1;
  const void* Wp;
  const float* bias;
  const void* residual;
  void* out;
  float* partial;
  int M, N, Npad;
  int Kc;
  int K0;
  int taps;
  int H, W;
  long lda0, lda1;
  int ldo, ldr;
  int out_mode;
  int act;
  int splitk;
  int force_bm, force_bn;
  int stages;
  int xcd_remap;
  int algo;
  const void* S0; const void* S1; const void* Ws; const float* bias2;
  int SK0, SK1;
  void* kall; void* vtall;
  int att_T, att_S, att_Tkp;
  unsigned long long* trace;
  int res_f32;
  float* stats;
  const void* Wfrag; const void* Wsfrag;
  int a_raw;
  const float* gn_coeff; const void* gn_x0; const void* gn_x1; int gn_C0, gn_act;
  unsigned long long* st_trace;
  int st_tm, st_rb, st_mtiles, st_buf;
};

struct IgemmStatsInfo { int rows_per_image; };
int igemm_stats_rows_per_image(const IgemmParams& p, int dtype);

int launch_igemm(const IgemmParams& p, int dtype, hipStream_t stream);
bool conv3_halo_supported(const IgemmParams& p, int dtype, int bm);
inline bool conv3_algo_fuses_gn(int algo) { return algo == 11 || algo == 12; }
int conv3_halo_tiles_per_image(const IgemmParams& p, int bm);
int launch_conv3_halo(const IgemmParams& p, int dtype, int bm, int splitk, hipStream_t stream);
int launch_conv3_halo_trace(const IgemmParams& p, int dtype, hipStream_t stream);
bool gemm8_supported(const IgemmParams& p, int dtype, int bm);
bool gemm8_spec_supported(int dtype);
int gemm8_tiles_per_image(const IgemmParams& p, int bm);
int launch_gemm8(const IgemmParams& p, int dtype, int bm, int splitk, hipStream_t stream);
bool stream_supported(const IgemmParams& p, int dtype, int mb);
int stream_mtiles(const IgemmParams& p, int mb);
int launch_stream(const IgemmParams& p, int dtype, int mb, int splitk, hipStream_t stream);
long stream_launch_count();
long loop_capture_count();
long loop_launch_count();
size_t stream_frag_bytes(int Npad, int taps, int Kc, int dtype);
int launch_stream_repack(const void* W, void* out, int Npad, int taps, int Kc, int dtype, hipStream_t stream);
void igemm_set_gemm_algo(int v);
void igemm_set_conv_algo(int v);
void igemm_set_default_stages(int v);
void igemm_set_xcd_remap(int v);
void attention_set_pipe(int v);
int igemm_choose_splitk(const IgemmParams& p, int dtype);
```

Before: 141.0 steps/s.

## Drain load rings with counted waits and prefetch residual/bias before epilogue

The multi-stage global-to-LDS rings in the igemm, skip-GEMM and spec conv3 kernels no longer re-issue clamped duplicate loads on the final iterations. Instead the tail iterations use compile-time-verified counted vmcnt waits that shrink as the ring drains, with static_asserts checking the schedule. The halo epilogue now loads residual and bias vectors before the accumulator LDS staging barrier, so their latency overlaps the staging. Debug-only timestamp tracing and a ring-depth query API are added, at the cost of more code paths and waits that depend on the verified issue schedule being exact.

```diff
diff --git a/include/k22.h b/include/k22.h
--- a/include/k22.h
+++ b/include/k22.h
@@ -141,6 +141,7 @@
 } K22IgemmOperands;
 int k22_igemm_cfg_accepted(const K22IgemmProblem* pr);
 int k22_igemm_cfg(const K22IgemmProblem* pr, const K22IgemmOperands* ops, int* rows_per_image, void* stream);
+int k22_conv3_halo_ring_depth(int H, int W, int bm, int fused_skip);
 int k22_debug_conv_trace(const void* x_padded, const void* Wp, const float* bias, void* out, int B, int H, int W, int Cin, int Cout,
                          int Npad, unsigned long long* trace, void* stream);
 int k22_conv3x3_gn(const void* x0, const void* x1, int C0, int C1, const float* gamma, const float* beta, const float* film, long film_ld,
diff --git a/kandinsky-2_amd/_lib.py b/kandinsky-2_amd/_lib.py
--- a/kandinsky-2_amd/_lib.py
+++ b/kandinsky-2_amd/_lib.py
@@ -133,6 +133,7 @@
     "k22_igemm_cfg_accepted": (_I, [C.POINTER(K22IgemmProblem)]),
     "k22_igemm_cfg": (_I, [C.POINTER(K22IgemmProblem), C.POINTER(K22IgemmOperands), C.POINTER(_I), _P]),
     "k22_conv3x3_gn": (_I, [_P, _P, _I, _I, _P, _P, _P, _L, _F, _I, _P, _P, _P, _P, _P, _P, _I, _I, _I, _I, _I, _I, _I, _I, _I, _P]),
+    "k22_conv3_halo_ring_depth": (_I, [_I, _I, _I, _I]),
     "k22_debug_conv_trace": (_I, [_P, _P, _P, _P, _I, _I, _I, _I, _I, _I, _P, _P]),
     "k22_groupnorm": (_I, [_P, _P, _I, _I, _I, _I, _I, _P, _P, _P, _L, _F, _I, _I, _I, _P, _P, _I, _P]),
     "k22_groupnorm_scratch_bytes": (_Z, [_I, _I]),
diff --git a/kandinsky-2_amd/csrc/capi.hip b/kandinsky-2_amd/csrc/capi.hip
--- a/kandinsky-2_amd/csrc/capi.hip
+++ b/kandinsky-2_amd/csrc/capi.hip
@@ -49,12 +49,24 @@
 #else
 #define K22_DBG_TRACE(p) (void)0
 #endif
+#ifdef K22_DEBUG_VARIANTS
+static unsigned long long* g_dbg_kloop_trace = nullptr;
+extern "C" int k22_debug_set_kloop_trace(unsigned long long* t, long workgroups) {
+  if (t != nullptr && workgroups < 4096) return k22_set_error(K22_EINVAL, "k22_debug_set_kloop_trace: the buffer holds 4096 workgroups x 2 x 8 stamps");
+  g_dbg_kloop_trace = t;
+  return K22_OK;
+}
+#define K22_DBG_KLOOP(p) (p).trace = g_dbg_kloop_trace
+#else
+#define K22_DBG_KLOOP(p) (void)0
+#endif
 static const void* g_dbg_wfrag = nullptr;
 static const void* g_dbg_wsfrag = nullptr;
 static void* g_dbg_scratch = nullptr;
 static size_t g_dbg_scratch_bytes = 0;
 static int dbg_frag(IgemmParams& p, int dtype, hipStream_t st) {
   K22_DBG_TRACE(p);
+  K22_DBG_KLOOP(p);
   p.Wfrag = g_dbg_wfrag; p.Wsfrag = g_dbg_wsfrag;
   if (g_dbg_wfrag || !g_dbg_scratch || dtype == K22_F32 || (p.taps != 1 && p.taps != 9) || p.Kc % 64 || p.Npad % 64) return K22_OK;
   const size_t n1 = stream_frag_bytes(p.Npad, p.taps, p.Kc, dtype);
@@ -296,6 +308,13 @@
   return launch_igemm(q, d.dtype, reinterpret_cast<hipStream_t>(stream));
 }
 
+int k22_conv3_halo_ring_depth(int H, int W, int bm, int fused_skip) {
+  IgemmParams p = {};
+  p.H = H; p.W = W; p.taps = 9;
+  if (fused_skip) p.S0 = reinterpret_cast<const void*>(1);
+  return conv3_halo_ring_depth(p, bm);
+}
+
 int k22_debug_conv_trace(const void* x_padded, const void* Wp, const float* bias, void* out, int B, int H, int W, int Cin, int Cout,
                          int Npad, unsigned long long* trace, void* stream) {
   IgemmParams p = {};
diff --git a/kandinsky-2_amd/csrc/common.h b/kandinsky-2_amd/csrc/common.h
--- a/kandinsky-2_amd/csrc/common.h
+++ b/kandinsky-2_amd/csrc/common.h
@@ -217,6 +217,44 @@
   asm volatile("" ::: "memory");
 }
 
+template <int N> __device__ __forceinline__ void k22_wait_vmcnt() { asm volatile("s_waitcnt vmcnt(%0)" ::"n"(N) : "memory"); }
+constexpr int slab_ring_ahead(int nst, int left) { return left < nst - 2 ? left : nst - 2; }
+constexpr int slab_ring_wait(int nst, int ch, int left) { return slab_ring_ahead(nst, left) * ch; }
+constexpr bool slab_ring_issues(int nst, int left) { return left >= nst - 1; }
+constexpr bool slab_ring_ok(int nst, int ch, int n) {
+  int issued = 0, retired = 0, next = 0;
+  for (int t = 0; t < nst - 1 && next < n; ++t) { issued += ch; ++next; }
+  for (int s = 0; s < n; ++s) {
+    const int w = slab_ring_wait(nst, ch, n - 1 - s);
+    if (w > issued - retired) return false;
+    if (issued - w > retired) retired = issued - w;
+    if (retired < (s + 1) * ch) return false;
+    if (slab_ring_issues(nst, n - 1 - s)) {
+      if (next != s + nst - 1) return false;
+      issued += ch; ++next;
+    }
+  }
+  return next == n && retired == issued;
+}
+constexpr bool slab_ring_ok_all(int nst, int ch) {
+  if ((nst - 2) * ch > 63) return false;
+  for (int n = 1; n <= 2 * nst + 2; ++n)
+    if (!slab_ring_ok(nst, ch, n)) return false;
+  return true;
+}
+template <int CH, int A> __device__ __forceinline__ void slab_ring_wait_le(int left) {
+  if constexpr (A == 0) {
+    k22_wait_vmcnt<0>();
+  } else {
+    if (left >= A) k22_wait_vmcnt<A * CH>();
+    else slab_ring_wait_le<CH, A - 1>(left);
+  }
+}
+template <int NST, int CH> __device__ __forceinline__ void slab_ring_wait_vmcnt(int left) {
+  static_assert(slab_ring_ok_all(NST, CH), "slab ring: counted waits do not match the issue schedule");
+  slab_ring_wait_le<CH, NST - 2>(left);
+}
+
 __device__ __forceinline__ float wave_sum(float v) {
 #pragma unroll
   for (int o = 32; o > 0; o >>= 1) v += __shfl_xor(v, o, 64);
diff --git a/kandinsky-2_amd/csrc/conv3_common.h b/kandinsky-2_amd/csrc/conv3_common.h
--- a/kandinsky-2_amd/csrc/conv3_common.h
+++ b/kandinsky-2_amd/csrc/conv3_common.h
@@ -80,6 +80,31 @@
 }
 template <> __device__ __forceinline__ void load8f<x3_t>(const x3_t* src, float* v) { load8f<float>(reinterpret_cast<const float*>(src), v); }
 template <> __device__ __forceinline__ void load8f<x2_t>(const x2_t* src, float* v) { load8f<float>(reinterpret_cast<const float*>(src), v); }
+template <typename T> struct ResSeg {
+  uint4 r;
+  __device__ __forceinline__ void load(const T* src) { r = *reinterpret_cast<const uint4*>(src); }
+  __device__ __forceinline__ void unpack(float* v) const;
+};
+template <> __device__ __forceinline__ void ResSeg<bf16_t>::unpack(float* v) const {
+  v[0] = __uint_as_float(r.x << 16); v[1] = __uint_as_float(r.x & 0xffff0000u);
+  v[2] = __uint_as_float(r.y << 16); v[3] = __uint_as_float(r.y & 0xffff0000u);
+  v[4] = __uint_as_float(r.z << 16); v[5] = __uint_as_float(r.z & 0xffff0000u);
+  v[6] = __uint_as_float(r.w << 16); v[7] = __uint_as_float(r.w & 0xffff0000u);
+}
+template <> __device__ __forceinline__ void ResSeg<f16_t>::unpack(float* v) const {
+  unpack2_f16(r.x, v[0], v[1]); unpack2_f16(r.y, v[2], v[3]); unpack2_f16(r.z, v[4], v[5]); unpack2_f16(r.w, v[6], v[7]);
+}
+template <typename T> struct ResSeg32 {
+  float4 a, b;
+  __device__ __forceinline__ void load(const T* src) {
+    a = *reinterpret_cast<const float4*>(src);
+    b = *(reinterpret_cast<const float4*>(src) + 1);
+  }
+  __device__ __forceinline__ void unpack(float* v) const { v[0] = a.x; v[1] = a.y; v[2] = a.z; v[3] = a.w; v[4] = b.x; v[5] = b.y; v[6] = b.z; v[7] = b.w; }
+};
+template <> struct ResSeg<float> : ResSeg32<float> {};
+template <> struct ResSeg<x3_t> : ResSeg32<x3_t> {};
+template <> struct ResSeg<x2_t> : ResSeg32<x2_t> {};
 template <typename T> __device__ __forceinline__ float stored(float v);
 template <> __device__ __forceinline__ float stored<bf16_t>(float v) { return bf16_to_f32(f32_to_bf16(v)); }
 template <> __device__ __forceinline__ float stored<f16_t>(float v) { return (float)(f16_t)v; }
@@ -163,10 +188,60 @@
   return c;
 }
 
+constexpr int KLOOP_TRACE_WORKGROUPS = 4096;
+struct KStamp {
+#ifdef K22_DEBUG_VARIANTS
+  unsigned long long t[6] = {0, 0, 0, 0, 0, 0};
+  __device__ __forceinline__ void at(int i) { t[i] = __builtin_amdgcn_s_memrealtime(); }
+  __device__ __forceinline__ void flush(const IgemmParams& p) const {
+    const int w = threadIdx.x >> 6;
+    if (p.trace == nullptr || (threadIdx.x & 63) != 0 || (w != 0 && w != 4) || blockIdx.x >= KLOOP_TRACE_WORKGROUPS) return;
+    unsigned long long* o = p.trace + ((size_t)blockIdx.x * 2 + (w >> 2)) * 8;
+#pragma unroll
+    for (int i = 0; i < 6; ++i) o[i] = t[i];
+  }
+#else
+  __device__ __forceinline__ void at(int) {}
+  __device__ __forceinline__ void flush(const IgemmParams&) const {}
+#endif
+};
+
+template <int NBST> constexpr int tap_ring_wait(int tap, bool last, int b, int a) {
+  if (!last) return b * (NBST - 2) + a * halo_count_a<NBST>(tap);
+  return b * (8 - tap < NBST - 2 ? 8 - tap : NBST - 2);
+}
+template <int NBST> constexpr bool tap_ring_issues_b(int tap, bool last) { return !last || tap + NBST - 1 < 9; }
+template <int NBST> constexpr bool tap_ring_issues_a(int tap, bool last) { return !last && tap <= 9 - NBST; }
+template <int NBST> constexpr bool tap_ring_ok(int n, int b, int a) {
+  int issued = 0, retired = 0;
+  int tile_end[9 + NBST] = {};
+  int halo_end = 0, halo_next_end = 0;
+  issued += (10 - NBST) * a; halo_end = issued;
+  for (int t = 0; t < NBST - 1; ++t) { issued += b; tile_end[t] = issued; }
+  for (int s = 0; s < n; ++s) {
+    const bool last = s == n - 1;
+    for (int t = 0; t < 9; ++t) {
+      const int w = tap_ring_wait<NBST>(t, last, b, a);
+      if (w > 63 || w > issued - retired) return false;
+      if (issued - w > retired) retired = issued - w;
+      if (tile_end[t] == 0 || tile_end[t] > retired) return false;
+      if (t == 0 && halo_end > retired) return false;
+      if (tap_ring_issues_b<NBST>(t, last)) { issued += b; tile_end[t + NBST - 1] = issued; }
+      if (tap_ring_issues_a<NBST>(t, last)) { issued += a; halo_next_end = issued; }
+    }
+    for (int t = 0; t < NBST; ++t) { tile_end[t] = tile_end[9 + t]; tile_end[9 + t] = 0; }
+    for (int t = NBST; t < 9; ++t) tile_end[t] = 0;
+    halo_end = halo_next_end;
+  }
+  return retired == issued;
+}
+template <int NBST> constexpr bool tap_ring_ok_all(int b, int a) { return tap_ring_ok<NBST>(1, b, a) && tap_ring_ok<NBST>(2, b, a) && tap_ring_ok<NBST>(3, b, a); }
+
 }
 
 template <typename T, int BM, bool PLAIN = false, bool SPEC = false>
-__device__ __forceinline__ void halo_tail(const IgemmParams& p, f32x16_t (&acc)[SPEC ? BM / 64 : BM / 128][2], char* smem, int bx, int bz, int img, int v0, int n0) {
+__device__ __forceinline__ void halo_tail(const IgemmParams& p, f32x16_t (&acc)[SPEC ? BM / 64 : BM / 128][2], char* smem, int bx, int bz, int img, int v0, int n0,
+                                          KStamp& ks) {
   using TR = TT<T>;
   constexpr int BK = TR::BK, EPC = TR::EPC, KSTEPS = TR::KSTEPS;
   constexpr int BN = HALO_BN, NW = HALO_NW, WM = SPEC ? 2 : 4, WN = 2;
@@ -225,9 +300,7 @@
       const unsigned lds0 = __builtin_amdgcn_readfirstlane((unsigned)(size_t)(__attribute__((address_space(3))) char*)smem);
 #define K22_ISSUE_SKIP(Q, BUFI)                                                                            \
       {                                                                                                    \
-        int q_ = (Q);                                                                                      \
-        if (q_ > q1 - 1) q_ = q1 - 1;                                                                      \
-        const int k0_ = q_ * BK;                                                                           \
+        const int k0_ = (Q) * BK;                                                                          \
         const bool second_ = k0_ >= p.SK0;                                                                 \
         const T* xs_ = second_ ? X1 : X0;                                                                  \
         const int ldx_ = second_ ? p.SK1 : p.SK0;                                                          \
@@ -239,37 +312,80 @@
             glds16w_asm(Ws + wsoff[i] + k0_, __builtin_amdgcn_readfirstlane(dA_ + BM * 128 + i * NW * 1024)); \
       }
 #pragma unroll
-      for (int t = 0; t < NSK - 1; ++t) K22_ISSUE_SKIP(q0 + t, t);
+      for (int t = 0; t < NSK - 1; ++t)
+        if (q0 + t < q1) K22_ISSUE_SKIP(q0 + t, t);
       int buf = 0, fill = NSK - 1;
-      for (int q = q0; q < q1; ++q) {
-        wait_vmcnt<(NSK - 2) * SCH>();
-        raw_barrier();
-        K22_ISSUE_SKIP(q + NSK - 1, fill);
-        const char* sA = smem + buf * SBUF;
-        const char* sB = sA + BM * 128;
-        if (cw) {
-        using TSK = typename SkipT<T>::type;
-#pragma unroll
-        for (int ks = 0; ks < KSTEPS; ++ks) {
-          Frag<TSK> a[MI], b[NI];
-#pragma unroll
-          for (int mi = 0; mi < MI; ++mi) ld_frag_at_a<true, TSK>(a[mi], sA + (abase + mi * 32) * 128, bsw, ks, h);
-#pragma unroll
-          for (int ni = 0; ni < NI; ++ni) ld_frag_at(b[ni], sB + brow[ni], bsw, ks, h);
-#pragma unroll
-          for (int mi = 0; mi < MI; ++mi)
-#pragma unroll
-            for (int ni = 0; ni < NI; ++ni) mma_atom(acc[mi][ni], b[ni], a[mi]);
-        }
-        }
-        asm volatile("s_waitcnt lgkmcnt(0)" ::: "memory");
-        buf = (buf + 1 == NSK) ? 0 : buf + 1;
-        fill = (fill + 1 == NSK) ? 0 : fill + 1;
-      }
+#define K22_SKIP_SLAB(FULL)                                                                                \
+      {                                                                                                    \
+        if constexpr (FULL) k22_wait_vmcnt<slab_ring_wait(NSK, SCH, NSK)>();                               \
+        else slab_ring_wait_vmcnt<NSK, SCH>(q1 - 1 - q);                                                   \
+        raw_barrier();                                                                                     \
+        if constexpr (FULL) K22_ISSUE_SKIP(q + NSK - 1, fill);                                             \
+        const char* sA = smem + buf * SBUF; \
+        const char* sB = sA + BM * 128; \
+        if (cw) { \
+         \
+         \
+        using TSK = typename SkipT<T>::type; \
+_Pragma("unroll") \
+        for (int ks = 0; ks < KSTEPS; ++ks) { \
+          Frag<TSK> a[MI], b[NI]; \
+_Pragma("unroll") \
+          for (int mi = 0; mi < MI; ++mi) ld_frag_at_a<true, TSK>(a[mi], sA + (abase + mi * 32) * 128, bsw, ks, h);    \
+_Pragma("unroll") \
+          for (int ni = 0; ni < NI; ++ni) ld_frag_at(b[ni], sB + brow[ni], bsw, ks, h); \
+_Pragma("unroll") \
+          for (int mi = 0; mi < MI; ++mi) \
+_Pragma("unroll") \
+            for (int ni = 0; ni < NI; ++ni) mma_atom(acc[mi][ni], b[ni], a[mi]); \
+        } \
+        } \
+        asm volatile("s_waitcnt lgkmcnt(0)" ::: "memory");    \
+        buf = (buf + 1 == NSK) ? 0 : buf + 1; \
+        fill = (fill + 1 == NSK) ? 0 : fill + 1; \
+      }
+      int q = q0;
+      for (; q < q1 - (NSK - 1); ++q) K22_SKIP_SLAB(true)
+      for (; q < q1; ++q) K22_SKIP_SLAB(false)
+#undef K22_SKIP_SLAB
 #undef K22_ISSUE_SKIP
     }
   }
   wait_vmcnt<0>();
+  ks.at(3);
+
+  constexpr int SEGS = BN / 8;
+  constexpr int RGS = 512 / SEGS;
+  constexpr int RPT = BM / RGS;
+  const int cs = tid % SEGS, rg = tid / SEGS;
+  const int n = n0 + cs * 8;
+  const bool n_ok = n < p.N;
+  const bool finish = (p.splitk <= 1);
+  const T* __restrict__ res = reinterpret_cast<const T*>(p.residual);
+  bool qkv_vt = false;
+  if constexpr (PLAIN) qkv_vt = p.out_mode == IG_OUT_QKV && n0 >= 2 * (p.N / 3);
+  const bool pre = finish && n_ok && !qkv_vt;
+  const bool has_b2 = !PLAIN && pre && p.bias2 != nullptr;
+  float4 pb[PLAIN ? 2 : 4];
+#pragma unroll
+  for (int e = 0; e < (PLAIN ? 2 : 4); ++e) pb[e] = make_float4(0.f, 0.f, 0.f, 0.f);
+  if (pre && p.bias != nullptr) { pb[0] = *reinterpret_cast<const float4*>(p.bias + n); pb[1] = *reinterpret_cast<const float4*>(p.bias + n + 4); }
+  if constexpr (!PLAIN) {
+    if (has_b2) { pb[2] = *reinterpret_cast<const float4*>(p.bias2 + n); pb[3] = *reinterpret_cast<const float4*>(p.bias2 + n + 4); }
+  }
+  int mrow[RPT];
+  ResSeg<T> rseg[RPT];
+#pragma unroll
+  for (int k = 0; k < RPT; ++k) {
+    const int v = v0 + rg * RPT + k;
+    if constexpr (PLAIN) {
+      mrow[k] = (!n_ok || v >= VR) ? -1 : img * VR + v;
+    } else {
+      const int y = v / W2, x = v - y * W2;
+      mrow[k] = (!n_ok || v >= VR || x >= p.W) ? -1 : (img * p.H + y) * p.W + x;
+    }
+    if (pre && res != nullptr && mrow[k] >= 0) rseg[k].load(res + (int64_t)mrow[k] * p.ldr + n);
+  }
   __syncthreads();
 
   if (cw)
@@ -287,6 +403,7 @@
       }
   }
   __syncthreads();
+  ks.at(4);
 
   if constexpr (PLAIN) {
     if (p.out_mode == IG_OUT_QKV && n0 >= 2 * (p.N / 3)) {
@@ -310,31 +427,18 @@
           vt[(int64_t)3 * p.att_Tkp] = from_f32<T>(t.w + b.w);
         }
       }
+      ks.at(5);
       return;
     }
   }
 
-  constexpr int SEGS = BN / 8;
-  constexpr int RGS = 512 / SEGS;
-  constexpr int RPT = BM / RGS;
-  const int cs = tid % SEGS, rg = tid / SEGS;
-  const int n = n0 + cs * 8;
-  const bool n_ok = n < p.N;
-  float bias8[8];
-#pragma unroll
-  for (int e = 0; e < 8; ++e) bias8[e] = 0.f;
-  const bool finish = (p.splitk <= 1);
-  if (finish && n_ok && p.bias != nullptr) {
-    const float4 b0 = *reinterpret_cast<const float4*>(p.bias + n), b1 = *reinterpret_cast<const float4*>(p.bias + n + 4);
-    bias8[0] = b0.x; bias8[1] = b0.y; bias8[2] = b0.z; bias8[3] = b0.w;
-    bias8[4] = b1.x; bias8[5] = b1.y; bias8[6] = b1.z; bias8[7] = b1.w;
-  }
-  if (finish && n_ok && p.bias2 != nullptr) {
-    const float4 b0 = *reinterpret_cast<const float4*>(p.bias2 + n), b1 = *reinterpret_cast<const float4*>(p.bias2 + n + 4);
-    bias8[0] += b0.x; bias8[1] += b0.y; bias8[2] += b0.z; bias8[3] += b0.w;
-    bias8[4] += b1.x; bias8[5] += b1.y; bias8[6] += b1.z; bias8[7] += b1.w;
-  }
-  const T* __restrict__ res = reinterpret_cast<const T*>(p.residual);
+  float bias8[8] = {pb[0].x, pb[0].y, pb[0].z, pb[0].w, pb[1].x, pb[1].y, pb[1].z, pb[1].w};
+  if constexpr (!PLAIN) {
+    if (has_b2) {
+      bias8[0] += pb[2].x; bias8[1] += pb[2].y; bias8[2] += pb[2].z; bias8[3] += pb[2].w;
+      bias8[4] += pb[3].x; bias8[5] += pb[3].y; bias8[6] += pb[3].z; bias8[7] += pb[3].w;
+    }
+  }
   float* part = finish ? nullptr : p.partial + (int64_t)bz * p.M * p.N;
   float ssum[8], ssq[8];
 #pragma unroll
@@ -343,15 +447,8 @@
   for (int k = 0; k < RPT; ++k) {
     const int row = rg * RPT + k;
     const int v = v0 + row;
-    int64_t m;
-    if constexpr (PLAIN) {
-      if (!n_ok || v >= VR) continue;
-      m = (int64_t)img * VR + v;
-    } else {
-      const int y = v / W2, x = v - y * W2;
-      if (!n_ok || v >= VR || x >= p.W) continue;
-      m = ((int64_t)img * p.H + y) * p.W + x;
-    }
+    const int64_t m = mrow[k];
+    if (m < 0) continue;
     const float4 t0 = *reinterpret_cast<const float4*>(smem + row * TS + cs * 32);
     const float4 t1 = *reinterpret_cast<const float4*>(smem + row * TS + cs * 32 + 16);
     float val[8] = {t0.x, t0.y, t0.z, t0.w, t1.x, t1.y, t1.z, t1.w};
@@ -364,7 +461,7 @@
     for (int e = 0; e < 8; ++e) val[e] += bias8[e];
     if (res != nullptr) {
       float rv[8];
-      load8f<T>(res + m * p.ldr + n, rv);
+      rseg[k].unpack(rv);
 #pragma unroll
       for (int e = 0; e < 8; ++e) val[e] += rv[e];
     }
@@ -396,6 +493,7 @@
       }
     }
   }
+  ks.at(5);
   if (!finish || p.stats == nullptr) return;
 
   __syncthreads();
diff --git a/kandinsky-2_amd/csrc/conv3_halo.hip b/kandinsky-2_amd/csrc/conv3_halo.hip
--- a/kandinsky-2_amd/csrc/conv3_halo.hip
+++ b/kandinsky-2_amd/csrc/conv3_halo.hip
@@ -22,6 +22,8 @@
   constexpr int GM = 8;
   extern __shared__ __attribute__((aligned(16))) char smem[];
 
+  KStamp ks;
+  ks.at(0);
   const int tid = threadIdx.x, lane = tid & 63;
   const int wave = __builtin_amdgcn_readfirstlane(tid >> 6);
   const int wm = wave >> 1, wn = wave & 1;
@@ -135,28 +137,26 @@
 #pragma unroll
       for (int t = 0; t < NBST - 1; ++t) K22_ISSUE_B(s0, t, t);
     }
+    static_assert(tap_ring_ok_all<NBST>(B_SLOTS, APT), "tap ring: counted waits do not match the issue schedule");
     int trace_it = 0;
     (void)trace_it;
     int cur = 0;
     int fill = NBST - 1;
-    for (int s = s0; s < s1; ++s) {
-      char* const Acur = smem + ((s - s0) & 1) * A_BYTES;
-      char* const Anext = smem + (((s - s0) & 1) ^ 1) * A_BYTES;
-      const int sn = s + 1 < s1 ? s + 1 : s1 - 1;
-#define K22_TAP(TAP)                                                                                       \
+#define K22_TAP(TAP, LAST)                                                                                 \
       {                                                                                                    \
         unsigned long long tr0_ = 0, tr1_ = 0, tr2_ = 0;                                                   \
         if constexpr (TRACE) tr0_ = __builtin_amdgcn_s_memtime();                                          \
-        if (loader && !DBG_NOLOAD) wait_vmcnt<B_SLOTS * (NBST - 2) + APT * halo_count_a<NBST>(TAP)>();     \
+        if (loader && !DBG_NOLOAD) wait_vmcnt<tap_ring_wait<NBST>(TAP, LAST, B_SLOTS, APT)>();             \
         if constexpr (TRACE) tr1_ = __builtin_amdgcn_s_memtime();                                          \
         raw_barrier();                                                                      \
         if constexpr (TRACE) tr2_ = __builtin_amdgcn_s_memtime();                                          \
+        if constexpr ((TAP) == 0) { if (s == s0) ks.at(1); }                                               \
                     \
         if (loader && !DBG_NOLOAD) {                                                                       \
           constexpr int ta_ = ((TAP) + NBST - 1) % 9;                                                      \
           const int sa_ = ((TAP) + NBST - 1 >= 9) ? sn : s;                                                \
-          K22_ISSUE_B(sa_, ta_, fill);                                                                     \
-          if constexpr ((TAP) <= 9 - NBST) {                                                               \
+          if constexpr (tap_ring_issues_b<NBST>(TAP, LAST)) K22_ISSUE_B(sa_, ta_, fill);                   \
+          if constexpr (tap_ring_issues_a<NBST>(TAP, LAST)) {                                              \
             _Pragma("unroll") for (int a_ = 0; a_ < APT; ++a_) {                                           \
               constexpr int qb_ = ((TAP) <= 9 - NBST ? (TAP) : 0) * APT;                                   \
               K22_ISSUE_A(qb_ + a_, sn, Anext);                                                            \
@@ -221,9 +221,19 @@
         cur = (cur + 1 == NBST) ? 0 : cur + 1;                                                             \
         fill = (fill + 1 == NBST) ? 0 : fill + 1;                                                          \
       }
-      K22_TAP(0) K22_TAP(1) K22_TAP(2) K22_TAP(3) K22_TAP(4) K22_TAP(5) K22_TAP(6) K22_TAP(7) K22_TAP(8)
+#define K22_SLAB(LAST)                                                                                     \
+    {                                                                                                      \
+      char* const Acur = smem + ((s - s0) & 1) * A_BYTES;                                                  \
+      char* const Anext = smem + (((s - s0) & 1) ^ 1) * A_BYTES;                                           \
+      const int sn = s + 1;                                                                                \
+      (void)Anext; (void)sn;                                                                               \
+      K22_TAP(0, LAST) K22_TAP(1, LAST) K22_TAP(2, LAST) K22_TAP(3, LAST) K22_TAP(4, LAST) K22_TAP(5, LAST) K22_TAP(6, LAST) K22_TAP(7, LAST) K22_TAP(8, LAST) \
+    }
+    int s = s0;
+    for (; s < s1 - 1; ++s) K22_SLAB(false)
+    K22_SLAB(true)
+#undef K22_SLAB
 #undef K22_TAP
-    }
   }
 #undef K22_ISSUE_A
 #undef K22_ISSUE_B
@@ -233,7 +243,9 @@
 #pragma unroll
       for (int ni = 0; ni < NI; ++ni) mma_atom(acc[mi][ni], pb[ni], pa[mi]);
   }
-  halo_tail<T, BM>(p, acc, smem, bx, bz, img, v0, n0);
+  ks.at(2);
+  halo_tail<T, BM>(p, acc, smem, bx, bz, img, v0, n0, ks);
+  ks.flush(p);
 }
 
 template <typename T, int BM, int NST, bool ARAW = false>
@@ -247,6 +259,8 @@
   constexpr int GM = 8;
   extern __shared__ __attribute__((aligned(16))) char smem[];
 
+  KStamp ks;
+  ks.at(0);
   const int tid = threadIdx.x, lane = tid & 63;
   const int wave = __builtin_amdgcn_readfirstlane(tid >> 6);
   const int wm = wave >> 1, wn = wave & 1;
@@ -304,8 +318,7 @@
   const unsigned lds0 = __builtin_amdgcn_readfirstlane((unsigned)(size_t)(__attribute__((address_space(3))) char*)smem);
 #define K22_ISSUE_G(SLAB, STAGE)                                                                           \
   {                                                                                                        \
-    int sl_ = (SLAB);                                                                                      \
-    if (sl_ > s1 - 1) sl_ = s1 - 1;       \
+    const int sl_ = (SLAB);            \
     const unsigned d_ = lds0 + (STAGE) * BUF + wave * 1024;                                                \
     _Pragma("unroll") for (int i = 0; i < A_SLOTS; ++i)                                                    \
         glds16_asm(A + aoff[i] + sl_ * BK, __builtin_amdgcn_readfirstlane(d_ + i * NW * 1024));            \
@@ -321,12 +334,15 @@
 
   if (s0 < s1) {
 #pragma unroll
-    for (int t = 0; t < NST - 1; ++t) K22_ISSUE_G(s0 + t, t);
+    for (int t = 0; t < NST - 1; ++t)
+      if (s0 + t < s1) K22_ISSUE_G(s0 + t, t);
     int cur = 0, fill = NST - 1;
     for (int s = s0; s < s1; ++s) {
-      wait_vmcnt<(NST - 2) * CH>();
+      const int left = s1 - 1 - s;
+      slab_ring_wait_vmcnt<NST, CH>(left);
       raw_barrier();
-      K22_ISSUE_G(s + NST - 1, fill);
+      if (s == s0) ks.at(1);
+      if (slab_ring_issues(NST, left)) K22_ISSUE_G(s + NST - 1, fill);
       const char* St = smem + cur * BUF;
 #pragma unroll
       for (int ks = 0; ks < KSTEPS; ++ks) {
@@ -346,7 +362,9 @@
     }
   }
 #undef K22_ISSUE_G
-  halo_tail<T, BM, true>(p, acc, smem, bx, bz, img, v0, n0);
+  ks.at(2);
+  halo_tail<T, BM, true>(p, acc, smem, bx, bz, img, v0, n0, ks);
+  ks.flush(p);
 }
 
 template <typename T, int BM, int NST>
@@ -362,6 +380,8 @@
   constexpr int GM = 8;
   extern __shared__ __attribute__((aligned(16))) char smem[];
 
+  KStamp ks;
+  ks.at(0);
   const int tid = threadIdx.x, lane = tid & 63;
   const int wave = __builtin_amdgcn_readfirstlane(tid >> 6);
   const bool producer = wave >= 4;
@@ -422,8 +442,7 @@
       const unsigned lds0 = __builtin_amdgcn_readfirstlane((unsigned)(size_t)(__attribute__((address_space(3))) char*)smem);
 #define K22_ISSUE_GS(SLAB, STAGE)                                                                          \
       {                                                                                                    \
-        int sl_ = (SLAB);                                                                                  \
-        if (sl_ > s1 - 1) sl_ = s1 - 1;    \
+        const int sl_ = (SLAB);            \
         const unsigned d_ = lds0 + (STAGE) * BUF + lw * 1024;                                              \
         _Pragma("unroll") for (int i = 0; i < A_SLOTS; ++i)                                                \
             glds16_asm(A + aoff[i] + sl_ * BK, __builtin_amdgcn_readfirstlane(d_ + i * NWL * 1024));       \
@@ -431,12 +450,15 @@
             glds16w_asm(Wp + boff[i] + sl_ * BK, __builtin_amdgcn_readfirstlane(d_ + A_BYTES + i * NWL * 1024)); \
       }
 #pragma unroll
-      for (int t = 0; t < NST - 1; ++t) K22_ISSUE_GS(s0 + t, t);
+      for (int t = 0; t < NST - 1; ++t)
+        if (s0 + t < s1) K22_ISSUE_GS(s0 + t, t);
       int fill = NST - 1;
       for (int s = s0; s < s1; ++s) {
-        wait_vmcnt<(NST - 2) * CH>();
+        const int left = s1 - 1 - s;
+        slab_ring_wait_vmcnt<NST, CH>(left);
         raw_barrier();
-        K22_ISSUE_GS(s + NST - 1, fill);
+        if (s == s0) ks.at(1);
+        if (slab_ring_issues(NST, left)) K22_ISSUE_GS(s + NST - 1, fill);
         fill = (fill + 1 == NST) ? 0 : fill + 1;
       }
 #undef K22_ISSUE_GS
@@ -466,6 +488,7 @@
       int cur = 0;
       for (int s = s0; s < s1; ++s) {
         raw_barrier();
+        if (s == s0) ks.at(1);
         const char* St = smem + cur * BUF;
         Frag<T> ca[MI], cb[NI];
 #pragma unroll
@@ -499,7 +522,9 @@
         for (int ni = 0; ni < NI; ++ni) mma_atom(acc[mi][ni], pb[ni], pa[mi]);
     }
   }
-  halo_tail<T, BM, true, true>(p, acc, smem, bx, bz, img, v0, n0);
+  ks.at(2);
+  halo_tail<T, BM, true, true>(p, acc, smem, bx, bz, img, v0, n0, ks);
+  ks.flush(p);
 }
 
 namespace {
@@ -671,7 +696,8 @@
   }
 #undef K22_ISSUE_A3
 #undef K22_ISSUE_B3
-  halo_tail<T, BM>(p, acc, smem, bx, bz, img, v0, n0);
+  KStamp ks;
+  halo_tail<T, BM>(p, acc, smem, bx, bz, img, v0, n0, ks);
 }
 
 static int halo3_rows(const IgemmParams& p, int bm) { return (bm + 2 * (p.W + 2) + 2 + 15) & ~15; }
@@ -768,6 +794,8 @@
   if (bm == 256) return launch_gemm8_cfg<float, 256, 3>(p, splitk, stream);
   return nst == 2 ? launch_gemm8_cfg<float, 128, 2>(p, splitk, stream) : launch_gemm8_cfg<float, 128, 4>(p, splitk, stream);
 }
+
+int conv3_halo_ring_depth(const IgemmParams& p, int bm) { return halo_pick_nbst(p, bm); }
 
 bool conv3_halo_supported(const IgemmParams& p, int dtype, int bm) {
   const int BK = k22_bk(dtype);
diff --git a/kandinsky-2_amd/csrc/conv3_spec.hip b/kandinsky-2_amd/csrc/conv3_spec.hip
--- a/kandinsky-2_amd/csrc/conv3_spec.hip
+++ b/kandinsky-2_amd/csrc/conv3_spec.hip
@@ -13,6 +13,8 @@
   constexpr int GM = 8;
   extern __shared__ __attribute__((aligned(16))) char smem[];
 
+  KStamp ks;
+  ks.at(0);
   const int tid = threadIdx.x, lane = tid & 63;
   const int wave = __builtin_amdgcn_readfirstlane(tid >> 6);
   const bool producer = wave >= 4;
@@ -226,20 +228,30 @@
 #pragma unroll
       for (int t = 0; t < NBST - 1; ++t) K22_SP_B(s0, t, t);
       int fill = NBST - 1;
+      static_assert(tap_ring_ok_all<NBST>(B_SLOTS, APT), "tap ring: counted waits do not match the issue schedule");
       for (int s = s0; s < s1; ++s) {
         const int anext_off = (((s - s0) & 1) ^ 1) * A_BYTES;
-        const int sn = s + 1 < s1 ? s + 1 : s1 - 1;
+        const int sn = s + 1;
+        const bool last = sn == s1;
 #define K22_SP_PTAP(TAP)                                                                                   \
         {                                                                                                  \
-          if constexpr (DBG == 0) wait_vmcnt<B_SLOTS * (NBST - 2) + APT * halo_count_a<NBST>(TAP)>();      \
+          if constexpr (DBG == 0) {                                                                        \
+            if (last) wait_vmcnt<tap_ring_wait<NBST>(TAP, true, B_SLOTS, APT)>();                          \
+            else wait_vmcnt<tap_ring_wait<NBST>(TAP, false, B_SLOTS, APT)>();                              \
+          }                                                                                                \
           raw_barrier();                                                                                   \
+          if constexpr ((TAP) == 0) { if (s == s0) ks.at(1); }                                             \
           constexpr int ta_ = ((TAP) + NBST - 1) % 9;                                                      \
           const int sa_ = ((TAP) + NBST - 1 >= 9) ? sn : s;                                                \
-          if constexpr (DBG != 1) K22_SP_B(sa_, ta_, fill);                                                \
-          if constexpr ((TAP) <= 9 - NBST && DBG != 1) {                                                   \
+          if constexpr (DBG != 1) {                                                                        \
+            if (tap_ring_issues_b<NBST>(TAP, true) || !last) K22_SP_B(sa_, ta_, fill);                     \
+          }                                                                                                \
+          if constexpr (tap_ring_issues_a<NBST>(TAP, false) && DBG != 1) {                                 \
+            if (!last) {                                                                                   \
             _Pragma("unroll") for (int a_ = 0; a_ < APT; ++a_) {                                           \
               constexpr int qb_ = ((TAP) <= 9 - NBST ? (TAP) : 0) * APT;                                   \
               K22_SP_A(qb_ + a_, sn, anext_off);                                                           \
+            }                                                                                              \
             }                                                                                              \
           }                                                                                                \
           fill = (fill + 1 == NBST) ? 0 : fill + 1;                                                        \
@@ -282,6 +294,7 @@
 #define K22_SP_CTAP(TAP)                                                                                   \
         {                                                                                                  \
           raw_barrier();                                                                                   \
+          if constexpr ((TAP) == 0) { if (s == s0) ks.at(1); }                                             \
           const char* Bcur = Bst + cur * B_BYTES;                                                          \
           const int shift = ((TAP) / 3) * W2 + ((TAP) % 3);                                                \
           const char* arow[MI];                                                                            \
@@ -332,7 +345,9 @@
       }
     }
   }
-  halo_tail<T, BM, false, true>(p, acc, smem, bx, bz, img, v0, n0);
+  ks.at(2);
+  halo_tail<T, BM, false, true>(p, acc, smem, bx, bz, img, v0, n0, ks);
+  ks.flush(p);
 }
 
 
diff --git a/kandinsky-2_amd/csrc/igemm.hip b/kandinsky-2_amd/csrc/igemm.hip
--- a/kandinsky-2_amd/csrc/igemm.hip
+++ b/kandinsky-2_amd/csrc/igemm.hip
@@ -1,7 +1,5 @@
 #include "kernels.h"
 #include <stdlib.h>
-
-template <int N> __device__ __forceinline__ void wait_vmcnt() { asm volatile("s_waitcnt vmcnt(%0)" ::"n"(N) : "memory"); }
 
 template <typename T> __device__ __forceinline__ void store4(T* dst, const float* v);
 template <> __device__ __forceinline__ void store4<bf16_t>(bf16_t* dst, const float* v) {
@@ -122,8 +120,7 @@
 
 #define K22_ISSUE(KT, BUFI)                                                                              \
   {                                                                                                      \
-    int kt_ = (KT);                                                                                      \
-    if (kt_ > kt1 - 1) kt_ = kt1 - 1;  \
+    const int kt_ = (KT);              \
     const int tap_ = kt_ / kt_per_tap;                                                                   \
     const int k0_ = (kt_ - tap_ * kt_per_tap) * BK;                                                      \
     const bool second_ = (!conv) && (k0_ >= p.K0);                                                       \
@@ -143,12 +140,14 @@
 
   if (kt0 < kt1) {
 #pragma unroll
-    for (int s_ = 0; s_ < STAGES - 1; ++s_) K22_ISSUE(kt0 + s_, s_);
+    for (int s_ = 0; s_ < STAGES - 1; ++s_)
+      if (kt0 + s_ < kt1) K22_ISSUE(kt0 + s_, s_);
     int cur = 0, fill = STAGES - 1;
     for (int kt = kt0; kt < kt1; ++kt) {
-      wait_vmcnt<(STAGES - 2) * CH>();
+      const int left = kt1 - 1 - kt;
+      slab_ring_wait_vmcnt<STAGES, CH>(left);
       raw_barrier();
-      K22_ISSUE(kt + STAGES - 1, fill);
+      if (slab_ring_issues(STAGES, left)) K22_ISSUE(kt + STAGES - 1, fill);
       {
         const char* As = smem + cur * BUF;
         const char* Bs = As + A_BYTES;
@@ -169,7 +168,6 @@
       cur = (cur + 1 == STAGES) ? 0 : cur + 1;
       fill = (fill + 1 == STAGES) ? 0 : fill + 1;
     }
-    wait_vmcnt<0>();
   }
 #undef K22_ISSUE
 
diff --git a/kandinsky-2_amd/csrc/kernels.h b/kandinsky-2_amd/csrc/kernels.h
--- a/kandinsky-2_amd/csrc/kernels.h
+++ b/kandinsky-2_amd/csrc/kernels.h
@@ -70,6 +70,7 @@
 int conv3_halo_tiles_per_image(const IgemmParams& p, int bm);
 int launch_conv3_halo(const IgemmParams& p, int dtype, int bm, int splitk, hipStream_t stream);
 int launch_conv3_halo_trace(const IgemmParams& p, int dtype, hipStream_t stream);
+int conv3_halo_ring_depth(const IgemmParams& p, int bm);
 bool gemm8_supported(const IgemmParams& p, int dtype, int bm);
 bool gemm8_spec_supported(int dtype);
 int gemm8_tiles_per_image(const IgemmParams& p, int bm);
```

Result: no change. 141.4 steps/s, median of 6 (+0.3%).
